# yeyupiaoling/PPASR

Hardware: AMD Instinct MI355X
Metric: audio-seconds/s (RTF^-1) Conformer-streaming fbank, batch32 per GPU, ctc_greedy (higher is better)
Workload: dtype f32; 1 GPU; configs[1]: Conformer streaming (configs/conformer.yml), fbank-80, 32 x 10 s utterances per GPU, V=4233, ctc_greedy, features resident in HBM -> token ids + scores on device; global_batch=32, frames=1000, decoder=ctc_greedy, parallelism=utterance-dp1, pipelined=False, gemm=f32

## Files before the change

include/ppasr_hip.h:

```cpp
#ifndef PPASR_HIP_H
#define PPASR_HIP_H

#include <stddef.h>
#include <stdint.h>

#define PPASR_API __attribute__((visibility("default")))

#ifdef __cplusplus
extern "C" {
#endif

typedef struct ppasr_model_s* ppasr_handle;
typedef struct ppasr_stream_s* ppasr_stream;

typedef enum {
  PPASR_OK = 0,
  PPASR_EINVAL = 1,
  PPASR_EHIP = 2,
  PPASR_EUNSUPPORTED = 3,
  PPASR_EMISSING = 4,
  PPASR_ENOSPACE = 5
} ppasr_status;

enum { PPASR_MODEL_CONFORMER = 0, PPASR_MODEL_EFFICIENT_CONFORMER = 1,
       PPASR_MODEL_SQUEEZEFORMER = 2, PPASR_MODEL_DEEPSPEECH2 = 3 };

typedef struct {
  const char* name;
  const float* data_host;
  int ndim;
  int64_t shape[4];
} ppasr_weight_blob;

typedef struct {
  int model_type;
  int input_dim;
  int vocab_size;
  int output_size;
  int attention_heads;
  int linear_units;
  int num_blocks;
  int cnn_module_kernel;
  int causal;
  int max_len;
  int reduce_idx;
  int recover_idx;
  int stride_layer_idx;
  int group_layer_mask;
  int group_size;
  int use_gru;
  int input_layer;
  int options;
  int stride_layer_mask;
} ppasr_model_desc;

enum {
  PPASR_OPT_POS_REL = 0,
  PPASR_OPT_POS_ABS = 1,
  PPASR_OPT_POS_NONE = 2,
  PPASR_OPT_POS_MASK = 3,
  PPASR_OPT_POST_NORM = 4,
  PPASR_OPT_CONCAT_AFTER = 8,
  PPASR_OPT_NO_MACARON = 16,
  PPASR_OPT_NO_CNN = 32,
  PPASR_OPT_SQ_NO_ADAPTIVE_SCALE = 4096,
  PPASR_OPT_SQ_PRE_NORM = 8192,
  PPASR_OPT_ACT_SHIFT = 8,
  PPASR_OPT_ACT_MASK = 15
};
enum { PPASR_ACT_SWISH = 0, PPASR_ACT_RELU = 1, PPASR_ACT_GELU = 2, PPASR_ACT_TANH = 3, PPASR_ACT_HARDTANH = 4,
       PPASR_ACT_RELU6 = 5, PPASR_ACT_LEAKYRELU = 6, PPASR_ACT_SELU = 7, PPASR_ACT_ELU = 8, PPASR_ACT_HARDSWISH = 9,
       PPASR_ACT_HARDSHRINK = 10 };

PPASR_API const char* ppasr_last_error(void);
PPASR_API const char* ppasr_version(void);

PPASR_API ppasr_status ppasr_create(const ppasr_model_desc* desc, const ppasr_weight_blob* weights_host, int n_weights,
                          ppasr_handle* out);
PPASR_API ppasr_status ppasr_destroy(ppasr_handle h);

PPASR_API int ppasr_out_frames(ppasr_handle h, int T);
PPASR_API size_t ppasr_workspace_bytes(ppasr_handle h, int B, int T);

PPASR_API ppasr_status ppasr_encode(ppasr_handle h, const float* feats, const int64_t* lens, int B, int T,
                          float* probs, float* logits, int32_t* frame_argmax, float* frame_maxprob,
                          void* workspace, size_t workspace_bytes, void* stream);

PPASR_API ppasr_status ppasr_set_debug_taps(ppasr_handle h, float* taps, size_t n_floats);

PPASR_API ppasr_status ppasr_set_skip_padding(ppasr_handle h, int enable);

PPASR_API ppasr_status ppasr_set_ffn_split(ppasr_handle h, int mode);

PPASR_API ppasr_status ppasr_set_front_fused(ppasr_handle h, int mode);

#define PPASR_ROW_BLOCK_32_W16 1032
PPASR_API ppasr_status ppasr_set_row_block(ppasr_handle h, int rows);

#define PPASR_GEMM_F32 0
#define PPASR_GEMM_F16X3 1
#define PPASR_GEMM_COVERS_LAYERS 1
#define PPASR_GEMM_COVERS_FRONT 2
#define PPASR_GEMM_COVERS_HEAD 4
PPASR_API ppasr_status ppasr_set_gemm_mode(ppasr_handle h, int mode);
PPASR_API int ppasr_gemm_coverage(ppasr_handle h);
PPASR_API ppasr_status ppasr_set_gemm_guard(ppasr_handle h, int enable);
PPASR_API ppasr_status ppasr_gemm_guard_stats(ppasr_handle h, long long* fallbacks_host, long long* events_host);
PPASR_API ppasr_status ppasr_set_lengths_hint(ppasr_handle h, const int64_t* lens_host, int B);

PPASR_API long long ppasr_edit_distance(const int32_t* a, int na, const int32_t* b, int nb);

PPASR_API size_t ppasr_ctc_beam_state_bytes(int B, int max_frames, int beam_size);
PPASR_API size_t ppasr_ctc_beam_scratch_bytes(int B, int T, int V, int beam_size, double cutoff_prob, int cutoff_top_n);
PPASR_API ppasr_status ppasr_ctc_beam_state_grow(const void* old_state, size_t old_bytes, void* new_state, size_t new_bytes, int B,
                                       int beam_size, void* stream);
PPASR_API ppasr_status ppasr_ctc_beam_status(const void* state, size_t state_bytes, int B, int beam_size, int32_t* status_host,
                                   void* stream);
PPASR_API ppasr_status ppasr_ctc_beam_state_compact(void* state, size_t state_bytes, int B, int beam_size, int rebuild_table,
                                          int32_t* live_nodes_host, void* stream);
PPASR_API ppasr_status ppasr_ctc_beam_search(const float* probs, const int32_t* frame_lens, int B, int T, int V, int beam_size,
                                   double cutoff_prob, int cutoff_top_n, int blank, int nbest, int max_tokens,
                                   int32_t* tokens, int32_t* lens, double* scores, void* state, size_t state_bytes,
                                   int init_state, void* stream);

typedef struct ppasr_lm_s* ppasr_lm_handle;
PPASR_API ppasr_status ppasr_lm_create(const char* model_path, const char* const* vocab_utf8, int V, ppasr_lm_handle* out);
PPASR_API ppasr_status ppasr_lm_create_arpa(const char* arpa_path, const char* const* vocab_utf8, int V, ppasr_lm_handle* out);
PPASR_API ppasr_status ppasr_lm_create_klm(const char* klm_path, const char* const* vocab_utf8, int V, ppasr_lm_handle* out);
PPASR_API const char*  ppasr_lm_format(ppasr_lm_handle lm);
PPASR_API int          ppasr_lm_word_index(ppasr_lm_handle lm, int token);
PPASR_API int          ppasr_lm_bos(ppasr_lm_handle lm);
PPASR_API int          ppasr_lm_eos(ppasr_lm_handle lm);
PPASR_API ppasr_status ppasr_lm_debug_load_host(const char* model_path, const char* const* vocab_utf8, int V, ppasr_lm_handle* out);
PPASR_API double       ppasr_lm_debug_host_score(ppasr_lm_handle lm, const int32_t* window);
PPASR_API ppasr_status ppasr_lm_destroy(ppasr_lm_handle lm);
PPASR_API int          ppasr_lm_order(ppasr_lm_handle lm);
PPASR_API int          ppasr_lm_is_character_based(ppasr_lm_handle lm);
PPASR_API long long    ppasr_lm_dict_size(ppasr_lm_handle lm);
PPASR_API int          ppasr_lm_space_id(ppasr_lm_handle lm);
PPASR_API long long    ppasr_lm_ngram_count(ppasr_lm_handle lm);
PPASR_API ppasr_status ppasr_ctc_beam_search_lm(const float* probs, const int32_t* frame_lens, int B, int T, int V, int beam_size,
                                      double cutoff_prob, int cutoff_top_n, int blank, int nbest, int max_tokens,
                                      int32_t* tokens, int32_t* lens, double* scores, void* state, size_t state_bytes,
                                      int init_state, ppasr_lm_handle lm, double alpha, double beta, void* stream);
PPASR_API ppasr_status ppasr_ctc_beam_search_ws(const float* probs, const int32_t* frame_lens, int B, int T, int V, int beam_size,
                                      double cutoff_prob, int cutoff_top_n, int blank, int nbest, int max_tokens,
                                      int32_t* tokens, int32_t* lens, double* scores, void* state, size_t state_bytes,
                                      int init_state, ppasr_lm_handle lm, double alpha, double beta, void* scratch,
                                      size_t scratch_bytes, void* stream);

PPASR_API ppasr_status ppasr_hyp_pack(const int32_t* tokens, long long token_stride, int L, const int32_t* n_tokens,
                                      long long n_stride, const double* score, long long score_stride, const int32_t* index,
                                      int k, int32_t* rec, int row0, int cols, int extra, void* stream);
PPASR_API ppasr_status ppasr_hyp_unpack(const int32_t* rec, const int64_t* order, int N, int cols, int extra, int32_t* tokens,
                                        int32_t* n_tokens, double* score, int32_t* index, void* stream);

PPASR_API ppasr_status ppasr_stream_create(ppasr_handle h, ppasr_stream* out);
PPASR_API ppasr_status ppasr_stream_destroy(ppasr_stream s);
PPASR_API ppasr_status ppasr_stream_reset(ppasr_stream s, void* stream);
PPASR_API int ppasr_stream_offset(ppasr_stream s);
PPASR_API int ppasr_stream_cache_frames(ppasr_stream s);
PPASR_API size_t ppasr_chunk_workspace_bytes(ppasr_handle h, int T);
PPASR_API ppasr_status ppasr_encode_chunk(ppasr_stream s, const float* feats, int T, int required_cache_size, float* probs,
                                int32_t* frame_argmax, float* frame_maxprob, int* c_out_host, void* workspace,
                                size_t workspace_bytes, void* stream);
PPASR_API ppasr_status ppasr_stream_export_cache(ppasr_stream s, float* att_cache, float* cnn_cache, void* stream);
PPASR_API ppasr_status ppasr_stream_import_cache(ppasr_stream s, const float* att_cache, int cache_t, const float* cnn_cache,
                                       int offset, void* stream);

PPASR_API size_t ppasr_ds2_workspace_bytes(ppasr_handle h, int B, int T);
PPASR_API ppasr_status ppasr_debug_occupy_cus(int n_workgroups, int milliseconds, void* stream);
PPASR_API ppasr_status ppasr_ds2_encode(ppasr_handle h, const float* feats, const int64_t* lens, int B, int T, const float* init_h,
                              const float* init_c, float* probs, int64_t* out_lens, float* final_h, float* final_c,
                              void* workspace, size_t workspace_bytes, void* stream);

#define PPASR_N_KERNEL_CLASSES 10
PPASR_API ppasr_status ppasr_profile_enable(ppasr_handle h, int enable);
PPASR_API ppasr_status ppasr_profile_read(ppasr_handle h, float* total_ms_host, int* launches_host);
PPASR_API const char* ppasr_kernel_class_name(int cls);

#define PPASR_KPROF_NAME_LEN 160
PPASR_API ppasr_status ppasr_kprof_begin(void);
PPASR_API ppasr_status ppasr_kprof_end(int max_entries, char* names_host, float* total_ms_host, int* launches_host, int* n_out_host);

PPASR_API ppasr_status ppasr_ctc_greedy(const float* probs, const int32_t* frame_lens, int B, int Tp, int V, int blank,
                              int32_t* tokens, int32_t* n_tokens, double* score,
                              void* workspace , size_t workspace_bytes, void* stream);

PPASR_API ppasr_status ppasr_ctc_collapse(const int32_t* frame_argmax, const float* frame_maxprob, const int32_t* frame_lens,
                                int B, int Tp, int blank, int32_t* tokens, int32_t* n_tokens, double* score,
                                void* stream);

typedef struct ppasr_stream_group_s* ppasr_stream_group;
PPASR_API ppasr_status ppasr_stream_group_create(ppasr_handle h, int n_sessions, int max_frames, ppasr_stream_group* out);
PPASR_API ppasr_status ppasr_sq_stream_group_create(ppasr_handle h, int n_sessions, int max_frames, ppasr_stream_group* out);
PPASR_API ppasr_status ppasr_eff_stream_group_create(ppasr_handle h, int n_sessions, int max_frames, ppasr_stream_group* out);
PPASR_API ppasr_status ppasr_ds2_stream_group_create(ppasr_handle h, int n_sessions, int max_frames, ppasr_stream_group* out);
PPASR_API ppasr_status ppasr_gen_stream_group_create(ppasr_handle h, int n_sessions, int max_frames, ppasr_stream_group* out);
PPASR_API ppasr_status ppasr_stream_group_destroy(ppasr_stream_group g);
PPASR_API ppasr_status ppasr_stream_group_reset(ppasr_stream_group g, int session , void* stream);
PPASR_API int          ppasr_stream_group_offset(ppasr_stream_group g, int session);
PPASR_API size_t       ppasr_group_chunk_workspace_bytes(ppasr_handle h, int n, int T);
PPASR_API ppasr_status ppasr_encode_chunk_group(ppasr_stream_group g, const int* sessions_host, int n, const float* feats, int T,
                                      float* probs, int32_t* frame_argmax, float* frame_maxprob, int* c_out_host,
                                      void* workspace, size_t workspace_bytes, void* stream);

typedef struct ppasr_beam_pool_s* ppasr_beam_pool;
PPASR_API ppasr_status ppasr_beam_pool_create(int n_sessions, int V, int beam_size, double cutoff_prob, int cutoff_top_n,
                                              int blank, ppasr_lm_handle lm , double alpha, double beta,
                                              int init_frames, ppasr_beam_pool* out);
PPASR_API ppasr_status ppasr_beam_pool_destroy(ppasr_beam_pool pool);
PPASR_API ppasr_status ppasr_beam_pool_reset(ppasr_beam_pool pool, int session, void* stream);
PPASR_API long long    ppasr_beam_pool_frames(ppasr_beam_pool pool, int session);
PPASR_API long long    ppasr_beam_pool_capacity(ppasr_beam_pool pool, int session);
PPASR_API ppasr_status ppasr_beam_pool_status(ppasr_beam_pool pool, int32_t* status_host, void* stream);
PPASR_API size_t       ppasr_beam_pool_workspace_bytes(ppasr_beam_pool pool, int n, int T);
PPASR_API ppasr_status ppasr_beam_pool_decode(ppasr_beam_pool pool, const int* sessions_host, int n, const float* probs, int T,
                                              const int32_t* frame_lens_host, int max_tokens, int32_t* tokens, int32_t* lens,
                                              double* scores, void* workspace, size_t workspace_bytes, void* stream);

PPASR_API ppasr_status ppasr_beam_arena_compact(ppasr_beam_pool pool, const int* sessions_host, int n, long long* live_nodes_host,
                                                void* stream);
PPASR_API ppasr_status ppasr_beam_arena_set_auto(ppasr_beam_pool pool, int enable);
PPASR_API long long    ppasr_beam_arena_live_nodes(ppasr_beam_pool pool, int session);
PPASR_API size_t       ppasr_beam_arena_bytes(ppasr_beam_pool pool);

typedef struct ppasr_fbank_s* ppasr_fbank_handle;
PPASR_API ppasr_status ppasr_fbank_create(int sample_rate, int n_mels, float frame_length_ms, float frame_shift_ms,
                                ppasr_fbank_handle* out);
PPASR_API ppasr_status ppasr_fbank_destroy(ppasr_fbank_handle f);
PPASR_API int          ppasr_fbank_frames(ppasr_fbank_handle f, int n_samples);
PPASR_API size_t       ppasr_fbank_workspace_bytes(ppasr_fbank_handle f, int n_samples);
PPASR_API ppasr_status ppasr_fbank_compute(ppasr_fbank_handle f, const float* samples, int n_samples, int use_db_norm,
                                 float target_db, float* feats, void* workspace, size_t workspace_bytes, void* stream);

typedef struct {
  long long first_sample;
  long long out_row;
  int n_samples;
  int first_chunk;
  int first_frame;
  int reserved;
} ppasr_fbank_segment;
PPASR_API ppasr_status ppasr_fbank_plan_batch(int sample_rate, float frame_length_ms, float frame_shift_ms, const int* n_samples,
                                    int n, int t_max, ppasr_fbank_segment* table, int* total_chunks, int* total_frames);
PPASR_API size_t       ppasr_fbank_batch_workspace_bytes(int n, int total_chunks);
PPASR_API ppasr_status ppasr_fbank_compute_batch(ppasr_fbank_handle f, const float* samples, const ppasr_fbank_segment* table_dev,
                                       int n, int total_chunks, int total_frames, int use_db_norm, float target_db,
                                       float* feats, void* workspace, size_t workspace_bytes, void* stream);

#ifdef __cplusplus
}
#endif
#endif
```

ppasr_amd/_lib.py:

```python
import ctypes
import os

_HERE = os.path.dirname(os.path.abspath(__file__))
LIB_PATH = os.environ.get("PPASR_HIP_LIB") or os.path.join(_HERE, "libppasr_hip.so")

c_i32p = ctypes.POINTER(ctypes.c_int32)
c_i64p = ctypes.POINTER(ctypes.c_int64)
c_f32p = ctypes.POINTER(ctypes.c_float)
c_f64p = ctypes.POINTER(ctypes.c_double)

PPASR_OK, PPASR_EINVAL, PPASR_EHIP, PPASR_EUNSUPPORTED, PPASR_EMISSING, PPASR_ENOSPACE = range(6)

PPASR_MODEL_CONFORMER = 0
PPASR_MODEL_EFFICIENT_CONFORMER = 1
PPASR_MODEL_SQUEEZEFORMER = 2
PPASR_MODEL_DEEPSPEECH2 = 3
N_KERNEL_CLASSES = 10
PPASR_OPT_POST_NORM, PPASR_OPT_CONCAT_AFTER, PPASR_OPT_NO_MACARON, PPASR_OPT_NO_CNN, PPASR_OPT_ACT_SHIFT = 4, 8, 16, 32, 8
PPASR_OPT_SQ_NO_ADAPTIVE_SCALE = 4096
PPASR_OPT_SQ_PRE_NORM = 8192
PPASR_GEMM_F32 = 0
PPASR_GEMM_F16X3 = 1
PPASR_GEMM_COVERS_LAYERS, PPASR_GEMM_COVERS_FRONT, PPASR_GEMM_COVERS_HEAD = 1, 2, 4
KPROF_NAME_LEN = 160


class WeightBlob(ctypes.Structure):
    _fields_ = [("name", ctypes.c_char_p), ("data_host", ctypes.c_void_p), ("ndim", ctypes.c_int),
                ("shape", ctypes.c_int64 * 4)]


class FbankSegment(ctypes.Structure):
    _fields_ = [("first_sample", ctypes.c_longlong), ("out_row", ctypes.c_longlong), ("n_samples", ctypes.c_int),
                ("first_chunk", ctypes.c_int), ("first_frame", ctypes.c_int), ("reserved", ctypes.c_int)]


class ModelDesc(ctypes.Structure):
    _fields_ = [("model_type", ctypes.c_int), ("input_dim", ctypes.c_int), ("vocab_size", ctypes.c_int),
                ("output_size", ctypes.c_int), ("attention_heads", ctypes.c_int), ("linear_units", ctypes.c_int),
                ("num_blocks", ctypes.c_int), ("cnn_module_kernel", ctypes.c_int), ("causal", ctypes.c_int),
                ("max_len", ctypes.c_int), ("reduce_idx", ctypes.c_int), ("recover_idx", ctypes.c_int),
                ("stride_layer_idx", ctypes.c_int), ("group_layer_mask", ctypes.c_int), ("group_size", ctypes.c_int),
                ("use_gru", ctypes.c_int), ("input_layer", ctypes.c_int), ("options", ctypes.c_int),
                ("stride_layer_mask", ctypes.c_int)]


_vp = ctypes.c_void_p
SYMBOLS = [
    ("ppasr_last_error", ctypes.c_char_p, []),
    ("ppasr_version", ctypes.c_char_p, []),
    ("ppasr_create", ctypes.c_int, [ctypes.POINTER(ModelDesc), ctypes.POINTER(WeightBlob), ctypes.c_int,
                                    ctypes.POINTER(_vp)]),
    ("ppasr_destroy", ctypes.c_int, [_vp]),
    ("ppasr_out_frames", ctypes.c_int, [_vp, ctypes.c_int]),
    ("ppasr_workspace_bytes", ctypes.c_size_t, [_vp, ctypes.c_int, ctypes.c_int]),
    ("ppasr_encode", ctypes.c_int, [_vp, _vp, _vp, ctypes.c_int, ctypes.c_int, _vp, _vp, _vp, _vp, _vp,
                                    ctypes.c_size_t, _vp]),
    ("ppasr_set_debug_taps", ctypes.c_int, [_vp, _vp, ctypes.c_size_t]),
    ("ppasr_set_skip_padding", ctypes.c_int, [_vp, ctypes.c_int]),
    ("ppasr_set_row_block", ctypes.c_int, [_vp, ctypes.c_int]),
    ("ppasr_set_lengths_hint", ctypes.c_int, [_vp, _vp, ctypes.c_int]),
    ("ppasr_set_ffn_split", ctypes.c_int, [_vp, ctypes.c_int]),
    ("ppasr_set_front_fused", ctypes.c_int, [_vp, ctypes.c_int]),
    ("ppasr_set_gemm_mode", ctypes.c_int, [_vp, ctypes.c_int]),
    ("ppasr_gemm_coverage", ctypes.c_int, [_vp]),
    ("ppasr_set_gemm_guard", ctypes.c_int, [_vp, ctypes.c_int]),
    ("ppasr_gemm_guard_stats", ctypes.c_int, [_vp, ctypes.POINTER(ctypes.c_longlong), ctypes.POINTER(ctypes.c_longlong)]),
    ("ppasr_edit_distance", ctypes.c_longlong, [_vp, ctypes.c_int, _vp, ctypes.c_int]),
    ("ppasr_ctc_beam_state_bytes", ctypes.c_size_t, [ctypes.c_int, ctypes.c_int, ctypes.c_int]),
    ("ppasr_ctc_beam_search", ctypes.c_int, [_vp, _vp, ctypes.c_int, ctypes.c_int, ctypes.c_int, ctypes.c_int,
                                             ctypes.c_double, ctypes.c_int, ctypes.c_int, ctypes.c_int, ctypes.c_int,
                                             _vp, _vp, _vp, _vp, ctypes.c_size_t, ctypes.c_int, _vp]),
    ("ppasr_stream_create", ctypes.c_int, [_vp, ctypes.POINTER(_vp)]),
    ("ppasr_stream_destroy", ctypes.c_int, [_vp]),
    ("ppasr_stream_reset", ctypes.c_int, [_vp, _vp]),
    ("ppasr_stream_offset", ctypes.c_int, [_vp]),
    ("ppasr_stream_cache_frames", ctypes.c_int, [_vp]),
    ("ppasr_chunk_workspace_bytes", ctypes.c_size_t, [_vp, ctypes.c_int]),
    ("ppasr_encode_chunk", ctypes.c_int, [_vp, _vp, ctypes.c_int, ctypes.c_int, _vp, _vp, _vp,
                                          ctypes.POINTER(ctypes.c_int), _vp, ctypes.c_size_t, _vp]),
    ("ppasr_stream_export_cache", ctypes.c_int, [_vp, _vp, _vp, _vp]),
    ("ppasr_stream_import_cache", ctypes.c_int, [_vp, _vp, ctypes.c_int, _vp, ctypes.c_int, _vp]),
    ("ppasr_ds2_workspace_bytes", ctypes.c_size_t, [_vp, ctypes.c_int, ctypes.c_int]),
    ("ppasr_ds2_encode", ctypes.c_int, [_vp, _vp, _vp, ctypes.c_int, ctypes.c_int, _vp, _vp, _vp, _vp, _vp, _vp, _vp,
                                        ctypes.c_size_t, _vp]),
    ("ppasr_debug_occupy_cus", ctypes.c_int, [ctypes.c_int, ctypes.c_int, _vp]),
    ("ppasr_profile_enable", ctypes.c_int, [_vp, ctypes.c_int]),
    ("ppasr_profile_read", ctypes.c_int, [_vp, c_f32p, c_i32p]),
    ("ppasr_kernel_class_name", ctypes.c_char_p, [ctypes.c_int]),
    ("ppasr_kprof_begin", ctypes.c_int, []),
    ("ppasr_kprof_end", ctypes.c_int, [ctypes.c_int, _vp, c_f32p, c_i32p, ctypes.POINTER(ctypes.c_int)]),
    ("ppasr_ctc_greedy", ctypes.c_int, [_vp, _vp, ctypes.c_int, ctypes.c_int, ctypes.c_int, ctypes.c_int, _vp, _vp,
                                        _vp, _vp, ctypes.c_size_t, _vp]),
    ("ppasr_ctc_collapse", ctypes.c_int, [_vp, _vp, _vp, ctypes.c_int, ctypes.c_int, ctypes.c_int, _vp, _vp, _vp,
                                          _vp]),
    ("ppasr_lm_create_arpa", ctypes.c_int, [ctypes.c_char_p, ctypes.POINTER(ctypes.c_char_p), ctypes.c_int,
                                            ctypes.POINTER(_vp)]),
    ("ppasr_ctc_beam_scratch_bytes", ctypes.c_size_t, [ctypes.c_int, ctypes.c_int, ctypes.c_int, ctypes.c_int,
                                                       ctypes.c_double, ctypes.c_int]),
    ("ppasr_ctc_beam_search_ws", ctypes.c_int, [_vp, _vp, ctypes.c_int, ctypes.c_int, ctypes.c_int, ctypes.c_int,
                                                ctypes.c_double, ctypes.c_int, ctypes.c_int, ctypes.c_int, ctypes.c_int,
                                                _vp, _vp, _vp, _vp, ctypes.c_size_t, ctypes.c_int, _vp, ctypes.c_double,
                                                ctypes.c_double, _vp, ctypes.c_size_t, _vp]),
    ("ppasr_ctc_beam_status", ctypes.c_int, [_vp, ctypes.c_size_t, ctypes.c_int, ctypes.c_int, _vp, _vp]),
    ("ppasr_ctc_beam_state_grow", ctypes.c_int, [_vp, ctypes.c_size_t, _vp, ctypes.c_size_t, ctypes.c_int, ctypes.c_int, _vp]),
    ("ppasr_hyp_pack", ctypes.c_int, [_vp, ctypes.c_longlong, ctypes.c_int, _vp, ctypes.c_longlong, _vp, ctypes.c_longlong, _vp,
                                      ctypes.c_int, _vp, ctypes.c_int, ctypes.c_int, ctypes.c_int, _vp]),
    ("ppasr_hyp_unpack", ctypes.c_int, [_vp, _vp, ctypes.c_int, ctypes.c_int, ctypes.c_int, _vp, _vp, _vp, _vp, _vp]),
    ("ppasr_lm_create", ctypes.c_int, [ctypes.c_char_p, ctypes.POINTER(ctypes.c_char_p), ctypes.c_int,
                                       ctypes.POINTER(_vp)]),
    ("ppasr_lm_create_klm", ctypes.c_int, [ctypes.c_char_p, ctypes.POINTER(ctypes.c_char_p), ctypes.c_int,
                                           ctypes.POINTER(_vp)]),
    ("ppasr_lm_debug_load_host", ctypes.c_int, [ctypes.c_char_p, ctypes.POINTER(ctypes.c_char_p), ctypes.c_int,
                                                ctypes.POINTER(_vp)]),
    ("ppasr_lm_debug_host_score", ctypes.c_double, [_vp, _vp]),
    ("ppasr_lm_format", ctypes.c_char_p, [_vp]),
    ("ppasr_lm_word_index", ctypes.c_int, [_vp, ctypes.c_int]),
    ("ppasr_lm_bos", ctypes.c_int, [_vp]),
    ("ppasr_lm_eos", ctypes.c_int, [_vp]),
    ("ppasr_lm_destroy", ctypes.c_int, [_vp]),
    ("ppasr_lm_order", ctypes.c_int, [_vp]),
    ("ppasr_lm_is_character_based", ctypes.c_int, [_vp]),
    ("ppasr_lm_dict_size", ctypes.c_longlong, [_vp]),
    ("ppasr_lm_space_id", ctypes.c_int, [_vp]),
    ("ppasr_lm_ngram_count", ctypes.c_longlong, [_vp]),
    ("ppasr_ctc_beam_search_lm", ctypes.c_int, [_vp, _vp, ctypes.c_int, ctypes.c_int, ctypes.c_int, ctypes.c_int,
                                                ctypes.c_double, ctypes.c_int, ctypes.c_int, ctypes.c_int, ctypes.c_int,
                                                _vp, _vp, _vp, _vp, ctypes.c_size_t, ctypes.c_int, _vp, ctypes.c_double,
                                                ctypes.c_double, _vp]),
    ("ppasr_stream_group_create", ctypes.c_int, [_vp, ctypes.c_int, ctypes.c_int, ctypes.POINTER(_vp)]),
    ("ppasr_sq_stream_group_create", ctypes.c_int, [_vp, ctypes.c_int, ctypes.c_int, ctypes.POINTER(_vp)]),
    ("ppasr_eff_stream_group_create", ctypes.c_int, [_vp, ctypes.c_int, ctypes.c_int, ctypes.POINTER(_vp)]),
    ("ppasr_ds2_stream_group_create", ctypes.c_int, [_vp, ctypes.c_int, ctypes.c_int, ctypes.POINTER(_vp)]),
    ("ppasr_gen_stream_group_create", ctypes.c_int, [_vp, ctypes.c_int, ctypes.c_int, ctypes.POINTER(_vp)]),
    ("ppasr_stream_group_destroy", ctypes.c_int, [_vp]),
    ("ppasr_stream_group_reset", ctypes.c_int, [_vp, ctypes.c_int, _vp]),
    ("ppasr_stream_group_offset", ctypes.c_int, [_vp, ctypes.c_int]),
    ("ppasr_group_chunk_workspace_bytes", ctypes.c_size_t, [_vp, ctypes.c_int, ctypes.c_int]),
    ("ppasr_encode_chunk_group", ctypes.c_int, [_vp, ctypes.POINTER(ctypes.c_int), ctypes.c_int, _vp, ctypes.c_int, _vp,
                                                _vp, _vp, ctypes.POINTER(ctypes.c_int), _vp, ctypes.c_size_t, _vp]),
    ("ppasr_beam_pool_create", ctypes.c_int, [ctypes.c_int, ctypes.c_int, ctypes.c_int, ctypes.c_double, ctypes.c_int,
                                              ctypes.c_int, _vp, ctypes.c_double, ctypes.c_double, ctypes.c_int,
                                              ctypes.POINTER(_vp)]),
    ("ppasr_beam_pool_destroy", ctypes.c_int, [_vp]),
    ("ppasr_beam_pool_reset", ctypes.c_int, [_vp, ctypes.c_int, _vp]),
    ("ppasr_beam_pool_frames", ctypes.c_longlong, [_vp, ctypes.c_int]),
    ("ppasr_beam_pool_capacity", ctypes.c_longlong, [_vp, ctypes.c_int]),
    ("ppasr_beam_pool_status", ctypes.c_int, [_vp, _vp, _vp]),
    ("ppasr_beam_pool_workspace_bytes", ctypes.c_size_t, [_vp, ctypes.c_int, ctypes.c_int]),
    ("ppasr_beam_pool_decode", ctypes.c_int, [_vp, ctypes.POINTER(ctypes.c_int), ctypes.c_int, _vp, ctypes.c_int, _vp,
                                              ctypes.c_int, _vp, _vp, _vp, _vp, ctypes.c_size_t, _vp]),
    ("ppasr_ctc_beam_state_compact", ctypes.c_int, [_vp, ctypes.c_size_t, ctypes.c_int, ctypes.c_int, ctypes.c_int, _vp, _vp]),
    ("ppasr_beam_arena_compact", ctypes.c_int, [_vp, ctypes.POINTER(ctypes.c_int), ctypes.c_int,
                                                ctypes.POINTER(ctypes.c_longlong), _vp]),
    ("ppasr_beam_arena_set_auto", ctypes.c_int, [_vp, ctypes.c_int]),
    ("ppasr_beam_arena_live_nodes", ctypes.c_longlong, [_vp, ctypes.c_int]),
    ("ppasr_beam_arena_bytes", ctypes.c_size_t, [_vp]),
    ("ppasr_fbank_create", ctypes.c_int, [ctypes.c_int, ctypes.c_int, ctypes.c_float, ctypes.c_float,
                                          ctypes.POINTER(_vp)]),
    ("ppasr_fbank_destroy", ctypes.c_int, [_vp]),
    ("ppasr_fbank_frames", ctypes.c_int, [_vp, ctypes.c_int]),
    ("ppasr_fbank_workspace_bytes", ctypes.c_size_t, [_vp, ctypes.c_int]),
    ("ppasr_fbank_compute", ctypes.c_int, [_vp, _vp, ctypes.c_int, ctypes.c_int, ctypes.c_float, _vp, _vp,
                                           ctypes.c_size_t, _vp]),
    ("ppasr_fbank_plan_batch", ctypes.c_int, [ctypes.c_int, ctypes.c_float, ctypes.c_float, _vp, ctypes.c_int, ctypes.c_int,
                                              _vp, ctypes.POINTER(ctypes.c_int), ctypes.POINTER(ctypes.c_int)]),
    ("ppasr_fbank_batch_workspace_bytes", ctypes.c_size_t, [ctypes.c_int, ctypes.c_int]),
    ("ppasr_fbank_compute_batch", ctypes.c_int, [_vp, _vp, _vp, ctypes.c_int, ctypes.c_int, ctypes.c_int, ctypes.c_int,
                                                 ctypes.c_float, _vp, _vp, ctypes.c_size_t, _vp]),
]

_lib = None


class PPASRHipError(RuntimeError):

    def __init__(self, msg, status=None):
        super().__init__(msg)
        self.status = status


def load():
    global _lib
    if _lib is not None:
        return _lib
    if not os.path.exists(LIB_PATH):
        raise PPASRHipError(
            f"{LIB_PATH} not found: build it with `python -c 'import __graft_entry__ as g; g.build()'` "
            "(hipcc --offload-arch=gfx950).  There is no CPU fallback.")
    lib = ctypes.CDLL(LIB_PATH)
    for name, restype, argtypes in SYMBOLS:
        fn = getattr(lib, name)
        fn.restype = restype
        fn.argtypes = argtypes
    _lib = lib
    return lib


def check(status):
    if status != 0:
        msg = load().ppasr_last_error()
        raise PPASRHipError(f"libppasr_hip status {status}: {msg.decode() if msg else ''}", status=int(status))


class kernel_profile:

    _stack = []

    def __init__(self, max_entries=128):
        self.max_entries = max_entries
        self.kernels = {}

    @staticmethod
    def _drain():
        n = max([k.max_entries for k in kernel_profile._stack] + [512])
        names = ctypes.create_string_buffer(n * KPROF_NAME_LEN)
        ms = (ctypes.c_float * n)()
        cnt = (ctypes.c_int32 * n)()
        got = ctypes.c_int(0)
        check(load().ppasr_kprof_end(n, ctypes.addressof(names), ms, cnt, ctypes.byref(got)))
        for i in range(got.value):
            nm = names.raw[i * KPROF_NAME_LEN:(i + 1) * KPROF_NAME_LEN].split(b"\0", 1)[0].decode()
            for scope in kernel_profile._stack:
                t, c = scope.kernels.get(nm, (0.0, 0))
                scope.kernels[nm] = (t + float(ms[i]), c + int(cnt[i]))

    def __enter__(self):
        if kernel_profile._stack:
            kernel_profile._drain()
        kernel_profile._stack.append(self)
        check(load().ppasr_kprof_begin())
        return self

    def __exit__(self, *exc):
        kernel_profile._drain()
        kernel_profile._stack.pop()
        if kernel_profile._stack:
            check(load().ppasr_kprof_begin())
        return False
```

ppasr_amd/csrc/capi.hip:

```cpp
#include <cxxabi.h>
#include <cstdlib>

#include "capi_internal.h"

namespace ppasr {
thread_local LaunchProf g_launch_prof;
}

static thread_local std::string g_err;
std::string& ppasr_err_slot() { return g_err; }

static ppasr_status validate_desc(const ppasr_model_desc* desc, ppasr_model_s* m) {
  m->desc = *desc;
  const int F = desc->input_dim;
  if (desc->model_type == PPASR_MODEL_DEEPSPEECH2) {
    if (F > 128 || F < 7) return fail(PPASR_EUNSUPPORTED, "input_dim out of range");
    m->F1 = (F - 1) / 2;
    m->F2 = (m->F1 - 1) / 2;
    if (m->F1 > 40) return fail(PPASR_EUNSUPPORTED, "deepspeech2: input_dim <= 82 ((input_dim - 1) / 2 <= 40)");
    return PPASR_OK;
  }
  if (desc->model_type != PPASR_MODEL_CONFORMER && desc->model_type != PPASR_MODEL_SQUEEZEFORMER &&
      desc->model_type != PPASR_MODEL_EFFICIENT_CONFORMER)
    return fail(PPASR_EUNSUPPORTED, "model_type not built (conformer, efficient_conformer, squeezeformer are)");
  const bool eff = desc->model_type == PPASR_MODEL_EFFICIENT_CONFORMER;
  const unsigned smask = eff_stride_mask(*desc);
  const bool multi_stride = __builtin_popcount(smask) > 1;
  if (eff) {
    if (desc->group_layer_mask != 0 && (desc->group_size < 2 || desc->group_size > 4))
      return fail(PPASR_EUNSUPPORTED, "efficient_conformer: grouped attention is built for group_size 2, 3 and 4");
    if (desc->num_blocks > 31 || (smask >> desc->num_blocks) != 0) return fail(PPASR_EINVAL, "stride layer index out of range");
    if (smask != 0 && !multi_stride && desc->cnn_module_kernel != 15 && desc->output_size == kD)
      return fail(PPASR_EUNSUPPORTED, "efficient_conformer: cnn_module_kernel must be 15 (7 after the stride layer)");
    if ((desc->cnn_module_kernel >> __builtin_popcount(smask)) < 1)
      return fail(PPASR_EINVAL, "efficient_conformer: cnn_module_kernel halves to 0 behind the stride layers");
  }
  if (desc->output_size % 256 != 0 || desc->output_size < 256 || desc->output_size > 1024)
    return fail(PPASR_EUNSUPPORTED, "output_size must be 256, 512, 768 or 1024");
  if (desc->attention_heads * 64 != desc->output_size) return fail(PPASR_EUNSUPPORTED, "kernels are specialised for d_k=64");
  const bool fused_ks = desc->cnn_module_kernel == 15 || desc->cnn_module_kernel == 31 || desc->cnn_module_kernel == 7;
  const bool generic = (desc->model_type == PPASR_MODEL_CONFORMER &&
                        (desc->output_size != kD || desc->options != 0 || desc->input_layer == 1 || !fused_ks)) ||
                       ((desc->model_type == PPASR_MODEL_SQUEEZEFORMER || desc->model_type == PPASR_MODEL_EFFICIENT_CONFORMER) &&
                        desc->output_size != kD) ||
                       (eff && multi_stride) ||
                       (desc->model_type == PPASR_MODEL_SQUEEZEFORMER &&
                        (((desc->options >> PPASR_OPT_ACT_SHIFT) & PPASR_OPT_ACT_MASK) != PPASR_ACT_SWISH ||
                         (desc->options & PPASR_OPT_SQ_PRE_NORM) != 0 ||
                         (desc->options & PPASR_OPT_POS_MASK) != PPASR_OPT_POS_REL));
  const int sq_opts = desc->model_type == PPASR_MODEL_SQUEEZEFORMER
                          ? (PPASR_OPT_SQ_NO_ADAPTIVE_SCALE | PPASR_OPT_SQ_PRE_NORM | PPASR_OPT_POS_MASK |
                             (PPASR_OPT_ACT_MASK << PPASR_OPT_ACT_SHIFT)) : 0;
  if (((desc->options & ~sq_opts) != 0 || desc->input_layer == 1) && desc->model_type != PPASR_MODEL_CONFORMER)
    return fail(PPASR_EUNSUPPORTED, "non-default encoder options / input_layer=linear are built for model_type=conformer");
  if ((desc->options & (PPASR_OPT_SQ_NO_ADAPTIVE_SCALE | PPASR_OPT_SQ_PRE_NORM)) && desc->model_type != PPASR_MODEL_SQUEEZEFORMER)
    return fail(PPASR_EINVAL, "PPASR_OPT_SQ_NO_ADAPTIVE_SCALE / PPASR_OPT_SQ_PRE_NORM are Squeezeformer options");
  if (desc->linear_units % 256 != 0 || desc->linear_units <= 0) return fail(PPASR_EUNSUPPORTED, "linear_units % 256 != 0");
  if (!generic && !fused_ks) return fail(PPASR_EUNSUPPORTED, "cnn_module_kernel must be 7, 15 or 31");
  if (generic) {
    const int ks = desc->cnn_module_kernel;
    const bool use_cnn = !(desc->options & PPASR_OPT_NO_CNN);
    if (use_cnn && (ks < 1 || ks > 63 || (!desc->causal && ks % 2 == 0)))
      return fail(PPASR_EINVAL, "cnn_module_kernel: 1..63, odd for the non-causal conv module (convolution.py:38)");
    if ((desc->options & PPASR_OPT_POS_MASK) == 3 || ((desc->options >> PPASR_OPT_ACT_SHIFT) & PPASR_OPT_ACT_MASK) > PPASR_ACT_HARDSHRINK)
      return fail(PPASR_EINVAL, "options: unknown pos_enc_layer_type / activation_type code");
  }
  if (desc->model_type == PPASR_MODEL_SQUEEZEFORMER && desc->cnn_module_kernel == 7)
    return fail(PPASR_EUNSUPPORTED, "squeezeformer: cnn_module_kernel must be 15 or 31");
  if (desc->input_dim > 128 || (desc->input_dim < 7 && desc->input_layer != 1) || desc->input_dim < 1)
    return fail(PPASR_EUNSUPPORTED, "input_dim out of range");
  if (eff) {
    m->desc.stride_layer_mask = (int)smask;
    m->desc.stride_layer_idx = smask ? __builtin_ctz(smask) : -1;
  }
  const int il = desc->input_layer;
  if (il != 0 && il != 1 && il != 6 && il != 8)
    return fail(PPASR_EINVAL, "input_layer: 0 (conv2d), 1 (linear), 6 (conv2d6) or 8 (conv2d8)");
  m->generic = generic;
  m->gen.pos = desc->options & PPASR_OPT_POS_MASK;
  m->gen.post_norm = (desc->options & PPASR_OPT_POST_NORM) != 0;
  m->gen.concat_after = (desc->options & PPASR_OPT_CONCAT_AFTER) != 0;
  m->gen.macaron = !(desc->options & PPASR_OPT_NO_MACARON);
  m->gen.use_cnn = !(desc->options & PPASR_OPT_NO_CNN);
  m->gen.act = (desc->options >> PPASR_OPT_ACT_SHIFT) & PPASR_OPT_ACT_MASK;
  m->gen.sq_pre_norm = (desc->options & PPASR_OPT_SQ_PRE_NORM) != 0;
  if (il != 0 && desc->model_type == PPASR_MODEL_SQUEEZEFORMER)
    return fail(PPASR_EUNSUPPORTED, "squeezeformer: only the conv2d front end is built");
  m->F1 = (F - 1) / 2;
  if (il == 6 && m->F1 < 5) return fail(PPASR_EINVAL, "input_dim too small for this input_layer (conv2d6: >= 11)");
  m->F2 = il == 6 ? (m->F1 - 5) / 3 + 1 : (m->F1 - 1) / 2;
  m->F3 = il == 8 ? (m->F2 - 1) / 2 : 0;
  if (il != 1 && m->F_last() < 1) return fail(PPASR_EINVAL, "input_dim too small for this input_layer");
  return PPASR_OK;
}

extern "C" {

const char* ppasr_last_error(void) { return g_err.c_str(); }
const char* ppasr_version(void) { return "ppasr_hip 0.1 (gfx950, fp32 MFMA)"; }

ppasr_status ppasr_create(const ppasr_model_desc* desc, const ppasr_weight_blob* blobs, int n_blobs, ppasr_handle* out) {
  if (!desc || !blobs || !out) return fail(PPASR_EINVAL, "null argument");
  std::unique_ptr<ppasr_model_s> m(new ppasr_model_s());
  LOAD_TRY(validate_desc(desc, m.get()));
  HIP_TRY(configure_kernels());
  if (desc->model_type != PPASR_MODEL_DEEPSPEECH2) {
    HIP_TRY(configure_generic_kernels());
    HIP_TRY(configure_squeezeformer_kernels());
  }
  const BlobMap sd = blob_map(blobs, n_blobs);
  Loader ld{m.get(), sd, ""};
  switch (desc->model_type) {
    case PPASR_MODEL_DEEPSPEECH2: LOAD_TRY(ds2_create(m.get(), ld)); break;
    case PPASR_MODEL_SQUEEZEFORMER: LOAD_TRY(squeezeformer_create(m.get(), ld)); break;
    default: LOAD_TRY(conformer_create(m.get(), ld));
  }
  HIP_TRY(hipDeviceSynchronize());
  *out = m.release();
  return PPASR_OK;
}

ppasr_status ppasr_destroy(ppasr_handle h) {
  delete h;
  return PPASR_OK;
}

int ppasr_out_frames(ppasr_handle h, int T) {
  if (T < (h ? h->min_frames() : 7)) return 0;
  int tp = h ? h->front_dims(T).Tp : ((T - 1) / 2 - 1) / 2;
  if (h)
    for (int n = __builtin_popcount(eff_stride_mask(h->desc)); n > 0; --n) tp = (tp + 1) / 2;
  return tp;
}

}
WsLayout ws_layout(const ppasr_model_s* m, int B, int T) {
  if (m->generic) {
    WsLayout g{};
    g.total = generic_ws_floats(m, B, T);
    return g;
  }
  const auto fd = m->front_dims(T);
  const size_t T1 = fd.T1, Tp = fd.Tp;
  const size_t M = (size_t)B * Tp;
  auto al = [](size_t n) { return (n + 63) & ~(size_t)63; };
  WsLayout w;
  size_t o = 0;
  const size_t split_rows = m->ffn_split > 1 ? (size_t)m->ffn_split * M
                          : m->ffn_split == 0 ? 0 : std::min((size_t)8 * M, (size_t)256 * kRows);
  w.y1 = o; o += al(std::max((size_t)B * T1 * m->F1 * kD, 4 * split_rows * kD));
  const size_t y2_floats = (size_t)B * (fd.T2 ? fd.T2 : Tp) * m->F2 * kD;
  w.y2 = o; o += al(m->desc.input_layer == 8 ? std::max(y2_floats, split_rows * kD) : y2_floats);
  w.xa = o; o += al(M * kD);
  w.xb = o; o += al(M * kD);
  w.xc = o; o += al(M * kD);
  w.qkv = o; o += al(M * 3 * kD);
  w.ctx = o; o += al(M * kD);
  w.g = o; o += al(M * kD);
  w.rmax = o; o += al(M);
  w.rsum = o; o += al(M);
  w.fa = o; o += al(M);
  w.fp = o; o += al(M);
  w.xs = o; o += al(M * kD);
  w.vt_stride = (int)(al(M) + 128);
  w.vt = o; o += al((size_t)kD * w.vt_stride);
  w.total = o;
  return w;
}
int wide_slices_for(const ppasr_model_s* m, int M, int units) {
  const int S = ffn_split_for(m, M);
  if (S <= 1) return S;
  const int blocks = (M + kRows - 1) / kRows;
  return std::max(S, std::min(units, 256 / blocks));
}
int ffn_split_for(const ppasr_model_s* m, int M) {
  if (m->desc.model_type == PPASR_MODEL_DEEPSPEECH2) return 1;
  const int n_chunks = m->desc.linear_units / 256;
  if (m->ffn_split >= 0) return m->ffn_split > 1 ? m->ffn_split : 1;
  const int blocks = (M + kRows - 1) / kRows;
  if (blocks > 128) return 1;
  int S = 8;
  while (S > 1 && (blocks * S > 256 || n_chunks % S != 0)) S >>= 1;
  return S;
}

bool block_tables_enabled() {
  static const bool on = [] {
    const char* e = getenv("PPASR_BLOCK_TABLE");
    return !(e && e[0] == '0');
  }();
  return on;
}

bool conv12_enabled(const ppasr_model_s* m) { return m->front_fused != 0; }

int row_block_for(const ppasr_model_s* m, int B, int Tcur, int mul, int slack, bool skip) {
  if (m->row_block == 16 || m->row_block == 32 || m->row_block == kW16) return m->row_block;
  long long rows = (long long)B * Tcur;
  if (skip && (int)m->lens_hint.size() == B) {
    rows = 0;
    for (int b = 0; b < B; ++b) {
      const long long len = m->lens_hint[b];
      const long long need = (len > 0 ? (len + mul - 1) / mul : 0) + slack;
      rows += need < Tcur ? need : Tcur;
    }
  }
  constexpr int min_blocks = 32;
  const long long b32 = (rows + 31) / 32, b16 = (rows + 15) / 16;
  if (b32 <= min_blocks) return 32;
  const double c32 = (double)((b32 + 255) / 256), c16 = 0.52 * (double)((b16 + 255) / 256);
  return c16 < c32 ? 16 : 32;
}

extern "C" {

ppasr_status ppasr_set_row_block(ppasr_handle h, int rows) {
  if (!h) return fail(PPASR_EINVAL, "null handle");
  if (rows != -1 && rows != 16 && rows != 32 && rows != PPASR_ROW_BLOCK_32_W16)
    return fail(PPASR_EINVAL, "row block: -1 (by grid size), 16, 32 or PPASR_ROW_BLOCK_32_W16");
  h->row_block = rows;
  return PPASR_OK;
}

ppasr_status ppasr_set_lengths_hint(ppasr_handle h, const int64_t* lens_host, int B) {
  if (!h) return fail(PPASR_EINVAL, "null handle");
  if (!lens_host || B <= 0) h->lens_hint.clear();
  else h->lens_hint.assign(lens_host, lens_host + B);
  return PPASR_OK;
}

size_t ppasr_workspace_bytes(ppasr_handle h, int B, int T) {
  if (!h || B <= 0 || T < 7) return 0;
  return ws_layout(h, B, T).total * sizeof(float);
}

ppasr_status ppasr_set_debug_taps(ppasr_handle h, float* taps, size_t n_floats) {
  if (!h) return fail(PPASR_EINVAL, "null handle");
  h->taps = taps;
  h->taps_floats = taps ? n_floats : 0;
  return PPASR_OK;
}

long long ppasr_edit_distance(const int32_t* a, int na, const int32_t* b, int nb) {
  if (na < 0 || nb < 0 || (na > 0 && !a) || (nb > 0 && !b)) return -1;
  if (na < nb) {
    std::swap(a, b);
    std::swap(na, nb);
  }
  if (nb == 0) return na;
  std::vector<int> prev(nb + 1), cur(nb + 1);
  for (int j = 0; j <= nb; ++j) prev[j] = j;
  for (int i = 1; i <= na; ++i) {
    cur[0] = i;
    const int32_t ca = a[i - 1];
    for (int j = 1; j <= nb; ++j) {
      const int sub = prev[j - 1] + (ca != b[j - 1]);
      const int del = prev[j] + 1, ins = cur[j - 1] + 1;
      cur[j] = sub < del ? (sub < ins ? sub : ins) : (del < ins ? del : ins);
    }
    std::swap(prev, cur);
  }
  return prev[nb];
}

ppasr_status ppasr_set_ffn_split(ppasr_handle h, int mode) {
  if (!h) return fail(PPASR_EINVAL, "null handle");
  if (mode != -1 && mode != 0 && mode != 2 && mode != 4 && mode != 8) return fail(PPASR_EINVAL, "ffn split: -1, 0, 2, 4 or 8");
  if (mode > 0 && (h->desc.linear_units / 256) % mode != 0) return fail(PPASR_EINVAL, "ffn split must divide linear_units / 256");
  h->ffn_split = mode;
  return PPASR_OK;
}

ppasr_status ppasr_set_front_fused(ppasr_handle h, int mode) {
  if (!h) return fail(PPASR_EINVAL, "null handle");
  if (mode < -1 || mode > 1) return fail(PPASR_EINVAL, "front fused: -1 (default), 0 or 1");
  h->front_fused = mode;
  return PPASR_OK;
}

struct GuardPtrs {
  const unsigned int* p[ppasr_model_s::kGuardN];
};
__global__ void k_h3_snapshot(GuardPtrs g, unsigned int* dst) {
  for (int i = 0; i < ppasr_model_s::kGuardN; ++i) dst[i] = *g.p[i];
}
static GuardPtrs guard_ptrs(ppasr_handle h) {
  GuardPtrs g;
  for (int i = 0; i < ppasr_model_s::kGuardN; ++i) g.p[i] = h->guard_ctr[i];
  return g;
}

static ppasr_status guard_alloc(ppasr_handle h) {
  if (h->guard_dev) return PPASR_OK;
  constexpr int N = ppasr_model_s::kGuardN;
  h->guard_ctr[0] = conformer_h3_ovf_counter();
  h->guard_ctr[1] = squeezeformer_h3_ovf_counter();
  h->guard_ctr[2] = front_h3_ovf_counter();
  h->guard_ctr[3] = ctc_head_h3_ovf_counter();
  h->guard_ctr[4] = split_route_h3_ovf_counter();
  for (int i = 0; i < N; ++i)
    if (!h->guard_ctr[i]) return fail(PPASR_EHIP, "fp16 x3 range guard: counter symbols not found");
  void* d = nullptr;
  LOAD_TRY(h->alloc(2 * N * sizeof(unsigned int), &d));
  h->guard_dev = static_cast<unsigned int*>(d);
  void* p = nullptr;
  HIP_TRY(hipHostMalloc(&p, 2 * N * sizeof(unsigned int), hipHostMallocDefault));
  h->guard_host = static_cast<unsigned int*>(p);
  return PPASR_OK;
}

ppasr_status ppasr_set_gemm_mode(ppasr_handle h, int mode) {
  if (!h) return fail(PPASR_EINVAL, "null handle");
  if (mode != PPASR_GEMM_F32 && mode != PPASR_GEMM_F16X3) return fail(PPASR_EINVAL, "gemm mode: PPASR_GEMM_F32 or PPASR_GEMM_F16X3");
  if (mode == PPASR_GEMM_F16X3) {
    const int mt = h->desc.model_type;
    bool layers_ok = (mt == PPASR_MODEL_CONFORMER || mt == PPASR_MODEL_EFFICIENT_CONFORMER) && !h->generic && !h->layers.empty();
    for (size_t i = 0; layers_ok && i < h->layers.size(); ++i)
      layers_ok = conv_ffn_h3_supported(h->layer_ks[i]) && h->layers[i].ffm_w1 != nullptr;
    const bool front_ok = !h->generic && mt != PPASR_MODEL_DEEPSPEECH2 && h->desc.input_layer == 0 && h->front.conv2_k == 3 &&
                          h->front.conv2_w != nullptr;
    const bool sq_ok = mt == PPASR_MODEL_SQUEEZEFORMER && !h->generic && !h->sq_layers.empty() &&
                       sq_h3_supported(h->desc.cnn_module_kernel, 4);
    if (!layers_ok && !front_ok && !sq_ok)
      return fail(PPASR_EUNSUPPORTED, "fp16 x3 GEMMs: built for the fused 256-wide routes (feed-forward modules of Conformer / "
                                      "Efficient-Conformer / Squeezeformer layers; conv2 of the 4x front end)");
    const int d = h->desc.output_size, H = h->desc.linear_units;
    {
      const ppasr_status g = guard_alloc(h);
      if (g != PPASR_OK) return g;
    }
    unsigned int w_before = 0, w_after = 0;
    unsigned int* w_ovf = nullptr;
    HIP_TRY(hipMalloc(reinterpret_cast<void**>(&w_ovf), sizeof(unsigned int)));
    struct OvfFree { unsigned int* p; ~OvfFree() { (void)hipFree(p); } } w_ovf_free{w_ovf};
    HIP_TRY(hipMemset(w_ovf, 0, sizeof(unsigned int)));
    const size_t alloc_mark = h->allocs.size();
    auto repack = [&](const f32x4** w, int n_tiles, int G) -> ppasr_status {
      void* dst = nullptr;
      LOAD_TRY(h->alloc((size_t)n_tiles * G * 256 * sizeof(float), &dst));
      launch_repack_h3(*w, static_cast<f32x4*>(dst), n_tiles, G, w_ovf, nullptr);
      *w = static_cast<const f32x4*>(dst);
      return PPASR_OK;
    };
    HIP_TRY(hipDeviceSynchronize());
    if (layers_ok && h->layers_h3.empty()) {
      std::vector<LayerW> view = h->layers;
      for (LayerW& L : view) {
        struct { const f32x4** w; int n_tiles, G; } items[8] = {
            {&L.ffm_w1, H / 32, d / 8}, {&L.ffm_w2, d / 32, H / 8}, {&L.ff_w1, H / 32, d / 8}, {&L.ff_w2, d / 32, H / 8},
            {&L.wqkv, 3 * d / 32, d / 8}, {&L.wo, d / 32, d / 8},   {&L.pw1, 2 * d / 32, d / 8}, {&L.pw2, d / 32, d / 8}};
        for (auto& it : items) LOAD_TRY(repack(it.w, it.n_tiles, it.G));
        if (L.ptab != h->zero_vec) {
          void* dst = nullptr;
          LOAD_TRY(h->alloc((size_t)h->desc.max_len * d * sizeof(float), &dst));
          launch_split_rows_h3(L.ptab, static_cast<float*>(dst), h->desc.max_len, w_ovf, nullptr);
          L.ptab = static_cast<const float*>(dst);
        }
      }
      HIP_TRY(hipGetLastError());
      HIP_TRY(hipDeviceSynchronize());
      h->layers_h3 = std::move(view);
    }
    if (sq_ok && h->sq_layers_h3.empty()) {
      std::vector<SqLayerW> view = h->sq_layers;
      for (SqLayerW& L : view) {
        const f32x4** w[4] = {&L.ff1_w1, &L.ff1_w2, &L.ff2_w1, &L.ff2_w2};
        for (int j = 0; j < 4; ++j) LOAD_TRY(repack(w[j], (j & 1) ? d / 32 : H / 32, (j & 1) ? H / 8 : d / 8));
      }
      HIP_TRY(hipGetLastError());
      HIP_TRY(hipDeviceSynchronize());
      h->sq_layers_h3 = std::move(view);
    }
    if ((layers_ok || sq_ok || front_ok) && !h->head_w_h3 && h->head.w) {
      const f32x4* w = h->head.w;
      LOAD_TRY(repack(&w, h->head.n_tiles, d / 8));
      HIP_TRY(hipGetLastError());
      HIP_TRY(hipDeviceSynchronize());
      h->head_w_h3 = w;
    }
    if (front_ok && !h->conv2_w_h3) {
      const f32x4 *wc = h->front.conv2_w, *we = h->front.embed_w;
      LOAD_TRY(repack(&wc, d / 32, 9 * d / 8));
      LOAD_TRY(repack(&we, d / 32, h->F2 * d / 8));
      HIP_TRY(hipGetLastError());
      HIP_TRY(hipDeviceSynchronize());
      h->conv2_w_h3 = wc;
      h->embed_w_h3 = we;
    }
    HIP_TRY(hipDeviceSynchronize());
    HIP_TRY(hipMemcpy(&w_after, w_ovf, sizeof(unsigned int), hipMemcpyDeviceToHost));
    if (w_after != w_before) {
      h->layers_h3.clear();
      h->sq_layers_h3.clear();
      h->head_w_h3 = h->conv2_w_h3 = h->embed_w_h3 = nullptr;
      for (size_t i = alloc_mark; i < h->allocs.size(); ++i) (void)hipFree(h->allocs[i]);
      h->allocs.resize(alloc_mark);
      return fail(PPASR_EUNSUPPORTED, "fp16 x3 GEMMs: a weight of magnitude >= 255.9 (or a positional-table entry >= 4094) does not fit the scaled fp16 pieces");
    }
    for (int i = 0; i < ppasr_model_s::kGuardN; ++i)
      HIP_TRY(hipMemcpy(&h->guard_seen[i], h->guard_ctr[i], sizeof(unsigned int), hipMemcpyDeviceToHost));
    h->gemm_coverage = (layers_ok ? PPASR_GEMM_COVERS_LAYERS : 0) | (sq_ok ? PPASR_GEMM_COVERS_LAYERS : 0) |
                       (front_ok ? PPASR_GEMM_COVERS_FRONT : 0) | (h->head_w_h3 ? PPASR_GEMM_COVERS_HEAD : 0);
  } else {
    h->gemm_coverage = 0;
  }
  h->gemm_mode = mode;
  return PPASR_OK;
}

int ppasr_gemm_coverage(ppasr_handle h) { return h ? h->gemm_coverage : 0; }

ppasr_status ppasr_set_skip_padding(ppasr_handle h, int enable) {
  if (!h) return fail(PPASR_EINVAL, "null handle");
  if (enable && (h->desc.model_type == PPASR_MODEL_DEEPSPEECH2 || h->desc.input_layer == 1))
    return fail(PPASR_EUNSUPPORTED, "skip_padding: built behind the conv front ends (DeepSpeech2 and input_layer = linear "
                                    "compute every row)");
  h->skip_padding = enable != 0;
  return PPASR_OK;
}

static ppasr_status encode_impl(ppasr_handle h, const float* feats, const int64_t* lens, int B, int T, float* probs,
                                float* logits, int32_t* frame_argmax, float* frame_maxprob, void* workspace,
                                size_t workspace_bytes, void* stream) {
  if (!h || !feats || !workspace) return fail(PPASR_EINVAL, "null argument");
  if (B <= 0 || T < h->min_frames()) return fail(PPASR_EINVAL, "need B > 0 and T >= 7 (conv2d6: 11, conv2d8: 15) frames");
  if (h->desc.model_type == PPASR_MODEL_DEEPSPEECH2) return fail(PPASR_EINVAL, "deepspeech2 handles use ppasr_ds2_encode");
  const auto fd = h->front_dims(T);
  const int F = h->desc.input_dim, T1 = fd.T1, F1 = h->F1, Tp = fd.Tp, F2 = h->F2;
  const int sub = h->sub_rate();
  if (Tp >= h->desc.max_len) return fail(PPASR_EINVAL, "utterance longer than the positional table (embedding.py:64-66)");
  const int M = B * Tp;
  const WsLayout wl = ws_layout(h, B, T);
  if (workspace_bytes < wl.total * sizeof(float)) return fail(PPASR_ENOSPACE, "workspace too small");
  hipStream_t st = static_cast<hipStream_t>(stream);
  float* ws = static_cast<float*>(workspace);
  if (h->generic)
    return h->desc.model_type == PPASR_MODEL_SQUEEZEFORMER
               ? generic_sq_encode(h, feats, lens, B, T, probs, logits, frame_argmax, frame_maxprob, ws, st)
               : generic_encode(h, feats, lens, B, T, probs, logits, frame_argmax, frame_maxprob, ws, st);
  if (h->desc.model_type == PPASR_MODEL_SQUEEZEFORMER)
    return squeezeformer_encode(h, feats, lens, B, T, probs, logits, frame_argmax, frame_maxprob, ws, wl, st);
  float *y1 = ws + wl.y1, *y2 = ws + wl.y2, *xa = ws + wl.xa, *xb = ws + wl.xb, *xc = ws + wl.xc;
  float *qkv = ws + wl.qkv, *ctx = ws + wl.ctx, *g = ws + wl.g;
  const VtOut vt_out{ws + wl.vt, wl.vt_stride};
  HIP_TRY(hipMemsetAsync(ws + wl.vt, 0, (size_t)kD * wl.vt_stride * sizeof(float), st));
  size_t tap_off = 0;
  auto tap = [&](const float* src, size_t n) {
    if (h->taps && tap_off + n <= h->taps_floats)
      (void)hipMemcpyAsync(h->taps + tap_off, src, n * sizeof(float), hipMemcpyDeviceToDevice, st);
    tap_off += n;
  };
  if (h->prof) {
    h->ev_used = 0;
    h->spans.clear();
  }
  auto timed = [&](int cls, auto&& fn) {
    if (!h->prof) {
      fn();
      return;
    }
    h->spans.push_back({cls, {}});
    g_launch_prof.ctx = h;
    g_launch_prof.next = [](void* ctx, const void*, hipEvent_t* s, hipEvent_t* e) {
      ppasr_model_s* m = static_cast<ppasr_model_s*>(ctx);
      *s = m->next_event();
      *e = m->next_event();
      m->spans.back().ev.emplace_back(*s, *e);
    };
    fn();
    g_launch_prof = LaunchProf{};
  };
  const bool eff = h->desc.model_type == PPASR_MODEL_EFFICIENT_CONFORMER;
  const bool skip = h->skip_padding && lens && !h->taps && h->desc.input_layer != 1;
  const bool skip_front = skip && h->desc.input_layer == 0;
  constexpr int fuse_min_blocks = 128;
  auto fuse_rows = [&](int rows) {
    return ffn_split_for(h, rows) == 1 &&
           (h->ffn_split == 0 || (rows + kRows - 1) / kRows > fuse_min_blocks);
  };
  if (skip && fuse_rows(M)) HIP_TRY(hipMemsetAsync(y2, 0, (wl.rmax - wl.y2) * sizeof(float), st));
  const int rc = h->desc.causal ? 0 : (h->desc.cnn_module_kernel - 1) / 2;
  const int slack_half = rc + 4, slack_full = eff ? 2 * slack_half + rc + 8 : rc + 4;
  auto pskip = [&](int Tcur, int mul_cur) {
    PadSkip ps;
    if (skip) {
      ps.lens = lens;
      ps.Tp = Tcur;
      ps.mul = mul_cur;
      ps.slack = mul_cur == sub ? slack_full : slack_half;
    }
    return ps;
  };
  const f32x4* conv2_h3 = h->gemm_mode == PPASR_GEMM_F16X3 ? h->conv2_w_h3 : nullptr;
  const bool conv12 = h->desc.input_layer == 0 && !conv2_h3 && conv12_enabled(h) && conv12_supported(h->front, F, F2);
  const PadSkip ps_front = skip_front ? pskip(Tp, sub) : PadSkip{};
  if (!conv12) timed(0, [&] { launch_conv1(feats, h->front, y1, B, T, F, T1, F1, st, ps_front); });
  if (h->desc.input_layer == 8) {
    timed(1, [&] {
      launch_conv_stage(y1, h->front.conv2_w, h->front.conv2_b, y2, B, T1, F1, fd.T2, F2, 3, 2, st);
      launch_conv_stage(y2, h->front.conv3_w, h->front.conv3_b, y1, B, fd.T2, F2, Tp, h->F3, 3, 2, st);
    });
    timed(2, [&] { launch_embed(y1, h->front, xa, M, h->F3 * kD, sqrtf((float)kD), false, st, PadSkip{}, ffn_split_for(h, M), y2); });
  } else {
    timed(1, [&] {
      int* tile_tab = (size_t)B + 2 <= ((size_t)M + 63) / 64 * 64 ? reinterpret_cast<int*>(ws + wl.rmax) : nullptr;
      if (conv12) launch_conv12(feats, h->front, y2, B, T, F, Tp, F2, st, ps_front, tile_tab);
      else if (h->desc.input_layer == 0 && !conv2_h3 && conv2_quad_supported(h->front))
        launch_conv2_quad(y1, h->front, y2, B, T1, F1, Tp, F2, st, ps_front, tile_tab);
      else launch_conv2(y1, h->front, y2, B, T1, F1, Tp, F2, st, ps_front, tile_tab, h->desc.input_layer == 0 ? conv2_h3 : nullptr);
    });
    timed(2, [&] {
      launch_embed(y2, h->front, xa, M, F2 * kD, sqrtf((float)kD), false, st, ps_front, wide_slices_for(h, M, F2), y1,
                   conv2_h3 ? h->embed_w_h3 : nullptr);
    });
  }
  tap(xa, (size_t)M * kD);
  const int n_chunks = h->desc.linear_units / 256;
  struct BlkTab { int Ti, R; int* tab; } btabs[4];
  int n_bt = 0;
  size_t bt_off = ((size_t)B + 2 + 15) / 16 * 16;
  const bool bt_ok = skip && block_tables_enabled() && (size_t)B + 2 <= ((size_t)M + 63) / 64 * 64;
  auto with_table = [&](PadSkip p, int Tcur, int R) {
    if (!bt_ok) return p;
    for (int k = 0; k < n_bt; ++k)
      if (btabs[k].Ti == Tcur && btabs[k].R == R) { p.tab = btabs[k].tab; return p; }
    const size_t n = 1 + ((size_t)B * Tcur + R - 1) / R;
    if (n_bt == 4 || bt_off + n > 2 * (((size_t)M + 63) / 64 * 64)) return p;
    int* t = reinterpret_cast<int*>(ws + wl.rmax) + bt_off;
    launch_block_table(p, B * Tcur, R, t, st);
    btabs[n_bt++] = BlkTab{Tcur, R, t};
    bt_off += (n + 15) / 16 * 16;
    p.tab = t;
    return p;
  };
  int Ti = Tp, mul = sub, pstride = 1;
  bool s1_done = false;
  for (int i = 0; i < h->desc.num_blocks; ++i) {
    const LayerW& L = h->layers[i];
    const int Mi = B * Ti;
    const int grp = h->layer_group[i];
    auto fusable = [&](int layer) {
      return h->layer_group[layer] == 1 && h->desc.attention_heads == 4 && !h->taps && fuse_rows(Mi);
    };
    const PadSkip ps = pskip(Ti, mul);
    const int rows = (!h->taps && conv_ffn_16_supported(h->layer_ks[i], Ti)) ? row_block_for(h, B, Ti, mul, ps.slack, skip) : 32;
    const bool r16 = rows == 16 && h->ffn_split < 0;
    const bool fuse_attn = !r16 && fusable(i);
    const int S = r16 ? 1 : ffn_split_for(h, Mi);
    const bool w16 = rows == kW16 && S == 1;
    const int form = r16 ? 16 : w16 ? kW16 : 32;
    const PadSkip psb = S == 1 ? with_table(ps, Ti, form_rows(form)) : ps;
    const bool h3 = h->gemm_mode == PPASR_GEMM_F16X3 && !h->layers_h3.empty() && !r16 && !w16 && S == 1;
    const bool h3s = h->gemm_mode == PPASR_GEMM_F16X3 && !h->layers_h3.empty() && S > 1;
    const LayerW& Lk = (h3 || h3s) ? h->layers_h3[i] : L;
    auto vt_for = [&](bool fused, bool mode, int layer) {
      VtOut v = fused ? vt_out : VtOut{};
      v.k_h3 = (fused && mode) ? 1 : 0;
      if (fused && !mode && h->layers[layer].dtab) {
        v.kpos = h->layers[layer].ptab;
        v.kpos_stride = pstride * kD;
        v.Ti = Ti;
      }
      return v;
    };
    float* partial = y1;
    float* x3 = ctx;
    if (!s1_done) {
      if (S > 1) {
        timed(3, [&] {
          launch_ffn_split(xa, L.ln_mac_g, L.ln_mac_b, Lk.ffm_w1, L.ffm_b1, Lk.ffm_w2, L.ffm_b2, 0.5f, nullptr, nullptr, partial,
                           xb, Mi, n_chunks, S, st, ps, false, h3s);
          launch_ln_qkv(xb, qkv, Lk, Mi, st, ps, nullptr, nullptr, h3s);
        });
      } else {
        timed(3, [&] { launch_ffn_qkv(xa, xb, qkv, Lk, Mi, n_chunks, st, psb, vt_for(fuse_attn, h3, i), h3, form); });
      }
    }
    s1_done = false;
    tap(xb, (size_t)Mi * kD);
    tap(qkv, (size_t)Mi * 3 * kD);
    const int Tt = (Ti + grp - 1) / grp;
    AttnArgs a{qkv, 768, qkv + 256, 768, qkv + 512, 768, Tt, Tt, 0, lens, ctx, L.pos_u, L.pos_v, (h3 && fuse_attn) ? Lk.ptab : L.ptab, pstride,
               mul * grp, Ti, Ti, grp};
    a.pad_skip = skip ? ps.slack + 1 : 0;
    a.vt = vt_out.vt;
    a.vt_stride = vt_out.stride;
    if (fuse_attn && !h3) {
      a.dtab = L.dtab;
      a.dtab_len = h->desc.max_len;
    }
    if (fuse_attn) {
      timed(9, [&] { launch_attn_out_glu(a, B, xb, xc, g, Lk, st, h3); });
    } else {
      timed(4, [&] { launch_attention(a, B, h->desc.attention_heads, st); });
      tap(ctx, (size_t)Mi * kD);
      timed(5, [&] {
        launch_out_glu(ctx, xb, xc, g, nullptr, h3s ? Lk : L, lens, Mi, Ti, mul, st, psb, S > 1 ? xa : nullptr, h3s, nullptr, form);
      });
    }
    tap(xc, (size_t)Mi * kD);
    tap(g, (size_t)Mi * kD);
    if (eff && i == h->desc.stride_layer_idx) {
      const int Ts = (Ti + 1) / 2;
      timed(6, [&] {
        const int Ss = r16 ? 1 : ffn_split_for(h, B * Ts);
        if (Ss > 1) {
          launch_conv_ffn_stride(g, nullptr, xc, xa, h3s ? Lk : L, lens, B, Ti, Ts, n_chunks, h->layer_ks[i], mul * 2, st,
                                 pskip(Ts, mul * 2), h->desc.causal != 0, h3s, ctx);
          launch_ffn_split(ctx, L.ln_ff_g, L.ln_ff_b, Lk.ff_w1, L.ff_b1, Lk.ff_w2, L.ff_b2, 0.5f, L.ln_fin_g, L.ln_fin_b, partial,
                           xa, B * Ts, n_chunks, Ss, st, pskip(Ts, mul * 2), false, h3s);
        } else {
          launch_conv_ffn_stride(g, nullptr, xc, xa, (h3 || h3s) ? Lk : L, lens, B, Ti, Ts, n_chunks, h->layer_ks[i], mul * 2, st,
                                 pskip(Ts, mul * 2), h->desc.causal != 0, h3 || h3s);
        }
      });
      Ti = Ts;
      mul *= 2;
      pstride *= 2;
    } else if (S > 1) {
      timed(6, [&] {
        launch_conv_pre(g, nullptr, xc, x3, Lk, lens, Mi, Ti, h->layer_ks[i], mul, st, h->desc.causal != 0, ps, h3s);
        launch_ffn_split(x3, L.ln_ff_g, L.ln_ff_b, Lk.ff_w1, L.ff_b1, Lk.ff_w2, L.ff_b2, 0.5f, L.ln_fin_g, L.ln_fin_b, partial,
                         xa, Mi, n_chunks, S, st, ps, false, h3s);
      });
    } else {
      const LayerW* next = (i + 1 < h->desc.num_blocks) ? (h3 ? &h->layers_h3[i + 1] : &h->layers[i + 1]) : nullptr;
      timed(next ? 8 : 6, [&] {
        launch_conv_ffn(g, nullptr, xc, (next && !h->taps) ? nullptr : xa, Lk, lens, Mi, Ti, n_chunks, h->layer_ks[i], mul, next,
                        xb, qkv, st, h->desc.causal != 0, psb, vt_for(next && fusable(i + 1), h3, next ? i + 1 : i), h3, form);
      });
      s1_done = next != nullptr;
    }
    tap(xa, (size_t)B * Ti * kD);
  }
  const int Mo = B * Ti;
  float* lg = logits ? logits : probs;
  int32_t* fa = frame_argmax ? frame_argmax : reinterpret_cast<int32_t*>(ws + wl.fa);
  float* fp = frame_maxprob ? frame_maxprob : ws + wl.fp;
  timed(7, [&] {
    const bool head_h3 = h->gemm_mode == PPASR_GEMM_F16X3 && h->head_w_h3;
    HeadW hw = h->head;
    if (head_h3) hw.w = h->head_w_h3;
    launch_ctc_head(xa, hw, lg, fa, fp, ws + wl.rmax, ws + wl.rsum, Mo, st, pskip(Ti, mul),
                    wide_slices_for(h, Mo, std::min((hw.n_tiles + 7) / 8, 32)), y1, head_h3);
  });
  if (probs) {
    if (logits)
      HIP_TRY(hipMemcpyAsync(probs, logits, (size_t)Mo * h->head.V * sizeof(float), hipMemcpyDeviceToDevice, st));
    launch_softmax_from_stats(probs, ws + wl.rmax, ws + wl.rsum, Mo, h->head.V, st, pskip(Ti, mul));
  }
  if (skip) launch_zero_pad_rows(probs, logits, fa, fp, lens, B, Ti, mul, h->head.V, st);
  HIP_TRY(hipGetLastError());
  return PPASR_OK;
}

ppasr_status ppasr_encode(ppasr_handle h, const float* feats, const int64_t* lens, int B, int T, float* probs,
                          float* logits, int32_t* frame_argmax, float* frame_maxprob, void* workspace,
                          size_t workspace_bytes, void* stream) {
  if (!h) return fail(PPASR_EINVAL, "null argument");
  if (h->gemm_mode != PPASR_GEMM_F16X3 || !h->gemm_guard || !h->guard_dev)
    return encode_impl(h, feats, lens, B, T, probs, logits, frame_argmax, frame_maxprob, workspace, workspace_bytes, stream);
  hipStream_t st = static_cast<hipStream_t>(stream);
  constexpr int N = ppasr_model_s::kGuardN;
  PPASR_LAUNCH(k_h3_snapshot, dim3(1), dim3(1), 0, st, guard_ptrs(h), h->guard_dev);
  ppasr_status rc = encode_impl(h, feats, lens, B, T, probs, logits, frame_argmax, frame_maxprob, workspace, workspace_bytes, stream);
  if (rc != PPASR_OK) return rc;
  PPASR_LAUNCH(k_h3_snapshot, dim3(1), dim3(1), 0, st, guard_ptrs(h), h->guard_dev + N);
  HIP_TRY(hipMemcpyAsync(h->guard_host, h->guard_dev, 2 * N * sizeof(unsigned int), hipMemcpyDeviceToHost, st));
  HIP_TRY(hipStreamSynchronize(st));
  long long events = 0;
  for (int i = 0; i < N; ++i) {
    h->guard_seen[i] = h->guard_host[N + i];
    events += (long long)(h->guard_host[N + i] - h->guard_host[i]);
  }
  if (events == 0) return PPASR_OK;
  h->guard_events += events;
  h->guard_fallbacks += 1;
  h->gemm_mode = PPASR_GEMM_F32;
  rc = encode_impl(h, feats, lens, B, T, probs, logits, frame_argmax, frame_maxprob, workspace, workspace_bytes, stream);
  h->gemm_mode = PPASR_GEMM_F16X3;
  return rc;
}

ppasr_status ppasr_set_gemm_guard(ppasr_handle h, int enable) {
  if (!h) return fail(PPASR_EINVAL, "null handle");
  h->gemm_guard = enable != 0;
  return PPASR_OK;
}

ppasr_status ppasr_gemm_guard_stats(ppasr_handle h, long long* fallbacks_host, long long* events_host) {
  if (!h) return fail(PPASR_EINVAL, "null handle");
  if (h->guard_dev) {
    HIP_TRY(hipDeviceSynchronize());
    for (int i = 0; i < ppasr_model_s::kGuardN; ++i) {
      unsigned int now = 0;
      HIP_TRY(hipMemcpy(&now, h->guard_ctr[i], sizeof(unsigned int), hipMemcpyDeviceToHost));
      h->guard_events += (long long)(now - h->guard_seen[i]);
      h->guard_seen[i] = now;
    }
  }
  if (fallbacks_host) *fallbacks_host = h->guard_fallbacks;
  if (events_host) *events_host = h->guard_events;
  return PPASR_OK;
}


static ppasr_status beam_config(int V, int beam_size, double cutoff_prob, int cutoff_top_n, int blank, int nbest,
                                int max_tokens, BeamConfig* c) {
  if (V <= 1 || V >= 16384) return fail(PPASR_EUNSUPPORTED, "beam search: vocabulary must be in (1, 16384)");
  if (beam_size < 1 || beam_size > kMaxBeam) return fail(PPASR_EUNSUPPORTED, "beam search: beam_size must be in [1, 512]");
  if (blank < 0 || blank >= V) return fail(PPASR_EINVAL, "beam search: blank id out of range");
  if (nbest < 1 || nbest > beam_size || max_tokens < 1) return fail(PPASR_EINVAL, "beam search: bad nbest / max_tokens");
  if (cutoff_top_n < 1) return fail(PPASR_EINVAL, "beam search: cutoff_top_n < 1");
  const int n_cand = (cutoff_prob < 1.0) ? (cutoff_top_n < V ? cutoff_top_n : V) : V;
  c->V = V; c->beam = beam_size; c->blank = blank; c->cutoff_top_n = cutoff_top_n; c->cutoff_prob = cutoff_prob;
  c->n_cand_max = n_cand; c->nbest = nbest; c->max_tokens = max_tokens; c->max_nodes = 0;
  c->sorted = (cutoff_prob < 1.0 || cutoff_top_n < V) ? 1 : 0;
  {
    const char* m = getenv("PPASR_BEAM_MARGIN");
    c->margin = m ? atoi(m) : 2;
    if (c->margin < 0) c->margin = 0;
  }
  c->list_cap = beam_list_cap(beam_size, V, n_cand, c->lm.order > 0);
  if (c->list_cap <= 0) return fail(PPASR_EUNSUPPORTED, "beam search: beam_size x vocabulary does not fit LDS");
  return PPASR_OK;
}


static size_t beam_max_nodes(size_t F, int beam_size) { return 1 + (F + 1) * (size_t)beam_size; }
static size_t beam_utt_bytes(size_t F, int beam_size) {
  return 4 * beam_state_words(beam_size, (int)beam_max_nodes(F, beam_size)) + 4 + F * 4 * (size_t)prune_rec_words(kSmallCand);
}
static size_t beam_frame_capacity(size_t per_utt_bytes, int beam_size) {
  if (per_utt_bytes < beam_utt_bytes(1, beam_size)) return 0;
  const size_t per_frame = beam_utt_bytes(2, beam_size) - beam_utt_bytes(1, beam_size);
  size_t F = 1 + (per_utt_bytes - beam_utt_bytes(1, beam_size)) / per_frame;
  while (F > 1 && beam_utt_bytes(F, beam_size) > per_utt_bytes) --F;
  return F;
}

size_t ppasr_ctc_beam_state_bytes(int B, int max_frames, int beam_size) {
  if (B <= 0 || max_frames < 0 || beam_size < 1) return 0;
  return (size_t)B * beam_utt_bytes((size_t)(max_frames < 1 ? 1 : max_frames), beam_size);
}

}
namespace ppasr { const LmDev* lm_device_view(ppasr_lm_handle lm); }
extern "C" {

ppasr_status ppasr_ctc_beam_search(const float* probs, const int32_t* frame_lens, int B, int T, int V, int beam_size,
                                   double cutoff_prob, int cutoff_top_n, int blank, int nbest, int max_tokens,
                                   int32_t* tokens, int32_t* lens, double* scores, void* state, size_t state_bytes,
                                   int init_state, void* stream) {
  return ppasr_ctc_beam_search_lm(probs, frame_lens, B, T, V, beam_size, cutoff_prob, cutoff_top_n, blank, nbest, max_tokens,
                                  tokens, lens, scores, state, state_bytes, init_state, nullptr, 0.0, 0.0, stream);
}

ppasr_status ppasr_ctc_beam_search_lm(const float* probs, const int32_t* frame_lens, int B, int T, int V, int beam_size,
                                      double cutoff_prob, int cutoff_top_n, int blank, int nbest, int max_tokens,
                                      int32_t* tokens, int32_t* lens, double* scores, void* state, size_t state_bytes,
                                      int init_state, ppasr_lm_handle lm, double alpha, double beta, void* stream) {
  return ppasr_ctc_beam_search_ws(probs, frame_lens, B, T, V, beam_size, cutoff_prob, cutoff_top_n, blank, nbest, max_tokens,
                                  tokens, lens, scores, state, state_bytes, init_state, lm, alpha, beta, nullptr, 0, stream);
}

size_t ppasr_ctc_beam_scratch_bytes(int B, int T, int V, int beam_size, double cutoff_prob, int cutoff_top_n) {
  BeamConfig c{};
  if (B <= 0 || T < 0) return 0;
  c.lm.order = 1;
  if (beam_config(V, beam_size, cutoff_prob, cutoff_top_n, 0, 1, 1, &c) != PPASR_OK) return 0;
  return beam_scratch_bytes(c, B, T);
}

ppasr_status ppasr_ctc_beam_search_ws(const float* probs, const int32_t* frame_lens, int B, int T, int V, int beam_size,
                                      double cutoff_prob, int cutoff_top_n, int blank, int nbest, int max_tokens,
                                      int32_t* tokens, int32_t* lens, double* scores, void* state, size_t state_bytes,
                                      int init_state, ppasr_lm_handle lm, double alpha, double beta, void* scratch,
                                      size_t scratch_bytes, void* stream) {
  if (!tokens || !lens || !scores || !state || (!probs && T > 0)) return fail(PPASR_EINVAL, "null argument");
  if (B <= 0 || T < 0) return fail(PPASR_EINVAL, "empty batch");
  BeamConfig c{};
  if (lm) {
    c.lm = *ppasr::lm_device_view(lm);
    c.alpha = alpha;
    c.beta = beta;
  }
  ppasr_status s = beam_config(V, beam_size, cutoff_prob, cutoff_top_n, blank, nbest, max_tokens, &c);
  if (s != PPASR_OK) return s;
  c.node_table = lm && c.lm.word_based;
  {
    const char* f = getenv("PPASR_BEAM_FAST");
    c.fast_path = f ? (atoi(f) != 0) : 1;
  }
  const size_t per_utt_bytes = state_bytes / (size_t)B;
  const size_t F = beam_frame_capacity(per_utt_bytes, beam_size);
  if (F == 0) return fail(PPASR_ENOSPACE, "beam search: state buffer too small");
  if ((size_t)T > F) return fail(PPASR_ENOSPACE, "beam search: more frames in one call than the state buffer was sized for");
  c.max_nodes = (int)beam_max_nodes(F, beam_size);
  const size_t block_words = beam_state_words(beam_size, c.max_nodes);
  int32_t* st_words = static_cast<int32_t*>(state);
  int32_t* status = st_words + (size_t)B * block_words;
  int32_t* prune_recs = status + B;
  hipStream_t hs = static_cast<hipStream_t>(stream);
  if (init_state) {
    HIP_TRY(hipMemsetAsync(status, 0, (size_t)B * 4, hs));
    if (c.node_table) {
    const size_t tab_off = (beam_fixed_words(beam_size) + beam_arena_words(c.max_nodes)) * 4, tab_bytes = 12 * beam_table_slots(c.max_nodes);
    HIP_TRY(hipMemset2DAsync(reinterpret_cast<char*>(state) + tab_off, block_words * 4, 0, tab_bytes, (size_t)B, hs));
    }
  }
  const size_t need_scratch = beam_scratch_bytes(c, B, T);
  if (need_scratch > 0 && (!scratch || scratch_bytes < need_scratch))
    return fail(PPASR_ENOSPACE, "beam search: this pruning configuration keeps more characters per frame than the LDS-resident "
                                "search holds (cutoff_prob >= 1 keeps the whole vocabulary): call ppasr_ctc_beam_search_ws with "
                                "ppasr_ctc_beam_scratch_bytes(...) bytes of device scratch");
  HIP_TRY(launch_ctc_beam(probs, frame_lens, B, T, c, prune_recs, st_words, init_state, 1, tokens, lens, scores, status,
                          need_scratch ? scratch : nullptr, hs));
  return PPASR_OK;
}

ppasr_status ppasr_ctc_beam_state_grow(const void* old_state, size_t old_bytes, void* new_state, size_t new_bytes, int B,
                                       int beam_size, void* stream) {
  if (!old_state || !new_state || B <= 0 || beam_size < 1) return fail(PPASR_EINVAL, "null argument");
  const size_t Fo = beam_frame_capacity(old_bytes / (size_t)B, beam_size), Fn = beam_frame_capacity(new_bytes / (size_t)B, beam_size);
  if (Fo == 0 || Fn == 0) return fail(PPASR_ENOSPACE, "beam search: state buffer too small");
  if (Fn < Fo) return fail(PPASR_EINVAL, "beam search: the new state buffer is smaller than the old one");
  const int mo = (int)beam_max_nodes(Fo, beam_size), mn = (int)beam_max_nodes(Fn, beam_size);
  const size_t ow = beam_state_words(beam_size, mo), nw = beam_state_words(beam_size, mn);
  const size_t head_words = beam_fixed_words(beam_size) + beam_arena_words(mo);
  hipStream_t hs = static_cast<hipStream_t>(stream);
  const int32_t* o = static_cast<const int32_t*>(old_state);
  int32_t* n = static_cast<int32_t*>(new_state);
  HIP_TRY(hipMemcpy2DAsync(n, nw * 4, o, ow * 4, head_words * 4, (size_t)B, hipMemcpyDeviceToDevice, hs));
  HIP_TRY(hipMemcpyAsync(n + (size_t)B * nw, o + (size_t)B * ow, (size_t)B * 4, hipMemcpyDeviceToDevice, hs));
  const size_t tab_off = (beam_fixed_words(beam_size) + beam_arena_words(mn)) * 4, tab_bytes = 12 * beam_table_slots(mn);
  HIP_TRY(hipMemset2DAsync(reinterpret_cast<char*>(new_state) + tab_off, nw * 4, 0, tab_bytes, (size_t)B, hs));
  HIP_TRY(launch_beam_rehash(n, B, beam_size, mn, hs));
  return PPASR_OK;
}

ppasr_status ppasr_ctc_beam_status(const void* state, size_t state_bytes, int B, int beam_size, int32_t* status_host,
                                   void* stream) {
  if (!state || B <= 0 || beam_size < 1) return fail(PPASR_EINVAL, "null argument");
  const size_t F = beam_frame_capacity(state_bytes / (size_t)B, beam_size);
  if (F == 0) return fail(PPASR_ENOSPACE, "beam search: state buffer too small");
  const int32_t* status = static_cast<const int32_t*>(state) + (size_t)B * beam_state_words(beam_size, (int)beam_max_nodes(F, beam_size));
  std::vector<int32_t> host(B);
  hipStream_t hs = static_cast<hipStream_t>(stream);
  HIP_TRY(hipMemcpyAsync(host.data(), status, (size_t)B * 4, hipMemcpyDeviceToHost, hs));
  HIP_TRY(hipStreamSynchronize(hs));
  bool any = false;
  for (int b = 0; b < B; ++b) {
    if (status_host) status_host[b] = host[b];
    any |= host[b] != 0;
  }
  if (any) return fail(PPASR_ENOSPACE, "beam search: the prefix arena of at least one utterance is exhausted (state sized for fewer frames)");
  return PPASR_OK;
}

ppasr_status ppasr_ctc_beam_state_compact(void* state, size_t state_bytes, int B, int beam_size, int rebuild_table,
                                          int32_t* live_nodes_host, void* stream) {
  if (!state || B <= 0 || beam_size < 1 || beam_size > kMaxBeam) return fail(PPASR_EINVAL, "beam search: null state, B <= 0 or bad beam_size");
  const size_t F = beam_frame_capacity(state_bytes / (size_t)B, beam_size);
  if (F == 0) return fail(PPASR_EINVAL, "beam search: state buffer too small for one frame");
  const int max_nodes = (int)beam_max_nodes(F, beam_size);
  const size_t block_words = beam_state_words(beam_size, max_nodes);
  int32_t* st_words = static_cast<int32_t*>(state);
  const int32_t* status = st_words + (size_t)B * block_words;
  hipStream_t hs = static_cast<hipStream_t>(stream);
  HIP_TRY(launch_beam_compact(st_words, status, B, beam_size, max_nodes, rebuild_table != 0, nullptr, hs));
  if (!live_nodes_host) return PPASR_OK;
  std::vector<int32_t> stat(B);
  HIP_TRY(hipMemcpy2DAsync(live_nodes_host, 4, st_words + 1, block_words * 4, 4, (size_t)B, hipMemcpyDeviceToHost, hs));
  HIP_TRY(hipMemcpyAsync(stat.data(), status, (size_t)B * 4, hipMemcpyDeviceToHost, hs));
  HIP_TRY(hipStreamSynchronize(hs));
  for (int b = 0; b < B; ++b)
    if (stat[b] != 0) live_nodes_host[b] = -1;
  return PPASR_OK;
}

struct ppasr_beam_pool_s {
  BeamConfig cfg;
  int n_sessions;
  std::vector<int32_t*> block;
  std::vector<size_t> cap;
  std::vector<long long> frames;
  std::vector<long long> used;
  std::vector<long long> live;
  bool auto_compact = false;
  int32_t* status;
  StagingRing ring;
};

namespace {
size_t pool_block_bytes(size_t F, int beam) { return 4 * beam_state_words(beam, (int)beam_max_nodes(F, beam)); }
size_t pool_rec_bytes(const BeamConfig& c, int n, int T) {
  return c.n_cand_max > kSmallCand ? 0 : (((size_t)n * T * prune_rec_words(c.n_cand_max) * 4 + 255) & ~(size_t)255);
}
bool pool_cap_ok(size_t F, int beam) { return F <= (size_t)(0x3fffffff / beam) - 2; }

ppasr_status pool_compact(ppasr_beam_pool_s* p, const int* sessions, int n, long long* live_out, hipStream_t hs) {
  StagingRing::Entry en;
  HIP_TRY(p->ring.acquire(&en));
  BeamSlot* tab = reinterpret_cast<BeamSlot*>(en.host);
  const int beam = p->cfg.beam;
  for (int b = 0; b < n; ++b) {
    const int s = sessions[b];
    tab[b] = BeamSlot{p->block[s], p->status + s, (int)beam_max_nodes(p->cap[s], beam), 0};
  }
  const size_t live_off = (size_t)n * sizeof(BeamSlot);
  HIP_TRY(hipMemcpyAsync(en.dev, en.host, live_off, hipMemcpyHostToDevice, hs));
  HIP_TRY(launch_beam_compact(nullptr, nullptr, n, beam, 0, p->cfg.node_table, reinterpret_cast<int32_t*>(en.dev + live_off), hs,
                              reinterpret_cast<const BeamSlot*>(en.dev)));
  HIP_TRY(hipMemcpyAsync(en.host + live_off, en.dev + live_off, (size_t)n * 4, hipMemcpyDeviceToHost, hs));
  HIP_TRY(hipStreamSynchronize(hs));
  HIP_TRY(p->ring.release(en, hs));
  const int32_t* live = reinterpret_cast<const int32_t*>(en.host + live_off);
  for (int b = 0; b < n; ++b) {
    const int s = sessions[b];
    if (live[b] >= 1) {
      p->live[s] = live[b];
      p->used[s] = ((long long)live[b] - 1 + beam - 1) / beam;
    }
    if (live_out) live_out[b] = live[b];
  }
  return PPASR_OK;
}
}

ppasr_status ppasr_beam_pool_create(int n_sessions, int V, int beam_size, double cutoff_prob, int cutoff_top_n, int blank,
                                    ppasr_lm_handle lm, double alpha, double beta, int init_frames, ppasr_beam_pool* out) {
  if (!out) return fail(PPASR_EINVAL, "null argument");
  *out = nullptr;
  if (n_sessions < 1 || init_frames < 1) return fail(PPASR_EINVAL, "beam pool: n_sessions and init_frames must be >= 1");
  BeamConfig c{};
  if (lm) {
    c.lm = *ppasr::lm_device_view(lm);
    c.alpha = alpha;
    c.beta = beta;
  }
  ppasr_status s = beam_config(V, beam_size, cutoff_prob, cutoff_top_n, blank, 1, 1, &c);
  if (s != PPASR_OK) return s;
// ... 432 lines not shown
```

ppasr_amd/csrc/capi_internal.h:

```cpp
#pragma once
#include <hip/hip_runtime.h>

#include <cmath>
#include <cstdio>
#include <cstring>
#include <memory>
#include <string>
#include <unordered_map>
#include <vector>

#include "../../include/ppasr_hip.h"
#include "conformer_kernels.h"
#include "launch.h"
#include "ctc_beam.h"

using namespace ppasr;

#include "squeezeformer_kernels.h"
#include "ds2_kernels.h"

std::string& ppasr_err_slot();
inline ppasr_status fail(ppasr_status s, const std::string& msg) {
  ppasr_err_slot() = msg;
  return s;
}
#define HIP_TRY(expr)                                                                              \
  do {                                                                                             \
    hipError_t _e = (expr);                                                                        \
    if (_e != hipSuccess) return fail(PPASR_EHIP, std::string(#expr) + ": " + hipGetErrorString(_e)); \
  } while (0)

inline bool session_list_ok(const int* sessions, int n, int n_sessions) {
  std::vector<char> seen(n_sessions, 0);
  for (int b = 0; b < n; ++b) {
    const int s = sessions[b];
    if (s < 0 || s >= n_sessions || seen[s]) return false;
    seen[s] = 1;
  }
  return true;
}

struct StagingRing {
  static constexpr int kRing = 8;
  struct Entry {
    int i;
    char* host;
    char* dev;
  };
  size_t entry_bytes = 0;
  char* host = nullptr;
  char* dev = nullptr;
  hipEvent_t ev[kRing] = {};
  int next = 0;

  hipError_t alloc(size_t bytes) {
    entry_bytes = bytes;
    hipError_t e = hipMalloc(reinterpret_cast<void**>(&dev), kRing * bytes);
    if (e == hipSuccess) e = hipHostMalloc(reinterpret_cast<void**>(&host), kRing * bytes, hipHostMallocDefault);
    for (int i = 0; i < kRing && e == hipSuccess; ++i) {
      e = hipEventCreateWithFlags(&ev[i], hipEventDisableTiming);
      if (e != hipSuccess) ev[i] = nullptr;
    }
    return e;
  }
  hipError_t acquire(Entry* out) {
    const int i = next;
    next = (i + 1) % kRing;
    *out = Entry{i, host + (size_t)i * entry_bytes, dev + (size_t)i * entry_bytes};
    return hipEventSynchronize(ev[i]);
  }
  hipError_t release(const Entry& en, hipStream_t st) { return hipEventRecord(ev[en.i], st); }
  void destroy() {
    for (hipEvent_t e : ev)
      if (e) (void)hipEventSynchronize(e);
    (void)hipFree(dev);
    (void)hipHostFree(host);
    for (hipEvent_t& e : ev)
      if (e) (void)hipEventDestroy(e);
  }
};

struct Blob {
  const float* p;
  int ndim;
  int64_t shape[4];
  size_t numel() const {
    size_t n = 1;
    for (int i = 0; i < ndim; ++i) n *= (size_t)shape[i];
    return n;
  }
};

template <typename Acc>
inline std::vector<float> pack_b(int K, int N, Acc w) {
  const int n_tiles = (N + 31) / 32, G = K / 8;
  std::vector<float> out((size_t)n_tiles * G * 256, 0.f);
  for (int nt = 0; nt < n_tiles; ++nt)
    for (int g = 0; g < G; ++g)
      for (int l = 0; l < 64; ++l) {
        int n = nt * 32 + (l & 31);
        if (n >= N) continue;
        float* dst = &out[(((size_t)nt * G + g) * 64 + l) * 4];
        for (int j = 0; j < 4; ++j) dst[j] = w(8 * g + 4 * (l >> 5) + j, n);
      }
  return out;
}

template <typename Acc>
inline std::vector<float> pack_conv2_quad(int d, Acc w) {
  static const int taps[4][2] = {{0, -1}, {1, -1}, {0, 2}, {2, -1}};
  return pack_b(32 * 128, d, [&](int k, int n) {
    const int h = k / 2048, slab = (k / 128) & 15, c = h * 128 + (k & 127);
    const int* th = taps[slab >> 2];
    const int* tw = taps[slab & 3];
    double v = 0.0;
    for (int a = 0; a < 2 && th[a] >= 0; ++a)
      for (int e = 0; e < 2 && tw[e] >= 0; ++e) v += (double)w((th[a] * 3 + tw[e]) * d + c, n);
    return (float)v;
  });
}

typedef std::unordered_map<std::string, Blob> BlobMap;

struct DeviceAllocs {
  std::vector<void*> allocs;
  ppasr_status alloc(size_t bytes, void** out) {
    HIP_TRY(hipMalloc(out, bytes));
    allocs.push_back(*out);
    return PPASR_OK;
  }
  ppasr_status upload_bytes(const void* src, size_t bytes, const void** out) {
    void* d = nullptr;
    ppasr_status s = alloc(bytes, &d);
    if (s != PPASR_OK) return s;
    HIP_TRY(hipMemcpy(d, src, bytes, hipMemcpyHostToDevice));
    *out = d;
    return PPASR_OK;
  }
  ~DeviceAllocs() {
    for (void* p : allocs) (void)hipFree(p);
  }
};

inline unsigned eff_stride_mask(const ppasr_model_desc& d) {
  if (d.model_type != PPASR_MODEL_EFFICIENT_CONFORMER) return 0u;
  if (d.stride_layer_mask != 0) return (unsigned)d.stride_layer_mask;
  return d.stride_layer_idx >= 0 ? (1u << d.stride_layer_idx) : 0u;
}
inline int eff_strides_before(const ppasr_model_desc& d, int layer) {
  return __builtin_popcount(eff_stride_mask(d) & ((1u << layer) - 1u));
}

struct ppasr_model_s : DeviceAllocs {
  ppasr_model_desc desc;
  int F1, F2;
  const f32x4* gen_head_w = nullptr;
  const float* gen_head_b = nullptr;
  int gen_vpad = 0;
  int F3 = 0;
  struct Front {
    int T1, T2, Tp;
  };
  int sub_rate() const { return desc.input_layer == 1 ? 1 : desc.input_layer ? desc.input_layer : 4; }
  int F_last() const { return desc.input_layer == 8 ? F3 : F2; }
  int min_frames() const { return desc.input_layer == 1 ? 1 : desc.input_layer == 6 ? 11 : desc.input_layer == 8 ? 15 : 7; }
  Front front_dims(int T) const {
    if (desc.input_layer == 1) return Front{0, 0, T};
    Front f{(T - 1) / 2, 0, 0};
    if (desc.input_layer == 6) {
      f.Tp = (f.T1 - 5) / 3 + 1;
    } else if (desc.input_layer == 8) {
      f.T2 = (f.T1 - 1) / 2;
      f.Tp = (f.T2 - 1) / 2;
    } else {
      f.Tp = (f.T1 - 1) / 2;
    }
    return f;
  }
  bool generic = false;
  struct GenOpts {
    int pos = 0;
    bool post_norm = false, concat_after = false, macaron = true, use_cnn = true;
    int act = 0;
    bool sq_pre_norm = false;
  } gen;
  struct GenLayerX {
    const f32x4* wcat = nullptr;
    const float* bcat = nullptr;
  };
  std::vector<GenLayerX> gen_x;
  const float* pe_dev = nullptr;
  const float* zero_vec = nullptr;
  const float *lin_ln_g = nullptr, *lin_ln_b = nullptr;
  int lin_kpad = 0;
  FrontW front;
  std::vector<LayerW> layers;
  std::vector<int> layer_ks;
  std::vector<int> layer_group;
  HeadW head;
  std::vector<SqLayerW> sq_layers;
  SqReduceW sq_reduce{};
  const f32x4* sq_wrec = nullptr;
  const float* sq_brec = nullptr;
  const float *preln_g = nullptr, *preln_b = nullptr;
  Ds2W ds2{};
  int ds2_persist_hold = 0, ds2_persist_giveups = 0;
  std::vector<Ds2LayerW> ds2_layers;
  float* taps = nullptr;
  size_t taps_floats = 0;
  bool prof = false;
  int front_fused = -1;
  int ffn_split = -1;
  bool skip_padding = false;
  int gemm_mode = 0;
  std::vector<LayerW> layers_h3;
  const f32x4* conv2_w_h3 = nullptr;
  const f32x4* embed_w_h3 = nullptr;
  const f32x4* head_w_h3 = nullptr;
  std::vector<SqLayerW> sq_layers_h3;
  int gemm_coverage = 0;
  bool gemm_guard = true;
  static constexpr int kGuardN = 5;
  unsigned int* guard_ctr[kGuardN] = {};
  unsigned int* guard_dev = nullptr;
  unsigned int* guard_host = nullptr;
  unsigned int guard_seen[kGuardN] = {};
  long long guard_fallbacks = 0, guard_events = 0;
  int row_block = -1;
  std::vector<int64_t> lens_hint;
  std::vector<hipEvent_t> ev_pool;
  size_t ev_used = 0;
  struct Span { int cls; std::vector<std::pair<hipEvent_t, hipEvent_t>> ev; };
  std::vector<Span> spans;

  ppasr_status upload(const std::vector<float>& v, const float** out) {
    return upload_bytes(v.data(), v.size() * sizeof(float), reinterpret_cast<const void**>(out));
  }
  ppasr_status upload4(const std::vector<float>& v, const f32x4** out) {
    return upload_bytes(v.data(), v.size() * sizeof(float), reinterpret_cast<const void**>(out));
  }
  hipEvent_t next_event() {
    if (ev_used == ev_pool.size()) {
      hipEvent_t e;
      (void)hipEventCreate(&e);
      ev_pool.push_back(e);
    }
    return ev_pool[ev_used++];
  }
  ~ppasr_model_s() {
    for (hipEvent_t e : ev_pool) (void)hipEventDestroy(e);
    if (guard_host) (void)hipHostFree(guard_host);
  }
};


struct ppasr_stream_s {
  ppasr_model_s* m;
  int D;
  int cap;
  int cache_t;
  int cache_r;
  int offset;
  int lo;
  float *kc, *vc;
  float* xh_hist;
  float* g_hist;
  HistLayer* hist_tab;
};

struct ChunkPlan {
  int c;
  int c_r;
  int used_r;
  int T2, T2_r;
  int ncs;
  int pos0;
};

struct WsLayout {
  size_t y1, y2, xa, xb, xc, qkv, ctx, g, rmax, rsum, fa, fp, xs, vt, total;
  int vt_stride;
};
WsLayout ws_layout(const ppasr_model_s* m, int B, int T);
int ffn_split_for(const ppasr_model_s* m, int M);
int wide_slices_for(const ppasr_model_s* m, int M, int units);
int row_block_for(const ppasr_model_s* m, int B, int Tcur, int mul, int slack, bool skip);
bool block_tables_enabled();
bool conv12_enabled(const ppasr_model_s* m);
ppasr::LayerW sq_conv_view(const ppasr::SqLayerW& W);

size_t generic_ws_floats(const ppasr_model_s* m, int B, int T);
ppasr_status generic_encode(ppasr_model_s* h, const float* feats, const int64_t* lens, int B, int T, float* probs,
                            float* logits, int32_t* frame_argmax, float* frame_maxprob, float* ws, hipStream_t st);
ppasr_status generic_chunk(ppasr_stream_s* s, const ChunkPlan& p, const float* feats, int T, float* probs,
                           int32_t* frame_argmax, float* frame_maxprob, float* ws, hipStream_t st, int* frames_out);
ppasr_status generic_sq_chunk(ppasr_stream_s* s, const ChunkPlan& p, const float* feats, int T, float* probs,
                              int32_t* frame_argmax, float* frame_maxprob, float* ws, hipStream_t st);
size_t generic_group_ws_floats(const ppasr_model_s* m, int n, int T);
ppasr_status generic_group_chunk(ppasr_model_s* h, const SessDesc* sess, int n, float* kc, float* vc, int cap,
                                 float* xh_hist, int lo, const float* feats, int T, float* probs, int32_t* frame_argmax,
                                 float* frame_maxprob, float* ws, hipStream_t st);
hipError_t configure_generic_kernels();
ppasr_status generic_sq_encode(ppasr_model_s* h, const float* feats, const int64_t* lens, int B, int T, float* probs,
                               float* logits, int32_t* frame_argmax, float* frame_maxprob, float* ws, hipStream_t st);

struct Loader;
ppasr_status conformer_create(ppasr_model_s* m, Loader& ld);
ppasr_status ds2_create(ppasr_model_s* m, Loader& ld);
size_t ds2_group_ws_floats(const ppasr_model_s* m, int n, int T);
ppasr_status ds2_group_round(ppasr_model_s* h, const int* slots, int n, const float* feats, int T, float* state_h,
                             float* state_c, float* probs, int32_t* frame_argmax, float* frame_maxprob, float* ws,
                             hipStream_t st);
ppasr_status squeezeformer_create(ppasr_model_s* m, Loader& ld);
ppasr_status squeezeformer_encode(ppasr_model_s* h, const float* feats, const int64_t* lens, int B, int T, float* probs,
                                  float* logits, int32_t* frame_argmax, float* frame_maxprob, float* ws,
                                  const WsLayout& wl, hipStream_t st);

#include "weights.h"
```

ppasr_amd/csrc/conformer_kernels.h:

```cpp
#pragma once
#include <hip/hip_runtime.h>
#include <stdint.h>

#include "rowblock.h"

namespace ppasr {

struct LayerW {
  const float *ln_mac_g, *ln_mac_b, *ln_mha_g, *ln_mha_b, *ln_conv_g, *ln_conv_b;
  const float *ln_ff_g, *ln_ff_b, *ln_fin_g, *ln_fin_b, *ln_cm_g, *ln_cm_b;
  float cm_eps;
  const f32x4 *ffm_w1, *ffm_w2, *ff_w1, *ff_w2, *wqkv, *wo, *pw1, *pw2;
  const float *ffm_b1, *ffm_b2, *ff_b1, *ff_b2, *bqkv, *bo, *pw1_b, *pw2_b;
  const float *dw_w;
  const float *dw_b;
  const float *glu_pad;
  const float *pos_u, *pos_v;
  const float *ptab;
  const float *dtab = nullptr;
};

struct FrontW {
  const float *cmvn_mean, *cmvn_istd;
  const float *conv1_w, *conv1_b;
  const f32x4 *conv2_w;
  const f32x4 *conv2_wp = nullptr;
  const float *conv2_b;
  int conv2_k = 3, conv2_s = 2;
  const f32x4 *conv3_w = nullptr;
  const float *conv3_b = nullptr;
  const f32x4 *embed_w;
  const float *embed_b;
};

struct HeadW {
  const float *ln_g, *ln_b;
  const f32x4 *w;
  const float *b;
  int V, n_tiles;
};

struct SessDesc {
  int sess;
  int cache_t;
  int pos0;
  int offset;
};

struct AttnArgs {
  const float* q;
  int q_stride;
  const float* k;
  int k_stride;
  const float* v;
  int v_stride;
  int T1, T2;
  int pos0;
  const int64_t* lens;
  float* ctx;
  const float *pos_u, *pos_v;
  const float* ptab;
  int pos_stride;
  int mask_mul;
  int q_frames, kv_frames;
  int group;
  const SessDesc* sess;
  long long sess_stride;
  int pad_skip;
  const float* vt = nullptr;
  int vt_stride = 0;
  int dm = 256;
  const float* dtab = nullptr;
  int dtab_len = 0;
};
struct VtOut {
  float* vt = nullptr;
  int stride = 0;
  int k_h3 = 0;
  const float* kpos = nullptr;
  int kpos_stride = 0;
  int Ti = 1;
};

constexpr size_t kLdsExclusive = 82 * 1024;
size_t ragged_lds(size_t lds, const PadSkip& ps, int n_blocks);

bool launch_attention_t(const AttnArgs& a, int B, int H, hipStream_t st);
hipError_t configure_attention_kernels();

void launch_block_table(const PadSkip& ps, int M, int R, int* tab, hipStream_t st);

bool conv2_quad_supported(const FrontW& fw);
bool conv12_supported(const FrontW& fw, int F, int F2);
void launch_conv12(const float* feats, const FrontW& fw, float* y2, int B, int T, int F, int Tp, int F2, hipStream_t st,
                   const PadSkip& ps_frames, int* tile_scratch);
void launch_conv2_quad(const float* y1, const FrontW& fw, float* y2, int B, int T1, int F1, int Tp, int F2, hipStream_t st,
                       const PadSkip& ps_frames, int* tile_scratch);
hipError_t configure_front_fused_kernels();

void launch_out_glu_split_16(const float* ctx, const float* x1, float* x2, float* g, float* xhat, const LayerW& w,
                             const int64_t* lens, int M, int Tp, int mask_mul, hipStream_t st, const PadSkip& ps,
                             float* hist = nullptr, int lo = 0);
void launch_shift_caches(float* kc, float* vc, long long layer_stride, int D, int n_layers, int from_full, int keep_full,
                         int from_half, int keep_half, unsigned long long half_mask, hipStream_t st);
void launch_oproj_ln_16(const float* ctx, const float* x1, float* x2_sink, float* xhat_out, const LayerW& w, int M,
                        hipStream_t st, const PadSkip& ps = PadSkip{});
void launch_pw1_glu_cols_16(const float* x, float* g, const LayerW& w, int M, hipStream_t st, float* hist = nullptr, int lo = 0,
                            const float* hist_scale = nullptr, const float* hist_bias = nullptr, const PadSkip& ps = PadSkip{},
                            const int64_t* lens = nullptr, int Tp = 1, int mask_mul = 1);
bool conv_ffn_16_supported(int ksize, int Tp);
hipError_t configure_conformer_t_kernels();

template <int R>
struct LayerStagesT {
  static hipError_t configure();
  static void ffn_qkv(const float* x_in, float* x1, float* qkv, const LayerW& w, int M, int n_chunks, hipStream_t st,
                      const PadSkip& ps, VtOut vt);
  static void out_glu(const float* ctx, const float* x1, float* x2, float* g, const LayerW& w, const int64_t* lens, int M,
                      int Tp, int mask_mul, hipStream_t st, const PadSkip& ps, float* xhat_out = nullptr,
                      int stop_after_ln = 0);
  static void conv_ffn(const float* g, const float* x2, float* x_out, const LayerW& w, const int64_t* lens, int M, int Tp,
                       int n_chunks, int ksize, int mask_mul, const LayerW* next, float* x1_next, float* qkv_next,
                       hipStream_t st, bool causal, const PadSkip& ps, VtOut vt_next);
};

void launch_posproj(const float* pe, const float* wpos , const float* bpos_or_null, float* ptab,
                    int max_len, hipStream_t st, int d = 256);
void launch_pos_dtab(const float* ptab, const float* pos_u, const float* pos_v, float* dtab, int max_len, hipStream_t st);
void launch_conv1(const float* feats, const FrontW& fw, float* y1, int B, int T, int F, int T1, int F1, hipStream_t st,
                  const PadSkip& ps = PadSkip{}, int channels = 256);
void launch_conv_stage(const float* y_in, const f32x4* w, const float* bias, float* y_out, int B, int T_in, int F_in,
                       int T_out, int F_out, int k, int s, hipStream_t st, const PadSkip& ps_frames = PadSkip{},
                       int channels = 256, int* tile_scratch = nullptr,
                       bool h3 = false,
                       float* part = nullptr, size_t part_floats = 0);
size_t conv_stage_part_floats(int M, int channels = 256);
size_t conv_stage_part_reserve(int M);
void launch_conv2(const float* y1, const FrontW& fw, float* y2, int B, int T1, int F1, int Tp, int F2, hipStream_t st,
                  const PadSkip& ps = PadSkip{}, int* tile_scratch = nullptr, const f32x4* w_h3 = nullptr, float* part = nullptr,
                  size_t part_floats = 0);
void launch_embed(const float* y2, const FrontW& fw, float* x0, int M, int K, float xscale, bool scale_before_bias,
                  hipStream_t st, const PadSkip& ps = PadSkip{}, int k_slices = 1, float* part = nullptr,
                  const f32x4* w_h3 = nullptr);
void launch_dense(const float* a, int lda, const f32x4* w, const float* bias, float* out, int M, int K, int n_cols_padded,
                  int ldc, int n_valid, hipStream_t st, float scale = 1.0f, float* part = nullptr, size_t part_floats = 0);
void launch_ffn_qkv(const float* x_in, float* x1, float* qkv, const LayerW& w, int M, int n_chunks, hipStream_t st,
                    const PadSkip& ps = PadSkip{}, VtOut vt = VtOut{}, bool h3 = false, int rows = 32);
void launch_repack_h3(const f32x4* src, f32x4* dst, int n_tiles, int G, unsigned int* ovf, hipStream_t st);
inline bool conv_ffn_h3_supported(int ksize) { return ksize == 15 || ksize == 7; }
void launch_split_rows_h3(const float* src, float* dst, long long n_rows, unsigned int* ovf, hipStream_t st);
unsigned int* conformer_h3_ovf_counter();
unsigned int* front_h3_ovf_counter();
unsigned int* ctc_head_h3_ovf_counter();
unsigned int* split_route_h3_ovf_counter();
hipError_t configure_front_kernels();
hipError_t configure_stream_kernels();
hipError_t configure_split_route_kernels();
hipError_t configure_ctc_head_kernels();
void launch_attention(const AttnArgs& a, int B, int H, hipStream_t st);
struct HistMove {
  float* hist;
  int lo;
  bool done;
};
void launch_out_glu(const float* ctx, const float* x1, float* x2, float* g, float* xhat_out, const LayerW& w,
                    const int64_t* lens, int M, int Tp, int mask_mul, hipStream_t st, const PadSkip& ps = PadSkip{},
                    float* split_xhat = nullptr,
                    bool h3 = false,
                    HistMove* hm = nullptr, int rows = 32);
void launch_conv_ffn(const float* g, const float* g_hist, const float* x2, float* x_out, const LayerW& w,
                     const int64_t* lens, int M, int Tp, int n_chunks, int ksize, int mask_mul, const LayerW* next,
                     float* x1_next, float* qkv_next, hipStream_t st, bool causal = true, const PadSkip& ps = PadSkip{},
                     VtOut vt_next = VtOut{}, bool h3 = false, int rows = 32);
void launch_conv_pre(const float* g, const float* g_hist, const float* x2, float* x3, const LayerW& w, const int64_t* lens,
                     int M, int Tp, int ksize, int mask_mul, hipStream_t st, bool causal = true,
                     const PadSkip& ps = PadSkip{}, bool h3 = false);
void launch_ffn_split(const float* x, const float* ln_g, const float* ln_b, const f32x4* w1, const float* b1,
                      const f32x4* w2, const float* b2, float scale, const float* out_ln_g, const float* out_ln_b,
                      float* partial, float* out, int M, int n_chunks, int S, hipStream_t st, const PadSkip& ps = PadSkip{},
                      bool residual_is_normed = false, bool h3 = false);
struct JoinIn {
  const float* partial = nullptr;
  int S = 0;
  const float* b2 = nullptr;
  float scale = 0.f;
  const float* x = nullptr;
  const float *ln_g = nullptr, *ln_b = nullptr;
  float* out = nullptr;
};
constexpr int kSplitRows16Max = 512;
bool ffn_half16_route(int M, int S, int n_chunks);
void launch_ffn_half16(const float* x, const JoinIn& jn, const float* ln_g, const float* ln_b, const f32x4* w1, const float* b1,
                       const f32x4* w2, float* partial, int M, int n_chunks, hipStream_t st);
void launch_join_ln_qkv16(const JoinIn& jn, float* qkv, const LayerW& w, int M, hipStream_t st, float* kc, float* vc);
void launch_join16(const JoinIn& jn, int M, hipStream_t st);
void launch_ln_qkv(const float* x1, float* qkv, const LayerW& w, int M, hipStream_t st, const PadSkip& ps = PadSkip{},
                   float* kc = nullptr, float* vc = nullptr, bool h3 = false);
void launch_conv_ffn_stride(const float* g, const float* g_hist, const float* x2, float* x_out, const LayerW& w, const int64_t* lens, int B,
                            int Tp, int Ts, int n_chunks, int ksize, int mask_mul_out, hipStream_t st,
                            const PadSkip& ps = PadSkip{}, bool causal = true, bool h3 = false,
                            float* x3_out = nullptr);
void launch_attn_out_glu(const AttnArgs& a, int B, const float* x1, float* x2, float* g, const LayerW& w, hipStream_t st,
                         bool h3 = false);
void launch_pw1_glu(const float* xhat, float* g, const LayerW& w, int M, hipStream_t st);
struct HistLayer {
  const f32x4* pw1;
  const float* pw1_b;
  int rows, pad;
};
void launch_pw1_glu_layers(const float* xh_hist, float* g_hist, const HistLayer* tab, int n_layers, int lo_stride,
                           hipStream_t st);
void launch_kv_append(const float* qkv, float* kc, float* vc, int n_rows, hipStream_t st);
void launch_pw1_glu_layers_group(const float* xh_hist, long long sess_stride, const SessDesc* sess, float* g_hist,
                                 const HistLayer* tab, int n_layers, int n, int lo, hipStream_t st);
void launch_kv_append_group(const float* qkv, float* kc, float* vc, long long sess_stride, const SessDesc* sess, int n, int c,
                            hipStream_t st);
void launch_hist_gather(const float* hist, long long sess_stride, const SessDesc* sess, float* dst, int n, int lo,
                        hipStream_t st);
void launch_hist_update_group(float* hist, long long sess_stride, const SessDesc* sess, const float* fresh, int n, int c,
                              int lo, hipStream_t st);
void launch_hist_update(float* hist, const float* fresh, int n, int lo, hipStream_t st);
void launch_cache_export(const float* kc, const float* vc, float* att, int T, int div, hipStream_t st, int D = 256);
void launch_cache_import(const float* att, float* kc, float* vc, int T, int div, hipStream_t st, int D = 256);
void launch_cnn_transpose(const float* src, float* dst, int lo, int lo_ref, int to_ref, hipStream_t st, int D = 256);
void launch_ctc_head(const float* x, const HeadW& hw, float* logits, int32_t* fr_argmax, float* fr_maxprob,
                     float* row_max, float* row_sum, int M, hipStream_t st, const PadSkip& ps = PadSkip{},
                     int n_slices = 1, float* part = nullptr, bool h3 = false);
void launch_softmax_from_stats(float* probs_inout, const float* row_max, const float* row_sum, int M, int V,
                               hipStream_t st, const PadSkip& ps = PadSkip{});
void launch_frame_argmax(const float* probs, int32_t* fr_argmax, float* fr_maxprob, int M, int V, hipStream_t st);
void launch_ctc_collapse(const int32_t* fr_argmax, const float* fr_maxprob, const int32_t* frame_lens, int B, int Tp,
                         int blank, int32_t* tokens, int32_t* n_tokens, double* score, hipStream_t st);
void launch_zero_pad_rows(float* probs, float* logits, int32_t* fr_argmax, float* fr_maxprob, const int64_t* lens, int B,
                          int Tp, int mul, int V, hipStream_t st);
hipError_t configure_kernels();

}
```

ppasr_amd/csrc/conformer_kernels.hip:

```cpp
#include <cstdlib>

#include "conformer_kernels.h"
#include "launch.h"
#include "phases.h"
#include "h3.h"

#include <math.h>

namespace ppasr {
#ifdef PPASR_PHASE_TS
}
extern "C" __attribute__((visibility("default"))) int ppasr_debug_read_phase_ts(long long* out) {
  return (int)hipMemcpyFromSymbol(out, HIP_SYMBOL(ppasr::g_phase_ts), sizeof(long long) * 128);
}
extern "C" __attribute__((visibility("default"))) int ppasr_debug_read_wave_ts(long long* out) {
  return (int)hipMemcpyFromSymbol(out, HIP_SYMBOL(ppasr::g_wave_ts), sizeof(long long) * 512);
}
extern "C" __attribute__((visibility("default"))) int ppasr_debug_read_wg_ts(long long* out) {
  return (int)hipMemcpyFromSymbol(out, HIP_SYMBOL(ppasr::g_wg_ts), sizeof(long long) * 2 * 1024);
}
namespace ppasr {
#endif


// ... 724 lines not shown
      rb_gemm<1, 1, kG256, kPF, NoSide, true>(bufA, kLda, seg_gate, 0, nullptr, 0, ring, ag);
    }
#pragma unroll
    for (int q = 0; q < 4; ++q) {
      const f32x4 bval = *reinterpret_cast<const f32x4*>(w.pw1_b + cq + 8 * q);
      const f32x4 bgate = *reinterpret_cast<const f32x4*>(w.pw1_b + kD + cq + 8 * q);
      const f32x2 s0 = sigmoid2(f32x2{ag[0][0][4 * q] + bgate[0], ag[0][0][4 * q + 1] + bgate[1]});
      const f32x2 s1 = sigmoid2(f32x2{ag[0][0][4 * q + 2] + bgate[2], ag[0][0][4 * q + 3] + bgate[3]});
      const f32x4 o = {(av[0][0][4 * q] + bval[0]) * s0[0], (av[0][0][4 * q + 1] + bval[1]) * s0[1],
                       (av[0][0][4 * q + 2] + bval[2]) * s1[0], (av[0][0][4 * q + 3] + bval[3]) * s1[1]};
      if (row_ok) *reinterpret_cast<f32x4*>(g + grow + cq + 8 * q) = o;
    }
    if constexpr (H3) {
      if (row_ok) {
#pragma unroll
        for (int q = 0; q < 4; ++q) *reinterpret_cast<f32x4*>(x2 + grow + cq + 8 * q) = x2v[q];
      }
    }
  }
  PPASR_TS(39);
  PPASR_WG_TS(512 + 1);
}
__global__ __launch_bounds__(kThreads) void k_attn_out_glu(AttnArgs a, int B, const float* __restrict__ x1,
                                                           float* __restrict__ x2, float* __restrict__ g, LayerW w) {
  attn_out_glu_body<false>(a, B, x1, x2, g, w);
}
__global__ __launch_bounds__(kThreads) void k_attn_out_glu_h3(AttnArgs a, int B, const float* __restrict__ x1,
                                                              float* __restrict__ x2, float* __restrict__ g, LayerW w) {
  attn_out_glu_body<true>(a, B, x1, x2, g, w);
}
constexpr size_t kLdsAttnOutGlu = (size_t)kFusedAttnFloats * sizeof(float);
void launch_attn_out_glu(const AttnArgs& a, int B, const float* x1, float* x2, float* g, const LayerW& w, hipStream_t st, bool h3) {
  const int nq = (a.T1 + 31) / 32;
  if (h3)
    PPASR_LAUNCH(k_attn_out_glu_h3, dim3(nq * ((B + 7) / 8) * 8), dim3(kThreads), kLdsAttnOutGlu + 512, st, a, B, x1, x2, g, w);
  else
    PPASR_LAUNCH(k_attn_out_glu, dim3(nq * ((B + 7) / 8) * 8), dim3(kThreads), kLdsAttnOutGlu, st, a, B, x1, x2, g, w);
}

template <int KS, bool STREAM, bool NEXT, bool H3>
__device__ __forceinline__ void conv_ffn_body(const float* __restrict__ g, const float* __restrict__ g_hist,
                                              const float* __restrict__ x2, float* __restrict__ x_out, const LayerW& w,
                                              const int64_t* __restrict__ lens, int M, int Tp, int n_chunks, int mask_mul,
                                              const LayerW& wn, float* __restrict__ x1_next, float* __restrict__ qkv_next,
                                              int left_ctx, const PadSkip& ps, VtOut vt_next) {
  extern __shared__ __attribute__((aligned(16))) float smem[];
  const int blk = pad_block_of(ps, kRows, M);
  if (blk < 0) return;
  float* bufX = smem;
  float* bufA = bufX + kRows * kLda;
  float* bufH = bufA + kRows * kLda;
  const int lane = lane_id(), wave = wave_id();
  const int r0 = blk * kRows;
  const int valid = min(kRows, M - r0);
  const int col = wave * 32 + (lane & 31);
  BRing<1> ring;
  const f32x4* seg_pw2 = w.pw2 + (size_t)wave * kTs256;
  PPASR_TS(0);
  if (NEXT) PPASR_WG_TS(0);
  ring_prime(ring, seg_pw2, 0);
  const int pb0 = r0 / Tp, pt0 = r0 - pb0 * Tp, pnb = max(M / Tp, 1);
  int64_t plen0 = 0, plen1 = 0;
  if (lens && Tp >= kRows) {
    plen0 = lens[min(pb0, pnb - 1)];
    plen1 = lens[min(pb0 + 1, pnb - 1)];
  }
  if (!STREAM && KS <= 15 && Tp >= kRows / kWaves) {
    if constexpr (!STREAM && KS <= 15)
      dwconv_ln_phase<KS>(g, bufA, w.dw_w, w.dw_b, w.glu_pad, w.ln_cm_g, w.ln_cm_b, w.cm_eps, r0, M, Tp, left_ctx);
    PPASR_TS(1);
  } else {
    dwconv_phase<KS, STREAM>(g, g_hist, bufA, bufH, bufX, w.dw_w, w.dw_b, w.glu_pad, r0, M, Tp, left_ctx);
    __syncthreads();
    PPASR_TS(1);
    rb_layernorm<true>(bufA, bufA, kLda, kRows, w.ln_cm_g, w.ln_cm_b, w.cm_eps);
  }
  PadRows is_pad{lens, r0, Tp, M, mask_mul};
  const int l31 = lane & 31, cq = wave * 32 + 4 * (lane >> 5);
  f32x4 res[4];
  {
    const float* rp = x2 + (size_t)(r0 + min(l31, valid - 1)) * kD + cq;
#pragma unroll
    for (int q = 0; q < 4; ++q) res[q] = *reinterpret_cast<const f32x4*>(rp + 8 * q);
  }
  bool pad = false;
  if (lens) {
    if (Tp >= kRows) {
      const int tt = pt0 + l31;
      const bool over = tt >= Tp;
      const int64_t t = over ? tt - Tp : tt, len = over ? plen1 : plen0;
      pad = r0 + l31 < M && (int64_t)mask_mul * t >= len;
    } else {
      pad = is_pad(l31);
    }
  }
  __syncthreads();
  PPASR_TS(2);
  {
    f32x16 acc[1][1];
    acc_zero(acc);
    if constexpr (H3) {
      h3_planes_from_tile(bufA, reinterpret_cast<_Float16*>(bufA));
      rb_gemm_h3(reinterpret_cast<const _Float16*>(bufA), seg_pw2, w.ff_w1 + (size_t)wave * kTs256, ring, acc[0][0]);
      acc[0][0] *= kH3Inv;
    } else {
      rb_gemm<1, 1, kG256, kPF, NoSide, true>(bufA, kLda, seg_pw2, 0, w.ff_w1 + (size_t)wave * kTs256, 0, ring, acc);
    }
#pragma unroll
    for (int q = 0; q < 4; ++q) {
      const f32x4 bv = *reinterpret_cast<const f32x4*>(w.pw2_b + cq + 8 * q);
      f32x4 o;
#pragma unroll
      for (int e = 0; e < 4; ++e) o[e] = (l31 < valid) ? res[q][e] + (pad ? 0.f : acc[0][0][4 * q + e] + bv[e]) : 0.f;
      *reinterpret_cast<f32x4*>(bufX + l31 * kLda + cq + 8 * q) = o;
    }
  }
  __syncthreads();
  PPASR_TS(3);
  rb_layernorm(bufX, bufA, kLda, kRows, w.ln_ff_g, w.ln_ff_b, 1e-5f);
  __syncthreads();
  PPASR_TS(4);
  f32x16 acc2[1][1];
  acc_zero(acc2);
  if constexpr (H3)
    ffn_phase_h3(bufA, w.ff_w1, w.ff_b1, w.ff_w2, n_chunks, NEXT ? wn.ffm_w1 + (size_t)wave * kTs256 : nullptr, ring, acc2);
  else
    ffn_phase<true>(bufA, bufH, w.ff_w1, w.ff_b1, w.ff_w2, n_chunks, NEXT ? wn.ffm_w1 + (size_t)wave * kTs256 : nullptr,
                    ring, acc2);
  PPASR_TS(5);
  residual_epilogue_t(bufX, acc2, w.ff_b2, 0.5f);
  __syncthreads();
  PPASR_TS(6);
  rb_layernorm(bufX, bufX, kLda, kRows, w.ln_fin_g, w.ln_fin_b, 1e-5f);
  if (x_out) rb_store_rows(x_out + (size_t)r0 * kD, bufX, kLda, kRows, valid);
  PPASR_TS(7);
  if (NEXT) ffn_qkv_body<H3>(bufX, bufA, bufH, x1_next, qkv_next, wn, r0, valid, n_chunks, ring, vt_next);
  PPASR_TS(15);
  if (NEXT) PPASR_WG_TS(1);
}
template <int KS, bool STREAM, bool NEXT>
__global__ __launch_bounds__(kThreads) void k_conv_ffn(const float* __restrict__ g, const float* __restrict__ g_hist,
                                                       const float* __restrict__ x2, float* __restrict__ x_out, LayerW w,
                                                       const int64_t* __restrict__ lens, int M, int Tp, int n_chunks,
                                                       int mask_mul, LayerW wn, float* __restrict__ x1_next,
                                                       float* __restrict__ qkv_next, int left_ctx, PadSkip ps, VtOut vt_next) {
  conv_ffn_body<KS, STREAM, NEXT, false>(g, g_hist, x2, x_out, w, lens, M, Tp, n_chunks, mask_mul, wn, x1_next, qkv_next,
                                         left_ctx, ps, vt_next);
}
template <int KS, bool NEXT>
__global__ __launch_bounds__(kThreads) void k_conv_ffn_h3(const float* __restrict__ g, const float* __restrict__ x2,
                                                          float* __restrict__ x_out, LayerW w, const int64_t* __restrict__ lens,
                                                          int M, int Tp, int n_chunks, int mask_mul, LayerW wn,
                                                          float* __restrict__ x1_next, float* __restrict__ qkv_next,
                                                          int left_ctx, PadSkip ps, VtOut vt_next) {
  conv_ffn_body<KS, false, NEXT, true>(g, nullptr, x2, x_out, w, lens, M, Tp, n_chunks, mask_mul, wn, x1_next, qkv_next,
                                       left_ctx, ps, vt_next);
}
constexpr size_t kLdsConvFfn = 4 * kRows * kLda * sizeof(float);
void launch_conv_ffn(const float* g, const float* g_hist, const float* x2, float* x_out, const LayerW& w,
                     const int64_t* lens, int M, int Tp, int n_chunks, int ksize, int mask_mul, const LayerW* next,
                     float* x1_next, float* qkv_next, hipStream_t st, bool causal, const PadSkip& ps, VtOut vt_next, bool h3,
                     int rows) {
  check_form("launch_conv_ffn", rows, h3 || g_hist);
  if (rows == 16)
    return LayerStagesT<16>::conv_ffn(g, x2, x_out, w, lens, M, Tp, n_chunks, ksize, mask_mul, next, x1_next, qkv_next, st,
                                      causal, ps, VtOut{});
  if (rows == kW16)
    return LayerStagesT<kW16>::conv_ffn(g, x2, x_out, w, lens, M, Tp, n_chunks, ksize, mask_mul, next, x1_next, qkv_next, st,
                                        causal, ps, vt_next);
  dim3 grid((M + kRows - 1) / kRows);
  const int left_ctx = causal ? ksize - 1 : (ksize - 1) / 2;
  const LayerW& wn = next ? *next : w;
  if (h3) {
#define LAUNCH_CF_H3(KS, NX)                                                                                                 \
  PPASR_LAUNCH((k_conv_ffn_h3<KS, NX>), grid, dim3(kThreads), kLdsConvFfn + kH3ExtraLds, st, g, x2, x_out, w, lens, M, Tp, \
               n_chunks, mask_mul, wn, x1_next, qkv_next, left_ctx, ps, vt_next)
    if (ksize == 15 && next) LAUNCH_CF_H3(15, true);
    else if (ksize == 15) LAUNCH_CF_H3(15, false);
    else if (next) LAUNCH_CF_H3(7, true);
    else LAUNCH_CF_H3(7, false);
#undef LAUNCH_CF_H3
    return;
  }
#define LAUNCH_CF(KS)                                                                                                  \
  if (g_hist)                                                                                                          \
    PPASR_LAUNCH((k_conv_ffn<KS, true, false>), grid, dim3(kThreads), kLdsConvFfn, st, g, g_hist, x2, x_out, w,  \
                       lens, M, Tp, n_chunks, mask_mul, wn, x1_next, qkv_next, left_ctx, ps, vt_next);                                    \
  else if (next)                                                                                                       \
    PPASR_LAUNCH((k_conv_ffn<KS, false, true>), grid, dim3(kThreads), kLdsConvFfn, st, g, g_hist, x2, x_out, w,  \
                       lens, M, Tp, n_chunks, mask_mul, wn, x1_next, qkv_next, left_ctx, ps, vt_next);                                    \
  else                                                                                                                 \
    PPASR_LAUNCH((k_conv_ffn<KS, false, false>), grid, dim3(kThreads), kLdsConvFfn, st, g, g_hist, x2, x_out, w, \
                       lens, M, Tp, n_chunks, mask_mul, wn, x1_next, qkv_next, left_ctx, ps, vt_next);
  if (ksize == 15) {
    LAUNCH_CF(15)
  } else if (ksize == 31) {
    LAUNCH_CF(31)
  } else if (ksize == 7) {
    LAUNCH_CF(7)
  }
#undef LAUNCH_CF
}

template <int KS, bool H3>
__global__ __launch_bounds__(kThreads) void k_conv_ffn_stride(const float* __restrict__ g, const float* __restrict__ g_hist,
                                                              const float* __restrict__ x2, float* __restrict__ x_out,
                                                              LayerW w,
                                                              const int64_t* __restrict__ lens, int B, int Tp, int Ts,
                                                              int n_chunks, int mask_mul_out, PadSkip ps, int causal,
                                                              float* __restrict__ x3_out) {
  extern __shared__ __attribute__((aligned(16))) float smem[];
  if (pad_block_skippable(ps, blockIdx.x * kRows, kRows, B * Ts)) return;
  float* bufX = smem;
  float* bufA = bufX + kRows * kLda;
  float* bufH = bufA + kRows * kLda;
  const int lane = lane_id(), wave = wave_id();
  const int Mo = B * Ts;
  const int r0 = blockIdx.x * kRows;
  const int valid = min(kRows, Mo - r0);
  const int col = wave * 32 + (lane & 31);
  constexpr int LO = KS - 1;
  BRing<1> ring;
  const f32x4* seg_pw2 = w.pw2 + (size_t)wave * kTs256;
  ring_prime(ring, seg_pw2, 0);
  {
    const f32x4 gp = *reinterpret_cast<const f32x4*>(w.glu_pad + 4 * lane);
    const f32x4 bias = *reinterpret_cast<const f32x4*>(w.dw_b + 4 * lane);
    for (int row = wave; row < kRows; row += kWaves) {
      f32x4 out = bias;
      if (row < valid) {
        const int mo = r0 + row, b = mo / Ts, j = mo - b * Ts;
        const float* gb = g + (size_t)b * Tp * kD + 4 * lane;
#pragma unroll
        for (int t = 0; t < KS; ++t) {
          const int f = 2 * j - (causal ? LO : LO / 2) + t;
          const f32x4 wj = *reinterpret_cast<const f32x4*>(w.dw_w + t * kD + 4 * lane);
          f32x4 v = causal ? gp : f32x4{0.f, 0.f, 0.f, 0.f};
          if (f >= 0 && f < Tp) v = *reinterpret_cast<const f32x4*>(gb + (size_t)f * kD);
          else if (f < 0 && g_hist) v = *reinterpret_cast<const f32x4*>(g_hist + ((size_t)b * LO + LO + f) * kD + 4 * lane);
          out += wj * v;
        }
      }
      *reinterpret_cast<f32x4*>(bufA + row * kLda + 4 * lane) = out;
    }
  }
  __syncthreads();
  rb_layernorm<true>(bufA, bufA, kLda, kRows, w.ln_cm_g, w.ln_cm_b, w.cm_eps);
  __syncthreads();
  PadRows is_pad{lens, r0, Ts, Mo, mask_mul_out};
  {
    f32x16 acc[1][1];
    acc_zero(acc);
    if constexpr (H3) unit_std_h3(bufA, seg_pw2, w.ff_w1 + (size_t)wave * kTs256, ring, acc);
    else rb_gemm<1, 1, kG256>(bufA, kLda, seg_pw2, 0, w.ff_w1 + (size_t)wave * kTs256, 0, ring, acc);
    const float bv = w.pw2_b[col];
#pragma unroll
    for (int r = 0; r < 16; ++r) {
      int row = acc_row(r, lane);
      float v = 0.f;
      if (row < valid) {
        const int mo = r0 + row, b = mo / Ts, j = mo - b * Ts;
        const float* xb = x2 + ((size_t)b * Tp + 2 * j) * kD + col;
        float res = xb[0];
        if (2 * j + 1 < Tp) res = (res + xb[kD]) * 0.5f;
        float c = is_pad(row) ? 0.f : acc[0][0][r] + bv;
        v = res + c;
      }
      bufX[row * kLda + col] = v;
    }
  }
  __syncthreads();
  if (x3_out) {
    rb_store_rows(x3_out + (size_t)r0 * kD, bufX, kLda, kRows, valid);
    return;
  }
  rb_layernorm(bufX, bufA, kLda, kRows, w.ln_ff_g, w.ln_ff_b, 1e-5f);
  __syncthreads();
  f32x16 acc2[1][1];
  acc_zero(acc2);
  if constexpr (H3) {
    ffn_phase_h3(bufA, w.ff_w1, w.ff_b1, w.ff_w2, n_chunks, nullptr, ring, acc2);
    residual_epilogue_t(bufX, acc2, w.ff_b2, 0.5f);
  } else {
    ffn_phase(bufA, bufH, w.ff_w1, w.ff_b1, w.ff_w2, n_chunks, nullptr, ring, acc2);
    residual_epilogue(bufX, acc2, w.ff_b2, 0.5f);
  }
  __syncthreads();
  rb_layernorm(bufX, bufX, kLda, kRows, w.ln_fin_g, w.ln_fin_b, 1e-5f);
  rb_store_rows(x_out + (size_t)r0 * kD, bufX, kLda, kRows, valid);
}
void launch_conv_ffn_stride(const float* g, const float* g_hist, const float* x2, float* x_out, const LayerW& w,
                            const int64_t* lens, int B, int Tp, int Ts, int n_chunks, int ksize, int mask_mul_out,
                            hipStream_t st, const PadSkip& ps, bool causal, bool h3, float* x3_out) {
  dim3 grid((B * Ts + kRows - 1) / kRows);
  (void)ksize;
  if (h3)
    PPASR_LAUNCH((k_conv_ffn_stride<15, true>), grid, dim3(kThreads), kLdsConvFfn + kH3ExtraLds, st, g, g_hist, x2, x_out, w, lens,
                 B, Tp, Ts, n_chunks, mask_mul_out, ps, causal ? 1 : 0, x3_out);
  else
    PPASR_LAUNCH((k_conv_ffn_stride<15, false>), grid, dim3(kThreads), kLdsConvFfn, st, g, g_hist, x2, x_out, w, lens, B, Tp, Ts,
                 n_chunks, mask_mul_out, ps, causal ? 1 : 0, x3_out);
}

hipError_t configure_kernels() {
  hipError_t e = configure_attention_kernels();
  if (e != hipSuccess) return e;
  e = configure_conformer_t_kernels();
  if (e != hipSuccess) return e;
  e = configure_front_fused_kernels();
  if (e != hipSuccess) return e;
  e = configure_front_kernels();
  if (e != hipSuccess) return e;
  e = configure_stream_kernels();
  if (e != hipSuccess) return e;
  e = configure_split_route_kernels();
  if (e != hipSuccess) return e;
  e = configure_ctc_head_kernels();
  if (e != hipSuccess) return e;
#define SET_LDS(fn, bytes)                                                                                     \
  e = hipFuncSetAttribute(reinterpret_cast<const void*>(fn), hipFuncAttributeMaxDynamicSharedMemorySize, (int)(bytes)); \
  if (e != hipSuccess) return e;
  SET_LDS(k_ffn_qkv, kLdsFfnQkv);
  SET_LDS(k_ffn_qkv_h3, kLdsFfnQkv + kH3ExtraLds);
  SET_LDS((k_conv_ffn_h3<15, true>), kLdsConvFfn + kH3ExtraLds);
  SET_LDS((k_conv_ffn_h3<15, false>), kLdsConvFfn + kH3ExtraLds);
  SET_LDS((k_conv_ffn_h3<7, true>), kLdsConvFfn + kH3ExtraLds);
  SET_LDS((k_conv_ffn_h3<7, false>), kLdsConvFfn + kH3ExtraLds);
  SET_LDS(k_out_glu<false>, kLdsOutGlu);
  SET_LDS(k_out_glu<true>, kLdsOutGlu + 512);
  SET_LDS(k_pw1_glu_cols<false>, kLdsPw1Cols);
  SET_LDS(k_pw1_glu_cols<true>, kLdsPw1Cols + 512);
  SET_LDS((k_conv_ffn<15, false, false>), kLdsConvFfn);
  SET_LDS((k_conv_ffn<31, false, false>), kLdsConvFfn);
  SET_LDS((k_conv_ffn<7, false, false>), kLdsConvFfn);
  SET_LDS((k_conv_ffn<15, false, true>), kLdsConvFfn);
  SET_LDS((k_conv_ffn<31, false, true>), kLdsConvFfn);
  SET_LDS((k_conv_ffn<7, false, true>), kLdsConvFfn);
  SET_LDS((k_conv_ffn<15, true, false>), kLdsConvFfn);
  SET_LDS((k_conv_ffn<31, true, false>), kLdsConvFfn);
  SET_LDS((k_conv_ffn<7, true, false>), kLdsConvFfn);
  SET_LDS(k_attn_out_glu, kLdsAttnOutGlu);
  SET_LDS(k_attn_out_glu_h3, kLdsAttnOutGlu + 512);
  SET_LDS((k_conv_ffn_stride<15, false>), kLdsConvFfn);
  SET_LDS((k_conv_ffn_stride<15, true>), kLdsConvFfn + kH3ExtraLds);
#undef SET_LDS
  return hipSuccess;
}

}
```

ppasr_amd/csrc/ctc_head_kernels.hip:

```cpp
#include <cstdlib>

#include "conformer_kernels.h"
#include "launch.h"
#include "phases.h"
#include "h3.h"

#include <math.h>

namespace ppasr {

template <bool LOGITS, bool H3>
__device__ __forceinline__ void ctc_head_body(const float* __restrict__ x, const HeadW& hw, float* __restrict__ logits,
                                              int32_t* __restrict__ fr_argmax, float* __restrict__ fr_maxprob,
                                              float* __restrict__ row_max, float* __restrict__ row_sum, int M, const PadSkip& ps,
                                              float* __restrict__ part) {
  extern __shared__ __attribute__((aligned(16))) float smem[];
  const int blk = pad_block_of(ps, kRows, M);
  if (blk < 0) return;
  const int ny = gridDim.y, y = blockIdx.y;
  float* bufA = smem;
  float* redM = bufA + (H3 ? kH3TileBytes / 4 : kRows * kLda);
  float* redS = redM + kWaves * 32;
  int* redI = reinterpret_cast<int*>(redS + kWaves * 32);
  const int lane = lane_id(), wave = wave_id();
  const int r0 = blk * kRows;
  const int valid = min(kRows, M - r0);
  const int V = hw.V;
  BRing<1> ring;
  if (wave + 8 * y < hw.n_tiles) ring_prime(ring, hw.w + (size_t)(wave + 8 * y) * kTs256, 0);
  rb_load_rows(bufA, kLda, x + (size_t)r0 * kD, kRows, valid);
  if (hw.ln_g) rb_layernorm(bufA, bufA, kLda, kRows, hw.ln_g, hw.ln_b, 1e-5f);
  __syncthreads();
  if constexpr (H3) h3_planes_from_tile(bufA, reinterpret_cast<_Float16*>(bufA));
  float mx = -INFINITY, sm = 0.f;
  int ix = 0x7fffffff;
  const int l31 = lane & 31, hh = lane >> 5;
  constexpr float kLog2e = 1.4426950408889634f;
  const int tstep = kWaves * ny;
  for (int tile = wave + 8 * y; tile < hw.n_tiles; tile += tstep) {
    f32x16 acc[1][1];
    acc_zero(acc);
    const f32x4* seg = hw.w + (size_t)tile * kTs256;
    if constexpr (H3) {
      rb_gemm_h3(reinterpret_cast<const _Float16*>(bufA), seg, tile + tstep < hw.n_tiles ? seg + (size_t)tstep * kTs256 : nullptr,
                 ring, acc[0][0]);
      acc[0][0] *= kH3Inv;
    } else {
      rb_gemm<1, 1, kG256, kPF, NoSide, true>(bufA, kLda, seg, 0, tile + tstep < hw.n_tiles ? seg + (size_t)tstep * kTs256 : nullptr,
                                              0, ring, acc);
    }
    const int c0 = tile * 32 + 4 * hh;
    float v[16];
#pragma unroll
    for (int q = 0; q < 4; ++q) {
      const f32x4 bq = *reinterpret_cast<const f32x4*>(hw.b + c0 + 8 * q);
#pragma unroll
      for (int e = 0; e < 4; ++e) v[4 * q + e] = acc[0][0][4 * q + e] + bq[e];
    }
    if (tile == hw.n_tiles - 1 && (V & 31)) {
#pragma unroll
      for (int r = 0; r < 16; ++r)
        if (c0 + 8 * (r >> 2) + (r & 3) >= V) v[r] = -INFINITY;
    }
    if (LOGITS) {
      if (l31 < valid) {
        float* lrow = logits + (size_t)(r0 + l31) * V;
#pragma unroll
        for (int r = 0; r < 16; ++r) {
          const int col = c0 + 8 * (r >> 2) + (r & 3);
          if (col < V) lrow[col] = v[r];
        }
      }
    }
    float tmax = max3f(v[0], v[1], v[2]);
#pragma unroll
    for (int r = 3; r < 15; r += 2) tmax = max3f(tmax, v[r], v[r + 1]);
    tmax = fmaxf(tmax, v[15]);
    if (tmax > mx) {
#pragma unroll
      for (int r = 15; r >= 0; --r) ix = (v[r] == tmax) ? c0 + 8 * (r >> 2) + (r & 3) : ix;
    }
    const float mn = fmaxf(mx, tmax);
    sm *= __builtin_amdgcn_exp2f((mx - mn) * kLog2e);
    f32x2 ps = {0.f, 0.f};
#pragma unroll
    for (int r = 0; r < 16; r += 2) {
      const f32x2 t = (f32x2{v[r], v[r + 1]} - f32x2{mn, mn}) * f32x2{kLog2e, kLog2e};
      ps += f32x2{__builtin_amdgcn_exp2f(t[0]), __builtin_amdgcn_exp2f(t[1])};
    }
    sm += ps[0] + ps[1];
    mx = mn;
  }
  {
    const float m2 = __shfl_xor(mx, 32), s2 = __shfl_xor(sm, 32);
    const int i2 = __shfl_xor(ix, 32);
    const float mn = fmaxf(mx, m2);
    const float sa = (mx == -INFINITY) ? 0.f : sm * __expf(mx - mn);
    const float sb = (m2 == -INFINITY) ? 0.f : s2 * __expf(m2 - mn);
    const bool take2 = (m2 > mx) || (m2 == mx && i2 < ix);
    if (hh == 0) {
      redM[wave * 32 + l31] = mn;
      redS[wave * 32 + l31] = sa + sb;
      redI[wave * 32 + l31] = take2 ? i2 : ix;
    }
  }
  __syncthreads();
  if (threadIdx.x < 32) {
    const int row = threadIdx.x;
    float m = redM[row], s = redS[row];
    int i = redI[row];
    for (int wv = 1; wv < kWaves; ++wv) {
      float m2 = redM[wv * 32 + row], s2 = redS[wv * 32 + row];
      int i2 = redI[wv * 32 + row];
      float mn = fmaxf(m, m2);
      float sa = (m == -INFINITY) ? 0.f : s * __expf(m - mn);
      float sb = (m2 == -INFINITY) ? 0.f : s2 * __expf(m2 - mn);
      bool take2 = (m2 > m) || (m2 == m && i2 < i);
      i = take2 ? i2 : i;
      m = mn;
      s = sa + sb;
    }
    if (row < valid) {
      if (ny > 1) {
        part[(size_t)y * M + r0 + row] = m;
        part[((size_t)ny + y) * M + r0 + row] = s;
        reinterpret_cast<int*>(part)[((size_t)2 * ny + y) * M + r0 + row] = i;
      } else {
        if (fr_argmax) fr_argmax[r0 + row] = i;
        if (fr_maxprob) fr_maxprob[r0 + row] = 1.0f / s;
        if (row_max) row_max[r0 + row] = m;
        if (row_sum) row_sum[r0 + row] = s;
      }
    }
  }
}
__global__ void k_ctc_merge(const float* __restrict__ part, int ny, int32_t* __restrict__ fr_argmax,
                            float* __restrict__ fr_maxprob, float* __restrict__ row_max, float* __restrict__ row_sum, int M,
                            PadSkip ps) {
  const int row = blockIdx.x * blockDim.x + threadIdx.x;
  if (row >= M) return;
  if (pad_block_skippable(ps, row & ~(kRows - 1), kRows, M)) return;
  float m = part[row], s = part[(size_t)ny * M + row];
  int i = reinterpret_cast<const int*>(part)[(size_t)2 * ny * M + row];
  for (int y = 1; y < ny; ++y) {
    const float m2 = part[(size_t)y * M + row], s2 = part[((size_t)ny + y) * M + row];
    const int i2 = reinterpret_cast<const int*>(part)[((size_t)2 * ny + y) * M + row];
    const float mn = fmaxf(m, m2);
    const float sa = (m == -INFINITY) ? 0.f : s * __expf(m - mn);
    const float sb = (m2 == -INFINITY) ? 0.f : s2 * __expf(m2 - mn);
    const bool take2 = (m2 > m) || (m2 == m && i2 < i);
    i = take2 ? i2 : i;
    m = mn;
    s = sa + sb;
  }
  if (fr_argmax) fr_argmax[row] = i;
  if (fr_maxprob) fr_maxprob[row] = 1.0f / s;
  if (row_max) row_max[row] = m;
  if (row_sum) row_sum[row] = s;
}
template <bool LOGITS>
__global__ __launch_bounds__(kThreads) void k_ctc_head(const float* __restrict__ x, HeadW hw, float* __restrict__ logits,
                                                       int32_t* __restrict__ fr_argmax, float* __restrict__ fr_maxprob,
                                                       float* __restrict__ row_max, float* __restrict__ row_sum, int M,
                                                       PadSkip ps, float* __restrict__ part) {
  ctc_head_body<LOGITS, false>(x, hw, logits, fr_argmax, fr_maxprob, row_max, row_sum, M, ps, part);
}
template <bool LOGITS>
__global__ __launch_bounds__(kThreads) void k_ctc_head_h3(const float* __restrict__ x, HeadW hw, float* __restrict__ logits,
                                                          int32_t* __restrict__ fr_argmax, float* __restrict__ fr_maxprob,
                                                          float* __restrict__ row_max, float* __restrict__ row_sum, int M,
                                                          PadSkip ps, float* __restrict__ part) {
  ctc_head_body<LOGITS, true>(x, hw, logits, fr_argmax, fr_maxprob, row_max, row_sum, M, ps, part);
}
constexpr size_t kLdsCtc = (kRows * kLda + 3 * kWaves * 32) * sizeof(float);
void launch_ctc_head(const float* x, const HeadW& hw, float* logits, int32_t* fr_argmax, float* fr_maxprob, float* row_max,
                     float* row_sum, int M, hipStream_t st, const PadSkip& ps, int n_slices, float* part, bool h3) {
  const int ny = (n_slices > 1 && part) ? n_slices : 1;
  dim3 grid((M + kRows - 1) / kRows, ny);
  const size_t lds = ragged_lds(kLdsCtc + (h3 ? 512 : 0), ps, (int)(grid.x * grid.y));
  if (h3 && logits)
    PPASR_LAUNCH(k_ctc_head_h3<true>, grid, dim3(kThreads), lds, st, x, hw, logits, fr_argmax, fr_maxprob, row_max, row_sum, M, ps,
                 part);
  else if (h3)
    PPASR_LAUNCH(k_ctc_head_h3<false>, grid, dim3(kThreads), lds, st, x, hw, logits, fr_argmax, fr_maxprob, row_max, row_sum, M, ps,
                 part);
  else if (logits)
    PPASR_LAUNCH(k_ctc_head<true>, grid, dim3(kThreads), lds, st, x, hw, logits, fr_argmax, fr_maxprob, row_max,
                       row_sum, M, ps, part);
  else
    PPASR_LAUNCH(k_ctc_head<false>, grid, dim3(kThreads), lds, st, x, hw, logits, fr_argmax, fr_maxprob, row_max,
                       row_sum, M, ps, part);
  if (ny > 1)
    PPASR_LAUNCH(k_ctc_merge, dim3((M + 255) / 256), dim3(256), 0, st, part, ny, fr_argmax, fr_maxprob, row_max, row_sum,
                       M, ps);
}

template <int NV>
__global__ __launch_bounds__(256) void k_softmax_row_wg(float* __restrict__ p, int M, int V, PadSkip ps) {
  const int row = blockIdx.x;
  if (pad_block_skippable(ps, row & ~(kRows - 1), kRows, M)) return;
  __shared__ float red[8];
  const int tid = threadIdx.x, lane = lane_id(), wave = wave_id();
  float* x = p + (size_t)row * V;
  constexpr int NR = NV > 0 ? NV : 1;
  float v[NR];
  float m = -INFINITY;
  if (NV > 0) {
#pragma unroll
    for (int i = 0; i < NR; ++i) {
      const int c = tid + 256 * i;
      v[i] = c < V ? x[c] : -INFINITY;
      m = fmaxf(m, v[i]);
    }
  } else {
    for (int c = tid; c < V; c += 256) m = fmaxf(m, x[c]);
  }
  m = wave_max(m);
  if (lane == 0) red[wave] = m;
  __syncthreads();
  m = fmaxf(fmaxf(red[0], red[1]), fmaxf(red[2], red[3]));
  float s = 0.f;
  if (NV > 0) {
#pragma unroll
    for (int i = 0; i < NR; ++i) {
      v[i] = expf(v[i] - m);
      s += v[i];
    }
  } else {
    for (int c = tid; c < V; c += 256) {
      const float e = expf(x[c] - m);
      x[c] = e;
      s += e;
    }
  }
  s = wave_sum(s);
  if (lane == 0) red[4 + wave] = s;
  __syncthreads();
  s = (red[4] + red[5]) + (red[6] + red[7]);
  if (NV > 0) {
#pragma unroll
    for (int i = 0; i < NR; ++i) {
      const int c = tid + 256 * i;
      if (c < V) x[c] = v[i] / s;
    }
  } else {
    for (int c = tid; c < V; c += 256) x[c] = x[c] / s;
  }
}
void launch_softmax_from_stats(float* probs_inout, const float*, const float*, int M, int V, hipStream_t st,
                               const PadSkip& ps) {
  if (V <= 256 * 8) PPASR_LAUNCH(k_softmax_row_wg<8>, dim3(M), dim3(256), 0, st, probs_inout, M, V, ps);
  else if (V <= 256 * 20) PPASR_LAUNCH(k_softmax_row_wg<20>, dim3(M), dim3(256), 0, st, probs_inout, M, V, ps);
  else PPASR_LAUNCH(k_softmax_row_wg<0>, dim3(M), dim3(256), 0, st, probs_inout, M, V, ps);
}

__global__ __launch_bounds__(256) void k_zero_pad_rows(float* __restrict__ probs, float* __restrict__ logits,
                                                       int32_t* __restrict__ fa, float* __restrict__ fp,
                                                       const int64_t* __restrict__ lens, int M, int Tp, int mul, int V) {
  const int row = blockIdx.x * 4 + wave_id();
  if (row >= M) return;
  const int b = row / Tp, t = row - b * Tp;
  if ((int64_t)mul * t < lens[b]) return;
  const int lane = lane_id();
  if (probs)
    for (int c = lane; c < V; c += 64) probs[(size_t)row * V + c] = 0.f;
  if (logits)
    for (int c = lane; c < V; c += 64) logits[(size_t)row * V + c] = 0.f;
  if (lane == 0) {
    if (fa) fa[row] = 0;
    if (fp) fp[row] = 0.f;
  }
}
void launch_zero_pad_rows(float* probs, float* logits, int32_t* fr_argmax, float* fr_maxprob, const int64_t* lens, int B,
                          int Tp, int mul, int V, hipStream_t st) {
  const int M = B * Tp;
  PPASR_LAUNCH(k_zero_pad_rows, dim3((M + 3) / 4), dim3(256), 0, st, probs, logits, fr_argmax, fr_maxprob, lens, M, Tp,
                     mul, V);
}

__global__ __launch_bounds__(256) void k_frame_argmax(const float* __restrict__ probs, int32_t* __restrict__ fr_argmax,
                                                      float* __restrict__ fr_maxprob, int M, int V) {
  const int row = blockIdx.x * 4 + wave_id();
  if (row >= M) return;
  const int lane = lane_id();
  const float* x = probs + (size_t)row * V;
  float m = -INFINITY;
  int idx = 0x7fffffff;
  for (int c = lane; c < V; c += 64) {
    float v = x[c];
    if (v > m || idx == 0x7fffffff) {
      m = v;
      idx = c;
    }
  }
#pragma unroll
  for (int o = 32; o > 0; o >>= 1) {
    float m2 = __shfl_xor(m, o);
    int i2 = __shfl_xor(idx, o);
    bool take2 = (i2 != 0x7fffffff) && (idx == 0x7fffffff || m2 > m || (m2 == m && i2 < idx));
    if (take2) {
      m = m2;
      idx = i2;
    }
  }
  if (lane == 0) {
    fr_argmax[row] = idx;
    fr_maxprob[row] = m;
  }
}
void launch_frame_argmax(const float* probs, int32_t* fr_argmax, float* fr_maxprob, int M, int V, hipStream_t st) {
  PPASR_LAUNCH(k_frame_argmax, dim3((M + 3) / 4), dim3(256), 0, st, probs, fr_argmax, fr_maxprob, M, V);
}

__global__ __launch_bounds__(64) void k_ctc_collapse(const int32_t* __restrict__ fr_argmax, const float* __restrict__ fr_maxprob,
                                                     const int32_t* __restrict__ frame_lens, int Tp, int blank,
                                                     int32_t* __restrict__ tokens, int32_t* __restrict__ n_tokens,
                                                     double* __restrict__ score) {
  const int b = blockIdx.x, lane = threadIdx.x;
  int n = frame_lens ? frame_lens[b] : Tp;
  n = max(0, min(n, Tp));
  const int32_t* ids = fr_argmax + (size_t)b * Tp;
  const float* pr = fr_maxprob + (size_t)b * Tp;
  int32_t* out = tokens + (size_t)b * Tp;
  int count = 0;
  int prev_last = -2;
  double dsum = 0.0;
  int nnb = 0;
  for (int base = 0; base < n; base += 64) {
    const int i = base + lane;
    const bool in = i < n;
    const int id = in ? ids[i] : -3;
    int prev = __shfl_up(id, 1);
    if (lane == 0) prev = prev_last;
    const bool nonblank = in && id != blank;
    const bool keep = nonblank && id != prev;
    if (nonblank) {
      dsum += (double)pr[i];
      nnb += 1;
    }
    unsigned long long mask = __ballot(keep);
    int pos = count + __popcll(mask & ((1ull << lane) - 1ull));
    if (keep) out[pos] = id;
    count += __popcll(mask);
    prev_last = __shfl(id, 63);
  }
#pragma unroll
  for (int o = 32; o > 0; o >>= 1) {
    dsum += __shfl_xor(dsum, o);
    nnb += __shfl_xor(nnb, o);
  }
  for (int i = count + lane; i < Tp; i += 64) out[i] = -1;
  if (lane == 0) {
    n_tokens[b] = count;
    score[b] = nnb > 0 ? (dsum / (double)nnb) * 100.0 : 0.0;
  }
}
void launch_ctc_collapse(const int32_t* fr_argmax, const float* fr_maxprob, const int32_t* frame_lens, int B, int Tp,
                         int blank, int32_t* tokens, int32_t* n_tokens, double* score, hipStream_t st) {
  PPASR_LAUNCH(k_ctc_collapse, dim3(B), dim3(64), 0, st, fr_argmax, fr_maxprob, frame_lens, Tp, blank, tokens,
                     n_tokens, score);
}
unsigned int* ctc_head_h3_ovf_counter() { return h3_ovf_counter(); }

hipError_t configure_ctc_head_kernels() {
  hipError_t e = hipSuccess;
#define SET_LDS(fn, bytes)                                                                                     \
  e = hipFuncSetAttribute(reinterpret_cast<const void*>(fn), hipFuncAttributeMaxDynamicSharedMemorySize, (int)(bytes)); \
  if (e != hipSuccess) return e;
  SET_LDS(k_ctc_head<true>, kLdsExclusive);
  SET_LDS(k_ctc_head_h3<true>, kLdsExclusive);
  SET_LDS(k_ctc_head_h3<false>, kLdsExclusive);
  SET_LDS(k_ctc_head<false>, kLdsExclusive);
#undef SET_LDS
  return hipSuccess;
}

}
```

ppasr_amd/csrc/phases.h:

```cpp
#pragma once
#include "conformer_kernels.h"
#include "rowblock.h"

namespace ppasr {

struct SwishSide {
  const f32x16& acc;
  float* dst;
  const f32x4 (&bias)[4];
  mutable f32x2 lo;
  __device__ __forceinline__ void operator()(int g) const {
    const int q = g >> 3;
    if ((g & 7) == 0) lo = swish2(f32x2{acc[4 * q] + bias[q][0], acc[4 * q + 1] + bias[q][1]});
    if ((g & 7) == 4) {
      const f32x2 hi = swish2(f32x2{acc[4 * q + 2] + bias[q][2], acc[4 * q + 3] + bias[q][3]});
      *reinterpret_cast<f32x4*>(dst + 8 * q) = f32x4{lo[0], lo[1], hi[0], hi[1]};
    }
  }
};

template <bool T2 = false>
__device__ __forceinline__ void ffn_phase(const float* bufA, float* bufH, const f32x4* __restrict__ w1,
                                          const float* __restrict__ b1, const f32x4* __restrict__ w2, int n_chunks,
                                          const f32x4* __restrict__ after, BRing<1>& ring, f32x16 (&acc2)[1][1],
                                          int c0 = 0, int n_total = -1) {
  const int lane = lane_id(), wave = wave_id();
  const int ts2 = (n_total > 0 ? n_total : n_chunks) * 32 * 64;
  b1 += c0 * 256;
  auto w1seg = [&](int c) { return w1 + (size_t)((c0 + c) * 8 + wave) * kTs256; };
  auto w2seg = [&](int c) { return w2 + (size_t)wave * ts2 + (size_t)(c0 + c) * 32 * 64; };
  f32x16 cur[1][1], nx[1][1];
  acc_zero(cur);
  rb_gemm<1, 1, kG256, kPF, NoSide, true>(bufA, kLda, w1seg(0), 0, n_chunks > 1 ? w1seg(1) : w2seg(0), 0, ring, cur);
  const int hoff = (lane & 31) * kLda + wave * 32 + 4 * (lane >> 5);
  for (int c = 0; c < n_chunks; ++c) {
    float* hb = bufH + (c & 1) * kRows * kLda;
    f32x4 bias[4];
#pragma unroll
    for (int q = 0; q < 4; ++q) bias[q] = *reinterpret_cast<const f32x4*>(b1 + c * 256 + wave * 32 + 8 * q + 4 * (lane >> 5));
    if (c + 1 < n_chunks) {
      acc_zero(nx);
      rb_gemm<1, 1, kG256, kPF, SwishSide, true>(bufA, kLda, w1seg(c + 1), 0, w2seg(c), 0, ring, nx,
                                                 SwishSide{cur[0][0], hb + hoff, bias, f32x2{0.f, 0.f}});
    } else {
#pragma unroll
      for (int q = 0; q < 4; ++q) {
        const f32x2 lo = swish2(f32x2{cur[0][0][4 * q] + bias[q][0], cur[0][0][4 * q + 1] + bias[q][1]});
        const f32x2 hi = swish2(f32x2{cur[0][0][4 * q + 2] + bias[q][2], cur[0][0][4 * q + 3] + bias[q][3]});
        *reinterpret_cast<f32x4*>(hb + hoff + 8 * q) = f32x4{lo[0], lo[1], hi[0], hi[1]};
      }
    }
    if (c < 8) PPASR_TS(16 + 2 * c);
    if (c < 8) PPASR_WAVE_TS(2 * c);
    __syncthreads();
    if (c < 8) PPASR_TS(17 + 2 * c);
    if (c < 8) PPASR_WAVE_TS(2 * c + 1);
    const f32x4* nseg = (c + 2 < n_chunks) ? w1seg(c + 2) : (c + 1 < n_chunks ? w2seg(c + 1) : after);
    rb_gemm<1, 1, kG256, kPF, NoSide, T2>(hb, kLda, w2seg(c), 0, nseg, 0, ring, acc2);
    cur[0][0] = nx[0][0];
  }
}

__device__ __forceinline__ void residual_epilogue(float* bufX, const f32x16 (&acc)[1][1], const float* __restrict__ bias,
                                                  float scale) {
  const int lane = lane_id(), wave = wave_id();
  const int col = wave * 32 + (lane & 31);
  const float bv = bias[col];
#pragma unroll
  for (int r = 0; r < 16; ++r) {
    float* p = bufX + acc_row(r, lane) * kLda + col;
    *p = *p + scale * (acc[0][0][r] + bv);
  }
}

__device__ __forceinline__ void residual_epilogue_t(float* bufX, const f32x16 (&acc)[1][1], const float* __restrict__ bias,
                                                    float scale) {
  const int lane = lane_id(), wave = wave_id();
  const int cq = wave * 32 + 4 * (lane >> 5);
  float* row = bufX + (lane & 31) * kLda + cq;
#pragma unroll
  for (int q = 0; q < 4; ++q) {
    const f32x4 bv = *reinterpret_cast<const f32x4*>(bias + cq + 8 * q);
    f32x4 x = *reinterpret_cast<const f32x4*>(row + 8 * q);
#pragma unroll
    for (int e = 0; e < 4; ++e) x[e] = x[e] + scale * (acc[0][0][4 * q + e] + bv[e]);
    *reinterpret_cast<f32x4*>(row + 8 * q) = x;
  }
}

struct PadRows {
  const int64_t* lens;
  int r0, Tp, M;
  int mul = 4;
  __device__ __forceinline__ bool operator()(int row) const {
    if (!lens) return false;
    int m = r0 + row;
    if (m >= M) return false;
    int b = m / Tp, t = m - b * Tp;
    return mul * (int64_t)t >= lens[b];
  }
};


template <int KS, bool STREAM>
__device__ __forceinline__ void dwconv_phase(const float* __restrict__ g, const float* __restrict__ g_hist, float* bufA,
                                             float* win_lds, float* w_lds, const float* __restrict__ dw_w,
                                             const float* __restrict__ dw_b, const float* __restrict__ glu_pad, int r0,
                                             int M, int Tp, int left = KS - 1) {
  const int lane = lane_id(), wave = wave_id();
  constexpr int LO = KS - 1;
  constexpr int RW = kRows / kWaves;
  const bool causal = (left == LO);
  for (int q = wave; q < LO + kRows; q += kWaves) {
    const int mq = r0 - left + q;
    f32x4 v = {0.f, 0.f, 0.f, 0.f};
    if (mq >= 0 && mq < M) v = *reinterpret_cast<const f32x4*>(g + (size_t)mq * kD + 4 * lane);
    *reinterpret_cast<f32x4*>(win_lds + q * kLda + 4 * lane) = v;
  }
  for (int j = wave; j < KS; j += kWaves)
    *reinterpret_cast<f32x4*>(w_lds + j * kLda + 4 * lane) = *reinterpret_cast<const f32x4*>(dw_w + j * kD + 4 * lane);
  f32x4 gp = *reinterpret_cast<const f32x4*>(glu_pad + 4 * lane);
  if (!causal) gp = f32x4{0.f, 0.f, 0.f, 0.f};
  const f32x4 bias = *reinterpret_cast<const f32x4*>(dw_b + 4 * lane);
  __syncthreads();
#pragma unroll
  for (int i = 0; i < RW; ++i) {
    const int row = wave * RW + i;
    const int m = r0 + row;
    const int b = m / Tp, t = m - b * Tp;
    const float* hist = STREAM ? g_hist + ((size_t)b * LO) * kD + 4 * lane : nullptr;
    f32x4 acc = bias;
#pragma unroll
    for (int j = 0; j < KS; ++j) {
      const f32x4 wj = *reinterpret_cast<const f32x4*>(w_lds + j * kLda + 4 * lane);
      f32x4 xv = *reinterpret_cast<const f32x4*>(win_lds + (row + j) * kLda + 4 * lane);
      const int tt = t - left + j;
      if (STREAM) {
        if (tt < 0 && m < M) xv = *reinterpret_cast<const f32x4*>(hist + (size_t)(LO + tt) * kD);
      } else if (!(tt >= 0 && tt < Tp)) {
        xv = gp;
      }
      acc += wj * xv;
    }
    *reinterpret_cast<f32x4*>(bufA + row * kLda + 4 * lane) = acc;
  }
}

template <int KS>
__device__ __forceinline__ void dwconv_ln_phase(const float* __restrict__ g, float* bufA, const float* __restrict__ dw_w,
                                                const float* __restrict__ dw_b, const float* __restrict__ glu_pad,
                                                const float* __restrict__ ln_g, const float* __restrict__ ln_b, float ln_eps, int r0,
                                                int M, int Tp, int left) {
  const int lane = lane_id(), wave = wave_id();
  constexpr int LO = KS - 1, RW = kRows / kWaves, NW = RW + LO;
  const bool causal = (left == LO);
  const int q0 = wave * RW;
  f32x4 x[NW];
#pragma unroll
  for (int q = 0; q < NW; ++q) {
    const int mq = r0 - left + q0 + q;
    const int mc = min(max(mq, 0), M - 1);
    const f32x4 v = *reinterpret_cast<const f32x4*>(g + (size_t)mc * kD + 4 * lane);
    x[q] = (mq >= 0 && mq < M) ? v : f32x4{0.f, 0.f, 0.f, 0.f};
  }
  f32x4 wt[KS];
#pragma unroll
  for (int j = 0; j < KS; ++j) wt[j] = *reinterpret_cast<const f32x4*>(dw_w + j * kD + 4 * lane);
  f32x4 gp = *reinterpret_cast<const f32x4*>(glu_pad + 4 * lane);
  if (!causal) gp = f32x4{0.f, 0.f, 0.f, 0.f};
  const f32x4 bias = *reinterpret_cast<const f32x4*>(dw_b + 4 * lane);
  const int m0 = r0 + q0;
  const int tq0 = m0 - (m0 / Tp) * Tp;
  const int npass = (tq0 + RW - 1 < Tp) ? 1 : 2;
  f32x4 out[RW];
#pragma unroll 1
  for (int p = 0; p < npass; ++p) {
    const int tqp = tq0 - p * Tp;
    f32x4 acc[RW];
#pragma unroll
    for (int i = 0; i < RW; ++i) acc[i] = bias;
#pragma unroll
    for (int q = 0; q < NW; ++q) {
      const int tt = tqp - left + q;
      const f32x4 xq = (tt >= 0 && tt < Tp) ? x[q] : gp;
#pragma unroll
      for (int i = 0; i < RW; ++i) {
        const int j = q - i;
        if (j >= 0 && j < KS) acc[i] += wt[j] * xq;
      }
    }
#pragma unroll
    for (int i = 0; i < RW; ++i)
      if (npass == 1 || (tqp + i >= 0 && tqp + i < Tp)) out[i] = acc[i];
  }
  const f32x4 gam = *reinterpret_cast<const f32x4*>(ln_g + 4 * lane);
  const f32x4 bet = *reinterpret_cast<const f32x4*>(ln_b + 4 * lane);
  ln_rows_inreg<true, RW>(out, gam, bet, ln_eps);
#pragma unroll
  for (int i = 0; i < RW; ++i) *reinterpret_cast<f32x4*>(bufA + (q0 + i) * kLda + 4 * lane) = out[i];
}

template <bool H3>
__device__ __forceinline__ f32x4 qkv_bias_quad(const float* __restrict__ bqkv, const VtOut& vt, int c, int m, int col) {
  if (c < 2) return *reinterpret_cast<const f32x4*>(bqkv + c * 256 + col);
  if constexpr (!H3) {
    if (vt.kpos) return *reinterpret_cast<const f32x4*>(vt.kpos + (size_t)(m - m / vt.Ti * vt.Ti) * vt.kpos_stride + col);
  }
  return f32x4{0.f, 0.f, 0.f, 0.f};
}
template <bool H3>
__device__ __forceinline__ void qkv_kpos_add(f32x4 (&bk)[4], const f32x4 (&kp)[4], const VtOut& vt) {
  if constexpr (!H3) {
    if (vt.kpos) {
#pragma unroll
      for (int q = 0; q < 4; ++q) bk[q] += kp[q];
    }
  }
}
constexpr int kDRow = 2048;
static_assert(4 * kDRow <= kRows * kLda, "the four heads' d rows fit in front of the merge tiles");
__device__ __forceinline__ void attn_stage_d(float* row, const float* __restrict__ dtab, int t128, int shift, int U, int pstride) {
  for (int u = t128; u < ((U + 63) & ~63); u += 128)
    row[u] = (dtab && u >= shift && u < U) ? dtab[(size_t)(u - shift) * pstride] : 0.f;
}
__device__ __forceinline__ void attn_score_init(f32x16 (&acc_s)[2], const float* dl, const float* __restrict__ dtab, int key0,
                                                int kv_end, int pstride) {
#pragma unroll
  for (int t = 0; t < 2; ++t)
#pragma unroll
    for (int i = 0; i < 4; ++i) {
      f32x4 dq;
      if (dl) {
        dq = *reinterpret_cast<const f32x4*>(dl + 32 * t + 8 * i);
      } else {
#pragma unroll
        for (int j = 0; j < 4; ++j)
          dq[j] = dtab ? dtab[(size_t)min(max(key0 + 32 * t + 8 * i + j, 0), kv_end - 1) * pstride] : 0.f;
      }
#pragma unroll
      for (int j = 0; j < 4; ++j) acc_s[t][4 * i + j] = dq[j];
    }
}

}
```

ppasr_amd/model_utils/conformer/model.py:

```python
import ctypes
import json
import math

import numpy as np
import torch

from ppasr_amd import _lib

__all__ = ["ConformerModel"]

_POS_CODES = {"rel_pos": 0, "abs_pos": 1, "no_pos": 2}
_ACT_CODES = {"swish": 0, "relu": 1, "gelu": 2, "tanh": 3, "hardtanh": 4, "relu6": 5, "leakyrelu": 6, "selu": 7, "elu": 8,
              "hardswish": 9, "hardshrink": 10}


def _pe_table(d_model, max_len):
    pe = torch.zeros(max_len, d_model, dtype=torch.float32)
    position = torch.arange(0, max_len, dtype=torch.float32).unsqueeze(1)
    div_term = torch.exp(torch.arange(0, d_model, 2, dtype=torch.float32) * -(math.log(10000.0) / d_model))
    pe[:, 0::2] = torch.sin(position * div_term)
    pe[:, 1::2] = torch.cos(position * div_term)
    return pe.numpy()


class ConformerModel:

    def __init__(self, input_dim, vocab_size, mean_istd_path=None, streaming=True, encoder_conf=None,
                 decoder_conf=None, ctc_weight=0.5, state_dict=None, device="cuda:0", **_ignored):
        if state_dict is None:
            raise ValueError("state_dict (Paddle-layout parameter dict) is required")
        if not torch.cuda.is_available():
            raise _lib.PPASRHipError("no HIP device visible: ppasr_amd has no CPU fallback")
        self.lib = _lib.load()
        self.device = torch.device(device)
        self.input_dim = input_dim
        self.vocab_size = vocab_size
        self.streaming = streaming
        conf = dict(encoder_conf or {})
        self.output_size = int(conf.get("output_size", 256))
        self.attention_heads = int(conf.get("attention_heads", 4))
        self.linear_units = int(conf.get("linear_units", 2048))
        self.num_blocks = int(conf.get("num_blocks", 6))
        self.cnn_module_kernel = int(conf.get("cnn_module_kernel", 15))
        self.max_len = int(conf.get("max_len", 5000))
        pos = conf.get("pos_enc_layer_type", "rel_pos")
        act = conf.get("activation_type", "swish")
        if pos not in _POS_CODES:
            raise ValueError("unknown pos_enc_layer: " + str(pos))
        if act not in _ACT_CODES:
            raise KeyError(act)
        self.options = (_POS_CODES[pos] | (0 if conf.get("normalize_before", True) else _lib.PPASR_OPT_POST_NORM)
                        | (_lib.PPASR_OPT_CONCAT_AFTER if conf.get("concat_after", False) else 0)
                        | (0 if conf.get("macaron_style", True) else _lib.PPASR_OPT_NO_MACARON)
                        | (0 if conf.get("use_cnn_module", True) else _lib.PPASR_OPT_NO_CNN)
                        | (_ACT_CODES[act] << _lib.PPASR_OPT_ACT_SHIFT))
        self.use_cnn_module = bool(conf.get("use_cnn_module", True))
        il = conf.get("input_layer", "conv2d")
        if il not in ("linear", "conv2d", "conv2d6", "conv2d8"):
            raise ValueError("unknown input_layer: " + str(il))
        self.input_layer = il
        self.subsampling_rate = {"linear": 1, "conv2d": 4, "conv2d6": 6, "conv2d8": 8}[il]
        norm = conf.get("cnn_module_norm", "layer_norm")
        if norm not in ("layer_norm", "batch_norm"):
            raise ValueError(f"encoder_conf.cnn_module_norm={norm!r}")
        has_stats = any(k.endswith("conv_module.norm._mean") for k in state_dict)
        if self.use_cnn_module and has_stats != (norm == "batch_norm"):
            raise ValueError(f"encoder_conf.cnn_module_norm={norm!r} but the checkpoint "
                             f"{'has' if has_stats else 'lacks'} conv_module.norm._mean / _variance")
        sd = dict(state_dict)
        if mean_istd_path is not None:
            with open(mean_istd_path, "r", encoding="utf-8") as f:
                js = json.load(f)
            sd["encoder.global_cmvn.mean"] = np.asarray(js["mean"], np.float32)
            sd["encoder.global_cmvn.istd"] = np.asarray(js["istd"], np.float32)
        sd["__pe_table__"] = _pe_table(self.output_size, self.max_len)
        keep = []
        blobs = (_lib.WeightBlob * len(sd))()
        for i, (name, arr) in enumerate(sd.items()):
            a = np.ascontiguousarray(arr, dtype=np.float32)
            if a.ndim > 4:
                raise ValueError(f"{name}: ndim > 4")
            keep.append(a)
            blobs[i].name = name.encode()
            blobs[i].data_host = a.ctypes.data
            blobs[i].ndim = a.ndim
            for j in range(a.ndim):
                blobs[i].shape[j] = a.shape[j]
        desc = _lib.ModelDesc(_lib.PPASR_MODEL_CONFORMER, input_dim, vocab_size, self.output_size,
                              self.attention_heads, self.linear_units, self.num_blocks, self.cnn_module_kernel,
                              1 if streaming else 0, self.max_len, -1, -1, -1, 0, 0, 0,
                              {"conv2d": 0, "linear": 1, "conv2d6": 6, "conv2d8": 8}[self.input_layer], self.options)
        handle = ctypes.c_void_p()
        with torch.cuda.device(self.device):
            _lib.check(self.lib.ppasr_create(ctypes.byref(desc), blobs, len(sd), ctypes.byref(handle)))
        self._h = handle
        self._ws = None
        self._taps = None

    def __del__(self):
        h = getattr(self, "_h", None)
        if h is not None and h.value:
            self.lib.ppasr_destroy(h)
            self._h = None

    def out_frames(self, T):
        return int(self.lib.ppasr_out_frames(self._h, int(T)))

    def _workspace(self, B, T):
        need = int(self.lib.ppasr_workspace_bytes(self._h, B, T))
        key = torch.cuda.current_stream(self.device).cuda_stream
        if not isinstance(self._ws, dict):
            self._ws = {}
        ws = self._ws.get(key)
        if ws is None or ws.numel() < need:
            ws = torch.empty(need, dtype=torch.uint8, device=self.device)
            self._ws[key] = ws
        return ws

    def _prep(self, speech, speech_lengths):
        speech = torch.as_tensor(speech, dtype=torch.float32).to(self.device).contiguous()
        lens = torch.as_tensor(speech_lengths, dtype=torch.int64).to(self.device).contiguous()
        assert speech.dim() == 3 and speech.shape[2] == self.input_dim and lens.shape[0] == speech.shape[0]
        return speech, lens

    def _encode(self, speech, lens, probs=None, logits=None, fa=None, fp=None):
        B, T, _ = speech.shape
        ws = self._workspace(B, T)
        ptr = lambda t: None if t is None else t.data_ptr()
        stream = torch.cuda.current_stream(self.device).cuda_stream
        _lib.check(self.lib.ppasr_encode(self._h, speech.data_ptr(), lens.data_ptr(), B, T, ptr(probs), ptr(logits),
                                         ptr(fa), ptr(fp), ws.data_ptr(), ws.numel(), stream))

    def get_encoder_out(self, speech, speech_lengths, return_logits=False):
        speech, lens = self._prep(speech, speech_lengths)
        B, T, _ = speech.shape
        Tp = self.out_frames(T)
        probs = torch.empty(B, Tp, self.vocab_size, dtype=torch.float32, device=self.device)
        logits = torch.empty_like(probs) if return_logits else None
        with torch.cuda.device(self.device):
            self._encode(speech, lens, probs=probs, logits=logits)
        return (probs, logits) if return_logits else probs

    def encode_greedy(self, speech, speech_lengths, trim_to_length=False, blank=0):
        speech, lens = self._prep(speech, speech_lengths)
        B, T, _ = speech.shape
        Tp = self.out_frames(T)
        fa = torch.empty(B, Tp, dtype=torch.int32, device=self.device)
        fp = torch.empty(B, Tp, dtype=torch.float32, device=self.device)
        tokens = torch.empty(B, Tp, dtype=torch.int32, device=self.device)
        n_tokens = torch.empty(B, dtype=torch.int32, device=self.device)
        score = torch.empty(B, dtype=torch.float64, device=self.device)
        frame_lens = None
        if trim_to_length:
            frame_lens = self.valid_out_frames(lens, T)
        with torch.cuda.device(self.device):
            self._encode(speech, lens, fa=fa, fp=fp)
            stream = torch.cuda.current_stream(self.device).cuda_stream
            _lib.check(self.lib.ppasr_ctc_collapse(fa.data_ptr(), fp.data_ptr(),
                                                   None if frame_lens is None else frame_lens.data_ptr(), B, Tp,
                                                   blank, tokens.data_ptr(), n_tokens.data_ptr(), score.data_ptr(),
                                                   stream))
        return tokens, n_tokens, score

    def valid_out_frames(self, speech_lengths, T):
        lens = torch.as_tensor(speech_lengths, dtype=torch.int64).to(self.device)
        mul = getattr(self, "subsampling_rate", 4) * (2 ** len(getattr(self, "_stride_layers", ())))
        return torch.clamp((lens + mul - 1) // mul, min=0, max=self.out_frames(int(T))).to(torch.int32)

    def set_skip_padding(self, enable=True):
        self.skip_padding = bool(enable)
        _lib.check(self.lib.ppasr_set_skip_padding(self._h, 1 if enable else 0))

    def set_ffn_split(self, mode=-1):
        _lib.check(self.lib.ppasr_set_ffn_split(self._h, int(mode)))

    def set_front_fused(self, mode=-1):
        _lib.check(self.lib.ppasr_set_front_fused(self._h, int(mode)))
        self.front_fused = int(mode)

    def set_gemm_mode(self, mode="f32"):
        modes = {"f32": _lib.PPASR_GEMM_F32, "f16x3": _lib.PPASR_GEMM_F16X3}
        if mode not in modes:
            raise ValueError(f"gemm mode {mode!r}: 'f32' or 'f16x3'")
        _lib.check(self.lib.ppasr_set_gemm_mode(self._h, modes[mode]))

    def gemm_coverage(self):
        bits = int(self.lib.ppasr_gemm_coverage(self._h))
        names = ((_lib.PPASR_GEMM_COVERS_LAYERS, "layers"), (_lib.PPASR_GEMM_COVERS_FRONT, "front"),
                 (_lib.PPASR_GEMM_COVERS_HEAD, "head"))
        return {n for b, n in names if bits & b}

    def set_gemm_guard(self, enable=True):
        _lib.check(self.lib.ppasr_set_gemm_guard(self._h, 1 if enable else 0))

    def gemm_guard_stats(self):
        f, e = ctypes.c_longlong(0), ctypes.c_longlong(0)
        _lib.check(self.lib.ppasr_gemm_guard_stats(self._h, ctypes.byref(f), ctypes.byref(e)))
        return int(f.value), int(e.value)

    def set_row_block(self, rows=-1):
        _lib.check(self.lib.ppasr_set_row_block(self._h, int(rows)))

    def set_lengths_hint(self, lengths=None):
        if lengths is None:
            _lib.check(self.lib.ppasr_set_lengths_hint(self._h, None, 0))
            return
        arr = (ctypes.c_int64 * len(lengths))(*[int(v) for v in lengths])
        _lib.check(self.lib.ppasr_set_lengths_hint(self._h, arr, len(lengths)))

    def set_debug_taps(self, n_floats):
        self._taps = torch.zeros(n_floats, dtype=torch.float32, device=self.device) if n_floats else None
        _lib.check(self.lib.ppasr_set_debug_taps(self._h, None if self._taps is None else self._taps.data_ptr(),
                                                 n_floats))
        return self._taps

    def profile_kernels(self, enable=True):
        _lib.check(self.lib.ppasr_profile_enable(self._h, 1 if enable else 0))

    def read_kernel_profile(self):
        ms = (ctypes.c_float * _lib.N_KERNEL_CLASSES)()
        n = (ctypes.c_int32 * _lib.N_KERNEL_CLASSES)()
        _lib.check(self.lib.ppasr_profile_read(self._h, ms, n))
        return {self.lib.ppasr_kernel_class_name(i).decode(): (float(ms[i]), int(n[i]))
                for i in range(_lib.N_KERNEL_CLASSES)}

    def new_stream(self):
        return ConformerStream(self)

    def get_encoder_out_chunk(self, speech, offset, required_cache_size, att_cache=None, cnn_cache=None):
        if getattr(self, "_scratch_stream", None) is None:
            self._scratch_stream = self.new_stream()
        s = self._scratch_stream
        s.load_caches(att_cache, cnn_cache, int(offset))
        probs = s.encode_chunk(speech, int(required_cache_size))
        att, cnn = s.export_caches()
        return probs, att, cnn


class ConformerStream:
    def __init__(self, model):
        self.model = model
        self.lib = model.lib
        self._s = ctypes.c_void_p()
        with torch.cuda.device(model.device):
            _lib.check(self.lib.ppasr_stream_create(model._h, ctypes.byref(self._s)))
        self._ws = None

    def __del__(self):
        s = getattr(self, "_s", None)
        if s is not None and s.value:
            self.lib.ppasr_stream_destroy(s)
            self._s = None

    @property
    def offset(self):
        return int(self.lib.ppasr_stream_offset(self._s))

    @property
    def cache_frames(self):
        return int(self.lib.ppasr_stream_cache_frames(self._s))

    def reset(self):
        m = self.model
        with torch.cuda.device(m.device):
            _lib.check(self.lib.ppasr_stream_reset(self._s, torch.cuda.current_stream(m.device).cuda_stream))

    def encode_chunk(self, speech, required_cache_size=-1, want_probs=True, want_frames=False):
        m = self.model
        x = torch.as_tensor(speech, dtype=torch.float32).to(m.device).contiguous()
        assert x.dim() == 3 and x.shape[0] == 1 and x.shape[2] == m.input_dim
        T = int(x.shape[1])
        c = m.out_frames(T)
        need = int(self.lib.ppasr_chunk_workspace_bytes(m._h, T))
        if self._ws is None or self._ws.numel() < need:
            self._ws = torch.empty(need, dtype=torch.uint8, device=m.device)
        probs = torch.empty(1, max(c, 0), m.vocab_size, dtype=torch.float32, device=m.device) if want_probs else None
        fa = torch.empty(1, max(c, 0), dtype=torch.int32, device=m.device) if want_frames else None
        fp = torch.empty(1, max(c, 0), dtype=torch.float32, device=m.device) if want_frames else None
        c_out = ctypes.c_int(0)
        ptr = lambda t: None if t is None else t.data_ptr()
        with torch.cuda.device(m.device):
            stream = torch.cuda.current_stream(m.device).cuda_stream
            _lib.check(self.lib.ppasr_encode_chunk(self._s, x.data_ptr(), T, int(required_cache_size), ptr(probs),
                                                   ptr(fa), ptr(fp), ctypes.byref(c_out), self._ws.data_ptr(),
                                                   self._ws.numel(), stream))
        if want_frames:
            return probs, fa, fp
        return probs

    def export_caches(self):
        m = self.model
        t = self.cache_frames
        att = torch.empty(m.num_blocks, m.attention_heads, t, 2 * (m.output_size // m.attention_heads),
                          dtype=torch.float32, device=m.device)
        if getattr(m, "use_cnn_module", True):
            cnn = torch.empty(m.num_blocks, 1, m.output_size, m.cnn_module_kernel - 1, dtype=torch.float32, device=m.device)
        else:
            cnn = torch.empty(m.num_blocks, 0, 0, 0, dtype=torch.float32, device=m.device)
        with torch.cuda.device(m.device):
            stream = torch.cuda.current_stream(m.device).cuda_stream
            _lib.check(self.lib.ppasr_stream_export_cache(self._s, att.data_ptr() if t > 0 else None,
                                                          cnn.data_ptr() if cnn.numel() else None,
                                                          stream))
        return att, cnn

    def load_caches(self, att_cache, cnn_cache, offset):
        m = self.model
        att = cnn = None
        t = 0
        if att_cache is not None and att_cache.numel() > 0:
            att = torch.as_tensor(att_cache, dtype=torch.float32).to(m.device).contiguous()
            t = int(att.shape[2])
        if cnn_cache is not None and cnn_cache.numel() > 0:
            cnn = torch.as_tensor(cnn_cache, dtype=torch.float32).to(m.device).contiguous()
        with torch.cuda.device(m.device):
            stream = torch.cuda.current_stream(m.device).cuda_stream
            _lib.check(self.lib.ppasr_stream_import_cache(self._s, None if att is None else att.data_ptr(), t,
                                                          None if cnn is None else cnn.data_ptr(), int(offset),
                                                          stream))
            torch.cuda.current_stream(m.device).synchronize()


class StreamHandleSet:

    def __init__(self, model, n_sessions, max_frames=0):
        self.model = model
        self.n_sessions = int(n_sessions)
        self._streams = [model.new_stream() for _ in range(self.n_sessions)]

    def offset(self, session):
        return self._streams[int(session)].offset

    def reset(self, session=-1):
        for i in (range(self.n_sessions) if int(session) < 0 else [int(session)]):
            self._streams[i].reset()

    def encode_chunks(self, sessions, speech, want_probs=False):
        m = self.model
        x = torch.as_tensor(speech, dtype=torch.float32).to(m.device)
        assert x.dim() == 3 and int(x.shape[0]) == len(sessions)
        outs = [self._streams[int(sid)].encode_chunk(x[k:k + 1], -16, want_probs=want_probs, want_frames=True)
                for k, sid in enumerate(sessions)]
        fa = torch.cat([o[1] for o in outs], 0)
        fp = torch.cat([o[2] for o in outs], 0)
        if want_probs:
            return fa, fp, torch.cat([o[0] for o in outs], 0)
        return fa, fp


def make_stream_group(model, n_sessions, max_frames=0):
    from ppasr_amd.model_utils.deepspeech2.model import DeepSpeech2Model, DeepSpeech2StreamGroup
    if isinstance(model, DeepSpeech2Model):
        return DeepSpeech2StreamGroup(model, n_sessions, max_frames=max_frames)
    try:
        return ConformerStreamGroup(model, n_sessions, max_frames=max_frames)
    except _lib.PPASRHipError as e:
        if e.status != _lib.PPASR_EUNSUPPORTED:
            raise
        return StreamHandleSet(model, n_sessions, max_frames=max_frames)


class ConformerStreamGroup:

    _create = "ppasr_stream_group_create"

    def __init__(self, model, n_sessions, max_frames=0):
        self.model = model
        self.lib = model.lib
        self.n_sessions = int(n_sessions)
        self._g = ctypes.c_void_p()
        with torch.cuda.device(model.device):
            _lib.check(getattr(self.lib, self._create)(model._h, self.n_sessions, int(max_frames), ctypes.byref(self._g)))
        self._ws = {}

    def __del__(self):
        g = getattr(self, "_g", None)
        if g is not None and g.value:
            self.lib.ppasr_stream_group_destroy(g)
            self._g = None

    def offset(self, session):
        return int(self.lib.ppasr_stream_group_offset(self._g, int(session)))

    def reset(self, session=-1):
        m = self.model
        with torch.cuda.device(m.device):
            _lib.check(self.lib.ppasr_stream_group_reset(self._g, int(session),
                                                         torch.cuda.current_stream(m.device).cuda_stream))

    def encode_chunks(self, sessions, speech, want_probs=False):
        m = self.model
        x = torch.as_tensor(speech, dtype=torch.float32).to(m.device).contiguous()
        n, T = int(x.shape[0]), int(x.shape[1])
        assert x.dim() == 3 and x.shape[2] == m.input_dim and n == len(sessions)
        c = m.out_frames(T)
        need = int(self.lib.ppasr_group_chunk_workspace_bytes(m._h, n, T))
        key = torch.cuda.current_stream(m.device).cuda_stream
        ws = self._ws.get(key)
        if ws is None or ws.numel() < need:
            ws = torch.empty(need, dtype=torch.uint8, device=m.device)
            self._ws[key] = ws
        probs = torch.empty(n, c, m.vocab_size, dtype=torch.float32, device=m.device) if want_probs else None
        fa = torch.empty(n, c, dtype=torch.int32, device=m.device)
        fp = torch.empty(n, c, dtype=torch.float32, device=m.device)
        ids = (ctypes.c_int * n)(*[int(s) for s in sessions])
        c_out = ctypes.c_int(0)
        with torch.cuda.device(m.device):
            _lib.check(self.lib.ppasr_encode_chunk_group(self._g, ids, n, x.data_ptr(), T,
                                                         None if probs is None else probs.data_ptr(), fa.data_ptr(),
                                                         fp.data_ptr(), ctypes.byref(c_out), ws.data_ptr(), ws.numel(),
                                                         key))
        return (fa, fp, probs) if want_probs else (fa, fp)


class GeneralConformerStreamGroup(ConformerStreamGroup):

    _create = "ppasr_gen_stream_group_create"
```

Baseline: 58440 audio-s/s.

## Fuse embed into first FFN/QKV kernel and last conv-FFN into CTC head

Adds a kernel that runs the front-end embedding GEMM and feeds its output straight into the first layer's macaron FFN and QKV projection. Adds a second kernel that runs the last layer's conv/FFN and then the CTC head's argmax and softmax statistics inside the same block. It also replaces the full memset of the vt buffer with a tail-only clear, or does the clear inside the kernel. Together these remove launches and HBM round-trips of activations at both ends of the encoder. The cost is fixed per-block tiles, which may lower occupancy, and the head tiles are now processed by only one block per row group.

```diff
diff --git a/include/ppasr_hip.h b/include/ppasr_hip.h
--- a/include/ppasr_hip.h
+++ b/include/ppasr_hip.h
@@ -96,6 +96,8 @@
 
 #define PPASR_ROW_BLOCK_32_W16 1032
 PPASR_API ppasr_status ppasr_set_row_block(ppasr_handle h, int rows);
+
+PPASR_API ppasr_status ppasr_set_fused_ends(ppasr_handle h, int mode);
 
 #define PPASR_GEMM_F32 0
 #define PPASR_GEMM_F16X3 1
diff --git a/ppasr_amd/_lib.py b/ppasr_amd/_lib.py
--- a/ppasr_amd/_lib.py
+++ b/ppasr_amd/_lib.py
@@ -59,6 +59,7 @@
     ("ppasr_set_debug_taps", ctypes.c_int, [_vp, _vp, ctypes.c_size_t]),
     ("ppasr_set_skip_padding", ctypes.c_int, [_vp, ctypes.c_int]),
     ("ppasr_set_row_block", ctypes.c_int, [_vp, ctypes.c_int]),
+    ("ppasr_set_fused_ends", ctypes.c_int, [_vp, ctypes.c_int]),
     ("ppasr_set_lengths_hint", ctypes.c_int, [_vp, _vp, ctypes.c_int]),
     ("ppasr_set_ffn_split", ctypes.c_int, [_vp, ctypes.c_int]),
     ("ppasr_set_front_fused", ctypes.c_int, [_vp, ctypes.c_int]),
diff --git a/ppasr_amd/csrc/capi.hip b/ppasr_amd/csrc/capi.hip
--- a/ppasr_amd/csrc/capi.hip
+++ b/ppasr_amd/csrc/capi.hip
@@ -219,6 +219,13 @@
   if (rows != -1 && rows != 16 && rows != 32 && rows != PPASR_ROW_BLOCK_32_W16)
     return fail(PPASR_EINVAL, "row block: -1 (by grid size), 16, 32 or PPASR_ROW_BLOCK_32_W16");
   h->row_block = rows;
+  return PPASR_OK;
+}
+
+ppasr_status ppasr_set_fused_ends(ppasr_handle h, int mode) {
+  if (!h) return fail(PPASR_EINVAL, "null handle");
+  if (mode < -1 || mode > 1) return fail(PPASR_EINVAL, "fused ends: -1 (by rule), 0 (never) or 1 (wherever the kernels serve the call)");
+  h->fused_ends = mode;
   return PPASR_OK;
 }
 
@@ -443,7 +450,6 @@
   float *y1 = ws + wl.y1, *y2 = ws + wl.y2, *xa = ws + wl.xa, *xb = ws + wl.xb, *xc = ws + wl.xc;
   float *qkv = ws + wl.qkv, *ctx = ws + wl.ctx, *g = ws + wl.g;
   const VtOut vt_out{ws + wl.vt, wl.vt_stride};
-  HIP_TRY(hipMemsetAsync(ws + wl.vt, 0, (size_t)kD * wl.vt_stride * sizeof(float), st));
   size_t tap_off = 0;
   auto tap = [&](const float* src, size_t n) {
     if (h->taps && tap_off + n <= h->taps_floats)
@@ -491,6 +497,29 @@
     }
     return ps;
   };
+  struct LayerForm { int form, S; };
+  auto layer_form = [&](int layer, int Tcur, int mul_cur) {
+    const int rows = (!h->taps && conv_ffn_16_supported(h->layer_ks[layer], Tcur))
+                         ? row_block_for(h, B, Tcur, mul_cur, pskip(Tcur, mul_cur).slack, skip) : 32;
+    const bool r16 = rows == 16 && h->ffn_split < 0;
+    const int S = r16 ? 1 : ffn_split_for(h, B * Tcur);
+    return LayerForm{r16 ? 16 : (rows == kW16 && S == 1) ? kW16 : 32, S};
+  };
+  const bool ends_ok = (h->fused_ends == 1 || (h->fused_ends < 0 && h->ffn_split < 0)) && h->desc.input_layer == 0 && h->gemm_mode != PPASR_GEMM_F16X3 && !h->taps &&
+                       !skip && h->desc.num_blocks > 0;
+  const bool head_ok = ends_ok && !probs && !logits;
+  const LayerForm lf0 = h->desc.num_blocks > 0 ? layer_form(0, Tp, sub) : LayerForm{32, 1};
+  const bool fuse_front = ends_ok && lf0.form == 32 && lf0.S == 1 && wide_slices_for(h, M, F2) <= 1;
+  const bool vt_rows_written = !skip && h->desc.num_blocks > 0 && h->layer_group[0] == 1 && h->desc.attention_heads == 4 &&
+                               !h->taps && fuse_rows(M) && lf0.form == 32 && lf0.S == 1;
+  const bool vt_tail_in_kernel = vt_rows_written && fuse_front;
+  if (!vt_rows_written) {
+    HIP_TRY(hipMemsetAsync(ws + wl.vt, 0, (size_t)kD * wl.vt_stride * sizeof(float), st));
+  } else if (!vt_tail_in_kernel) {
+    const size_t octs = (size_t)wl.vt_stride >> 3, oct0 = (size_t)((M + kRows - 1) / kRows) * (kRows / 8);
+    if (oct0 < octs)
+      HIP_TRY(hipMemset2DAsync(ws + wl.vt + oct0 * 256, octs * 256 * sizeof(float), 0, (octs - oct0) * 256 * sizeof(float), 8, st));
+  }
   const f32x4* conv2_h3 = h->gemm_mode == PPASR_GEMM_F16X3 ? h->conv2_w_h3 : nullptr;
   const bool conv12 = h->desc.input_layer == 0 && !conv2_h3 && conv12_enabled(h) && conv12_supported(h->front, F, F2);
   const PadSkip ps_front = skip_front ? pskip(Tp, sub) : PadSkip{};
@@ -509,10 +538,11 @@
         launch_conv2_quad(y1, h->front, y2, B, T1, F1, Tp, F2, st, ps_front, tile_tab);
       else launch_conv2(y1, h->front, y2, B, T1, F1, Tp, F2, st, ps_front, tile_tab, h->desc.input_layer == 0 ? conv2_h3 : nullptr);
     });
-    timed(2, [&] {
-      launch_embed(y2, h->front, xa, M, F2 * kD, sqrtf((float)kD), false, st, ps_front, wide_slices_for(h, M, F2), y1,
-                   conv2_h3 ? h->embed_w_h3 : nullptr);
-    });
+    if (!fuse_front)
+      timed(2, [&] {
+        launch_embed(y2, h->front, xa, M, F2 * kD, sqrtf((float)kD), false, st, ps_front, wide_slices_for(h, M, F2), y1,
+                     conv2_h3 ? h->embed_w_h3 : nullptr);
+      });
   }
   tap(xa, (size_t)M * kD);
   const int n_chunks = h->desc.linear_units / 256;
@@ -533,6 +563,9 @@
     p.tab = t;
     return p;
   };
+  int32_t* fa = frame_argmax ? frame_argmax : reinterpret_cast<int32_t*>(ws + wl.fa);
+  float* fp = frame_maxprob ? frame_maxprob : ws + wl.fp;
+  bool head_done = false;
   int Ti = Tp, mul = sub, pstride = 1;
   bool s1_done = false;
   for (int i = 0; i < h->desc.num_blocks; ++i) {
@@ -543,12 +576,10 @@
       return h->layer_group[layer] == 1 && h->desc.attention_heads == 4 && !h->taps && fuse_rows(Mi);
     };
     const PadSkip ps = pskip(Ti, mul);
-    const int rows = (!h->taps && conv_ffn_16_supported(h->layer_ks[i], Ti)) ? row_block_for(h, B, Ti, mul, ps.slack, skip) : 32;
-    const bool r16 = rows == 16 && h->ffn_split < 0;
+    const LayerForm lf = layer_form(i, Ti, mul);
+    const int form = lf.form, S = lf.S;
+    const bool r16 = form == 16, w16 = form == kW16;
     const bool fuse_attn = !r16 && fusable(i);
-    const int S = r16 ? 1 : ffn_split_for(h, Mi);
-    const bool w16 = rows == kW16 && S == 1;
-    const int form = r16 ? 16 : w16 ? kW16 : 32;
     const PadSkip psb = S == 1 ? with_table(ps, Ti, form_rows(form)) : ps;
     const bool h3 = h->gemm_mode == PPASR_GEMM_F16X3 && !h->layers_h3.empty() && !r16 && !w16 && S == 1;
     const bool h3s = h->gemm_mode == PPASR_GEMM_F16X3 && !h->layers_h3.empty() && S > 1;
@@ -571,6 +602,11 @@
           launch_ffn_split(xa, L.ln_mac_g, L.ln_mac_b, Lk.ffm_w1, L.ffm_b1, Lk.ffm_w2, L.ffm_b2, 0.5f, nullptr, nullptr, partial,
                            xb, Mi, n_chunks, S, st, ps, false, h3s);
           launch_ln_qkv(xb, qkv, Lk, Mi, st, ps, nullptr, nullptr, h3s);
+        });
+      } else if (i == 0 && fuse_front) {
+        timed(3, [&] {
+          launch_embed_ffn_qkv(y2, h->front, F2 * kD, sqrtf((float)kD), xb, qkv, L, Mi, n_chunks, st, vt_for(fuse_attn, false, 0),
+                               vt_tail_in_kernel);
         });
       } else {
         timed(3, [&] { launch_ffn_qkv(xa, xb, qkv, Lk, Mi, n_chunks, st, psb, vt_for(fuse_attn, h3, i), h3, form); });
@@ -625,7 +661,14 @@
       });
     } else {
       const LayerW* next = (i + 1 < h->desc.num_blocks) ? (h3 ? &h->layers_h3[i + 1] : &h->layers[i + 1]) : nullptr;
-      timed(next ? 8 : 6, [&] {
+      head_done = !next && head_ok && form == 32 && !h3 && conv_ffn_head_supported(h->layer_ks[i]) &&
+                  wide_slices_for(h, Mi, std::min((h->head.n_tiles + 7) / 8, 32)) <= 1;
+      if (head_done)
+        timed(6, [&] {
+          launch_conv_ffn_head(g, xc, L, lens, Mi, Ti, n_chunks, h->layer_ks[i], mul, st, h->desc.causal != 0, h->head, fa, fp,
+                               ws + wl.rmax, ws + wl.rsum);
+        });
+      else timed(next ? 8 : 6, [&] {
         launch_conv_ffn(g, nullptr, xc, (next && !h->taps) ? nullptr : xa, Lk, lens, Mi, Ti, n_chunks, h->layer_ks[i], mul, next,
                         xb, qkv, st, h->desc.causal != 0, psb, vt_for(next && fusable(i + 1), h3, next ? i + 1 : i), h3, form);
       });
@@ -635,9 +678,7 @@
   }
   const int Mo = B * Ti;
   float* lg = logits ? logits : probs;
-  int32_t* fa = frame_argmax ? frame_argmax : reinterpret_cast<int32_t*>(ws + wl.fa);
-  float* fp = frame_maxprob ? frame_maxprob : ws + wl.fp;
-  timed(7, [&] {
+  if (!head_done) timed(7, [&] {
     const bool head_h3 = h->gemm_mode == PPASR_GEMM_F16X3 && h->head_w_h3;
     HeadW hw = h->head;
     if (head_h3) hw.w = h->head_w_h3;
diff --git a/ppasr_amd/csrc/capi_internal.h b/ppasr_amd/csrc/capi_internal.h
--- a/ppasr_amd/csrc/capi_internal.h
+++ b/ppasr_amd/csrc/capi_internal.h
@@ -227,6 +227,7 @@
   unsigned int guard_seen[kGuardN] = {};
   long long guard_fallbacks = 0, guard_events = 0;
   int row_block = -1;
+  int fused_ends = -1;
   std::vector<int64_t> lens_hint;
   std::vector<hipEvent_t> ev_pool;
   size_t ev_used = 0;
diff --git a/ppasr_amd/csrc/conformer_kernels.h b/ppasr_amd/csrc/conformer_kernels.h
--- a/ppasr_amd/csrc/conformer_kernels.h
+++ b/ppasr_amd/csrc/conformer_kernels.h
@@ -172,6 +172,12 @@
                      const int64_t* lens, int M, int Tp, int n_chunks, int ksize, int mask_mul, const LayerW* next,
                      float* x1_next, float* qkv_next, hipStream_t st, bool causal = true, const PadSkip& ps = PadSkip{},
                      VtOut vt_next = VtOut{}, bool h3 = false, int rows = 32);
+void launch_embed_ffn_qkv(const float* y2, const FrontW& fw, int K, float xscale, float* x1, float* qkv, const LayerW& w, int M,
+                          int n_chunks, hipStream_t st, VtOut vt, bool clear_vt_tail);
+bool conv_ffn_head_supported(int ksize);
+void launch_conv_ffn_head(const float* g, const float* x2, const LayerW& w, const int64_t* lens, int M, int Tp, int n_chunks,
+                          int ksize, int mask_mul, hipStream_t st, bool causal, const HeadW& hw, int32_t* fr_argmax,
+                          float* fr_maxprob, float* row_max, float* row_sum);
 void launch_conv_pre(const float* g, const float* g_hist, const float* x2, float* x3, const LayerW& w, const int64_t* lens,
                      int M, int Tp, int ksize, int mask_mul, hipStream_t st, bool causal = true,
                      const PadSkip& ps = PadSkip{}, bool h3 = false);
diff --git a/ppasr_amd/csrc/conformer_kernels.hip b/ppasr_amd/csrc/conformer_kernels.hip
--- a/ppasr_amd/csrc/conformer_kernels.hip
+++ b/ppasr_amd/csrc/conformer_kernels.hip
@@ -1050,6 +1050,138 @@
                  n_chunks, mask_mul_out, ps, causal ? 1 : 0, x3_out);
 }
 
+struct EmbedStageSide {
+  const f32x4 (&stg)[4];
+  float* dst;
+  const int (&off)[4];
+  __device__ __forceinline__ void operator()(int g) const {
+    if ((g & 7) == 4 && dst) *reinterpret_cast<f32x4*>(dst + off[g >> 3]) = stg[g >> 3];
+  }
+};
+__global__ __launch_bounds__(kThreads) void k_embed_ffn_qkv(const float* __restrict__ y2, const f32x4* __restrict__ embed_w,
+                                                            const float* __restrict__ embed_b, int n_kc, float xscale,
+                                                            float* __restrict__ x1, float* __restrict__ qkv, LayerW w, int M,
+                                                            int n_chunks, VtOut vt, int clear_vt_tail) {
+  extern __shared__ __attribute__((aligned(16))) float smem[];
+  float* bufX = smem;
+  float* bufA = bufX + kRows * kLda;
+  float* bufH = bufA + kRows * kLda;
+  constexpr int KC = 256, G = KC / 8, F4_PER_ROW = KC / 4, NL = kRows * F4_PER_ROW / kThreads;
+  static_assert(NL == 4 && G == kG256, "four 16-byte pieces per thread and chunk, one per 8 k-groups");
+  const int tid = threadIdx.x, lane = lane_id(), wave = wave_id();
+  const int r0 = blockIdx.x * kRows;
+  const int valid = min(kRows, M - r0);
+  const int K = n_kc * KC;
+  const f32x4* wbase = embed_w + (size_t)wave * n_kc * kTs256;
+  BRing<1> ring;
+  ring_prime(ring, wbase, 0);
+  const float* tile_base = y2 + (size_t)r0 * K;
+  const __amdgpu_buffer_rsrc_t rs_a = wstream_rsrc(tile_base);
+  int voff[NL], lds_off[NL];
+#pragma unroll
+  for (int i = 0; i < NL; ++i) {
+    const int idx = tid + kThreads * i;
+    const int row = idx / F4_PER_ROW, c4 = idx - row * F4_PER_ROW;
+    voff[i] = (row < valid) ? (int)((size_t)row * K * sizeof(float)) + 16 * c4 : 0x7fffffff;
+    lds_off[i] = row * kLda + 4 * c4;
+  }
+  f32x4 stg[NL];
+  auto load_chunk = [&](int kc) {
+    const int soff = kc * KC * (int)sizeof(float);
+#pragma unroll
+    for (int i = 0; i < NL; ++i) stg[i] = wstream_load(rs_a, voff[i], soff);
+  };
+  f32x16 acc[1][1];
+  acc_zero(acc);
+  load_chunk(0);
+#pragma unroll
+  for (int i = 0; i < NL; ++i) *reinterpret_cast<f32x4*>(bufH + lds_off[i]) = stg[i];
+  __syncthreads();
+  for (int kc = 0; kc < n_kc; ++kc) {
+    const float* cur = bufH + (kc & 1) * kRows * kLda;
+    float* nxt = bufH + ((kc + 1) & 1) * kRows * kLda;
+    const bool more = kc + 1 < n_kc;
+    if (more) load_chunk(kc + 1);
+    const f32x4* seg = wbase + (size_t)kc * kTs256;
+    rb_gemm<1, 1, G, kPF, EmbedStageSide>(cur, kLda, seg, 0, more ? seg + kTs256 : w.ffm_w1 + (size_t)wave * kTs256, 0, ring, acc,
+                                          EmbedStageSide{stg, more ? nxt : nullptr, lds_off});
+    __syncthreads();
+  }
+  {
+    const int col = wave * 32 + (lane & 31);
+    const float bv = embed_b[col];
+#pragma unroll
+    for (int r = 0; r < 16; ++r) {
+      const int row = acc_row(r, lane);
+      bufX[row * kLda + col] = row < valid ? (acc[0][0][r] + bv) * xscale : 0.f;
+    }
+  }
+  __syncthreads();
+  ffn_qkv_body(bufX, bufA, bufH, x1, qkv, w, r0, valid, n_chunks, ring, vt);
+  if (clear_vt_tail && vt.vt && blockIdx.x == gridDim.x - 1) {
+    const int octs = vt.stride >> 3;
+    for (int o = (r0 >> 3) + kRows / 8; o < octs; ++o)
+      *reinterpret_cast<f32x4*>(vt.vt + ((size_t)wave * octs + o) * 256 + 4 * lane) = f32x4{0.f, 0.f, 0.f, 0.f};
+  }
+}
+void launch_embed_ffn_qkv(const float* y2, const FrontW& fw, int K, float xscale, float* x1, float* qkv, const LayerW& w, int M,
+                          int n_chunks, hipStream_t st, VtOut vt, bool clear_vt_tail) {
+  PPASR_LAUNCH(k_embed_ffn_qkv, dim3((M + kRows - 1) / kRows), dim3(kThreads), kLdsFfnQkv, st, y2, fw.embed_w, fw.embed_b,
+               K / 256, xscale, x1, qkv, w, M, n_chunks, vt, clear_vt_tail ? 1 : 0);
+}
+
+template <int KS>
+__global__ __launch_bounds__(kThreads) void k_conv_ffn_head(const float* __restrict__ g, const float* __restrict__ x2, LayerW w,
+                                                            const int64_t* __restrict__ lens, int M, int Tp, int n_chunks,
+                                                            int mask_mul, int left_ctx, HeadW hw, int32_t* __restrict__ fr_argmax,
+                                                            float* __restrict__ fr_maxprob, float* __restrict__ row_max,
+                                                            float* __restrict__ row_sum) {
+  conv_ffn_body<KS, false, false, false>(g, nullptr, x2, nullptr, w, lens, M, Tp, n_chunks, mask_mul, w, nullptr, nullptr,
+                                         left_ctx, PadSkip{}, VtOut{});
+  extern __shared__ __attribute__((aligned(16))) float smem[];
+  float* bufX = smem;
+  float* bufA = bufX + kRows * kLda;
+  float* redM = bufA + kRows * kLda;
+  float* redS = redM + kWaves * 32;
+  int* redI = reinterpret_cast<int*>(redS + kWaves * 32);
+  const int lane = lane_id(), wave = wave_id();
+  const int r0 = blockIdx.x * kRows;
+  const int valid = min(kRows, M - r0);
+  BRing<1> ring;
+  if (wave < hw.n_tiles) ring_prime(ring, hw.w + (size_t)wave * kTs256, 0);
+  const float* a = bufX;
+  if (hw.ln_g) {
+    rb_layernorm(bufX, bufA, kLda, kRows, hw.ln_g, hw.ln_b, 1e-5f);
+    a = bufA;
+  }
+  __syncthreads();
+  CtcRun run;
+  for (int tile = wave; tile < hw.n_tiles; tile += kWaves) {
+    f32x16 acc[1][1];
+    acc_zero(acc);
+    const f32x4* seg = hw.w + (size_t)tile * kTs256;
+    rb_gemm<1, 1, kG256, kPF, NoSide, true>(a, kLda, seg, 0, tile + kWaves < hw.n_tiles ? seg + (size_t)kWaves * kTs256 : nullptr,
+                                            0, ring, acc);
+    ctc_tile_update<false>(run, acc[0][0], hw, tile, lane >> 5, nullptr);
+  }
+  ctc_rows_finish(run, redM, redS, redI, r0, valid, M, 1, 0, nullptr, fr_argmax, fr_maxprob, row_max, row_sum);
+}
+bool conv_ffn_head_supported(int ksize) { return ksize == 15 || ksize == 7; }
+void launch_conv_ffn_head(const float* g, const float* x2, const LayerW& w, const int64_t* lens, int M, int Tp, int n_chunks,
+                          int ksize, int mask_mul, hipStream_t st, bool causal, const HeadW& hw, int32_t* fr_argmax,
+                          float* fr_maxprob, float* row_max, float* row_sum) {
+  dim3 grid((M + kRows - 1) / kRows);
+  const int left_ctx = causal ? ksize - 1 : (ksize - 1) / 2;
+  if (ksize == 15)
+    PPASR_LAUNCH(k_conv_ffn_head<15>, grid, dim3(kThreads), kLdsConvFfn, st, g, x2, w, lens, M, Tp, n_chunks, mask_mul, left_ctx,
+                 hw, fr_argmax, fr_maxprob, row_max, row_sum);
+  else if (ksize == 7)
+    PPASR_LAUNCH(k_conv_ffn_head<7>, grid, dim3(kThreads), kLdsConvFfn, st, g, x2, w, lens, M, Tp, n_chunks, mask_mul, left_ctx,
+                 hw, fr_argmax, fr_maxprob, row_max, row_sum);
+  else
+    check_form("launch_conv_ffn_head (cnn_module_kernel 15 or 7)", 0, false);
+}
+
 hipError_t configure_kernels() {
   hipError_t e = configure_attention_kernels();
   if (e != hipSuccess) return e;
@@ -1069,6 +1201,9 @@
   e = hipFuncSetAttribute(reinterpret_cast<const void*>(fn), hipFuncAttributeMaxDynamicSharedMemorySize, (int)(bytes)); \
   if (e != hipSuccess) return e;
   SET_LDS(k_ffn_qkv, kLdsFfnQkv);
+  SET_LDS(k_embed_ffn_qkv, kLdsFfnQkv);
+  SET_LDS(k_conv_ffn_head<15>, kLdsConvFfn);
+  SET_LDS(k_conv_ffn_head<7>, kLdsConvFfn);
   SET_LDS(k_ffn_qkv_h3, kLdsFfnQkv + kH3ExtraLds);
   SET_LDS((k_conv_ffn_h3<15, true>), kLdsConvFfn + kH3ExtraLds);
   SET_LDS((k_conv_ffn_h3<15, false>), kLdsConvFfn + kH3ExtraLds);
diff --git a/ppasr_amd/csrc/ctc_head_kernels.hip b/ppasr_amd/csrc/ctc_head_kernels.hip
--- a/ppasr_amd/csrc/ctc_head_kernels.hip
+++ b/ppasr_amd/csrc/ctc_head_kernels.hip
@@ -32,10 +32,8 @@
   if (hw.ln_g) rb_layernorm(bufA, bufA, kLda, kRows, hw.ln_g, hw.ln_b, 1e-5f);
   __syncthreads();
   if constexpr (H3) h3_planes_from_tile(bufA, reinterpret_cast<_Float16*>(bufA));
-  float mx = -INFINITY, sm = 0.f;
-  int ix = 0x7fffffff;
+  CtcRun run;
   const int l31 = lane & 31, hh = lane >> 5;
-  constexpr float kLog2e = 1.4426950408889634f;
   const int tstep = kWaves * ny;
   for (int tile = wave + 8 * y; tile < hw.n_tiles; tile += tstep) {
     f32x16 acc[1][1];
@@ -49,90 +47,9 @@
       rb_gemm<1, 1, kG256, kPF, NoSide, true>(bufA, kLda, seg, 0, tile + tstep < hw.n_tiles ? seg + (size_t)tstep * kTs256 : nullptr,
                                               0, ring, acc);
     }
-    const int c0 = tile * 32 + 4 * hh;
-    float v[16];
-#pragma unroll
-    for (int q = 0; q < 4; ++q) {
-      const f32x4 bq = *reinterpret_cast<const f32x4*>(hw.b + c0 + 8 * q);
-#pragma unroll
-      for (int e = 0; e < 4; ++e) v[4 * q + e] = acc[0][0][4 * q + e] + bq[e];
-    }
-    if (tile == hw.n_tiles - 1 && (V & 31)) {
-#pragma unroll
-      for (int r = 0; r < 16; ++r)
-        if (c0 + 8 * (r >> 2) + (r & 3) >= V) v[r] = -INFINITY;
-    }
-    if (LOGITS) {
-      if (l31 < valid) {
-        float* lrow = logits + (size_t)(r0 + l31) * V;
-#pragma unroll
-        for (int r = 0; r < 16; ++r) {
-          const int col = c0 + 8 * (r >> 2) + (r & 3);
-          if (col < V) lrow[col] = v[r];
-        }
-      }
-    }
-    float tmax = max3f(v[0], v[1], v[2]);
-#pragma unroll
-    for (int r = 3; r < 15; r += 2) tmax = max3f(tmax, v[r], v[r + 1]);
-    tmax = fmaxf(tmax, v[15]);
-    if (tmax > mx) {
-#pragma unroll
-      for (int r = 15; r >= 0; --r) ix = (v[r] == tmax) ? c0 + 8 * (r >> 2) + (r & 3) : ix;
-    }
-    const float mn = fmaxf(mx, tmax);
-    sm *= __builtin_amdgcn_exp2f((mx - mn) * kLog2e);
-    f32x2 ps = {0.f, 0.f};
-#pragma unroll
-    for (int r = 0; r < 16; r += 2) {
-      const f32x2 t = (f32x2{v[r], v[r + 1]} - f32x2{mn, mn}) * f32x2{kLog2e, kLog2e};
-      ps += f32x2{__builtin_amdgcn_exp2f(t[0]), __builtin_amdgcn_exp2f(t[1])};
-    }
-    sm += ps[0] + ps[1];
-    mx = mn;
-  }
-  {
-    const float m2 = __shfl_xor(mx, 32), s2 = __shfl_xor(sm, 32);
-    const int i2 = __shfl_xor(ix, 32);
-    const float mn = fmaxf(mx, m2);
-    const float sa = (mx == -INFINITY) ? 0.f : sm * __expf(mx - mn);
-    const float sb = (m2 == -INFINITY) ? 0.f : s2 * __expf(m2 - mn);
-    const bool take2 = (m2 > mx) || (m2 == mx && i2 < ix);
-    if (hh == 0) {
-      redM[wave * 32 + l31] = mn;
-      redS[wave * 32 + l31] = sa + sb;
-      redI[wave * 32 + l31] = take2 ? i2 : ix;
-    }
-  }
-  __syncthreads();
-  if (threadIdx.x < 32) {
-    const int row = threadIdx.x;
-    float m = redM[row], s = redS[row];
-    int i = redI[row];
-    for (int wv = 1; wv < kWaves; ++wv) {
-      float m2 = redM[wv * 32 + row], s2 = redS[wv * 32 + row];
-      int i2 = redI[wv * 32 + row];
-      float mn = fmaxf(m, m2);
-      float sa = (m == -INFINITY) ? 0.f : s * __expf(m - mn);
-      float sb = (m2 == -INFINITY) ? 0.f : s2 * __expf(m2 - mn);
-      bool take2 = (m2 > m) || (m2 == m && i2 < i);
-      i = take2 ? i2 : i;
-      m = mn;
-      s = sa + sb;
-    }
-    if (row < valid) {
-      if (ny > 1) {
-        part[(size_t)y * M + r0 + row] = m;
-        part[((size_t)ny + y) * M + r0 + row] = s;
-        reinterpret_cast<int*>(part)[((size_t)2 * ny + y) * M + r0 + row] = i;
-      } else {
-        if (fr_argmax) fr_argmax[r0 + row] = i;
-        if (fr_maxprob) fr_maxprob[r0 + row] = 1.0f / s;
-        if (row_max) row_max[r0 + row] = m;
-        if (row_sum) row_sum[r0 + row] = s;
-      }
-    }
-  }
+    ctc_tile_update<LOGITS>(run, acc[0][0], hw, tile, hh, (LOGITS && l31 < valid) ? logits + (size_t)(r0 + l31) * V : nullptr);
+  }
+  ctc_rows_finish(run, redM, redS, redI, r0, valid, M, ny, y, part, fr_argmax, fr_maxprob, row_max, row_sum);
 }
 __global__ void k_ctc_merge(const float* __restrict__ part, int ny, int32_t* __restrict__ fr_argmax,
                             float* __restrict__ fr_maxprob, float* __restrict__ row_max, float* __restrict__ row_sum, int M,
diff --git a/ppasr_amd/csrc/phases.h b/ppasr_amd/csrc/phases.h
--- a/ppasr_amd/csrc/phases.h
+++ b/ppasr_amd/csrc/phases.h
@@ -242,4 +242,109 @@
     }
 }
 
-}
+struct CtcRun {
+  float mx = -INFINITY, sm = 0.f;
+  int ix = 0x7fffffff;
+};
+template <bool LOGITS>
+__device__ __forceinline__ void ctc_tile_update(CtcRun& run, const f32x16& acc, const HeadW& hw, int tile, int hh,
+                                                float* __restrict__ lrow) {
+  constexpr float kLog2e = 1.4426950408889634f;
+  const int V = hw.V;
+  float& mx = run.mx;
+  float& sm = run.sm;
+  int& ix = run.ix;
+  const int c0 = tile * 32 + 4 * hh;
+  float v[16];
+#pragma unroll
+  for (int q = 0; q < 4; ++q) {
+    const f32x4 bq = *reinterpret_cast<const f32x4*>(hw.b + c0 + 8 * q);
+#pragma unroll
+    for (int e = 0; e < 4; ++e) v[4 * q + e] = acc[4 * q + e] + bq[e];
+  }
+  if (tile == hw.n_tiles - 1 && (V & 31)) {
+#pragma unroll
+    for (int r = 0; r < 16; ++r)
+      if (c0 + 8 * (r >> 2) + (r & 3) >= V) v[r] = -INFINITY;
+  }
+  if (LOGITS) {
+    if (lrow) {
+#pragma unroll
+      for (int r = 0; r < 16; ++r) {
+        const int col = c0 + 8 * (r >> 2) + (r & 3);
+        if (col < V) lrow[col] = v[r];
+      }
+    }
+  }
+  float tmax = max3f(v[0], v[1], v[2]);
+#pragma unroll
+  for (int r = 3; r < 15; r += 2) tmax = max3f(tmax, v[r], v[r + 1]);
+  tmax = fmaxf(tmax, v[15]);
+  if (tmax > mx) {
+#pragma unroll
+    for (int r = 15; r >= 0; --r) ix = (v[r] == tmax) ? c0 + 8 * (r >> 2) + (r & 3) : ix;
+  }
+  const float mn = fmaxf(mx, tmax);
+  sm *= __builtin_amdgcn_exp2f((mx - mn) * kLog2e);
+  f32x2 ps = {0.f, 0.f};
+#pragma unroll
+  for (int r = 0; r < 16; r += 2) {
+    const f32x2 t = (f32x2{v[r], v[r + 1]} - f32x2{mn, mn}) * f32x2{kLog2e, kLog2e};
+    ps += f32x2{__builtin_amdgcn_exp2f(t[0]), __builtin_amdgcn_exp2f(t[1])};
+  }
+  sm += ps[0] + ps[1];
+  mx = mn;
+}
+__device__ __forceinline__ void ctc_rows_finish(const CtcRun& run, float* redM, float* redS, int* redI, int r0, int valid, int M,
+                                                int ny, int y, float* __restrict__ part, int32_t* __restrict__ fr_argmax,
+                                                float* __restrict__ fr_maxprob, float* __restrict__ row_max,
+                                                float* __restrict__ row_sum) {
+  const int lane = lane_id(), wave = wave_id();
+  const int l31 = lane & 31, hh = lane >> 5;
+  const float mx = run.mx, sm = run.sm;
+  const int ix = run.ix;
+  {
+    const float m2 = __shfl_xor(mx, 32), s2 = __shfl_xor(sm, 32);
+    const int i2 = __shfl_xor(ix, 32);
+    const float mn = fmaxf(mx, m2);
+    const float sa = (mx == -INFINITY) ? 0.f : sm * __expf(mx - mn);
+    const float sb = (m2 == -INFINITY) ? 0.f : s2 * __expf(m2 - mn);
+    const bool take2 = (m2 > mx) || (m2 == mx && i2 < ix);
+    if (hh == 0) {
+      redM[wave * 32 + l31] = mn;
+      redS[wave * 32 + l31] = sa + sb;
+      redI[wave * 32 + l31] = take2 ? i2 : ix;
+    }
+  }
+  __syncthreads();
+  if (threadIdx.x < 32) {
+    const int row = threadIdx.x;
+    float m = redM[row], s = redS[row];
+    int i = redI[row];
+    for (int wv = 1; wv < kWaves; ++wv) {
+      float m2 = redM[wv * 32 + row], s2 = redS[wv * 32 + row];
+      int i2 = redI[wv * 32 + row];
+      float mn = fmaxf(m, m2);
+      float sa = (m == -INFINITY) ? 0.f : s * __expf(m - mn);
+      float sb = (m2 == -INFINITY) ? 0.f : s2 * __expf(m2 - mn);
+      bool take2 = (m2 > m) || (m2 == m && i2 < i);
+      i = take2 ? i2 : i;
+      m = mn;
+      s = sa + sb;
+    }
+    if (row < valid) {
+      if (ny > 1) {
+        part[(size_t)y * M + r0 + row] = m;
+        part[((size_t)ny + y) * M + r0 + row] = s;
+        reinterpret_cast<int*>(part)[((size_t)2 * ny + y) * M + r0 + row] = i;
+      } else {
+        if (fr_argmax) fr_argmax[r0 + row] = i;
+        if (fr_maxprob) fr_maxprob[r0 + row] = 1.0f / s;
+        if (row_max) row_max[r0 + row] = m;
+        if (row_sum) row_sum[r0 + row] = s;
+      }
+    }
+  }
+}
+
+}
diff --git a/ppasr_amd/model_utils/conformer/model.py b/ppasr_amd/model_utils/conformer/model.py
--- a/ppasr_amd/model_utils/conformer/model.py
+++ b/ppasr_amd/model_utils/conformer/model.py
@@ -201,6 +201,9 @@
     def set_row_block(self, rows=-1):
         _lib.check(self.lib.ppasr_set_row_block(self._h, int(rows)))
 
+    def set_fused_ends(self, mode=-1):
+        _lib.check(self.lib.ppasr_set_fused_ends(self._h, int(mode)))
+
     def set_lengths_hint(self, lengths=None):
         if lengths is None:
             _lib.check(self.lib.ppasr_set_lengths_hint(self._h, None, 0))
```

Result: no change. 58710 audio-s/s, median of 6 (+0.5%).
